# chaoting-sun/GCT-Plus

Hardware: AMD Instinct MI355X
Metric: SMILES/sec training step (vaetf, seq_len=80, d_model=512) (higher is better)
Workload: dtype f32

## Files before the change

### gct_plus_amd/csrc/gemm.hip

```cpp
#include <limits.h>
#include <stdlib.h>

#include <type_traits>

#include "common.h"

typedef float f32x16 __attribute__((ext_vector_type(16)));

namespace {

constexpr int BM = 128, BN = 128, BK = 32;
constexpr int TILE_FLOATS = BM * BK;

struct Seg3 {
  const float* p0;
  int64_t d1, d2;
};

struct GemmArgs {
  int64_t M, N, K;
  Seg3 a;
  int64_t lda;
  int64_t a_nper;
  Seg3 b;
// ... 839 lines not shown
int64_t g_x3_kernel_launches = 0;
#include "gemm_x6.inc"

__global__ __launch_bounds__(256) void gemm_f32_small_kernel(const GemmArgs g) {
  constexpr int SB = 64, STILE = SB * BK;
  __shared__ __attribute__((aligned(16))) float lds[4 * STILE];
  const int tid = threadIdx.x, lane = tid & 63, wave = tid >> 6;
  const int wm = (wave >> 1) * 32, wn = (wave & 1) * 32;
  const unsigned tiles_n = (unsigned)((g.N + SB - 1) / SB);
  const unsigned tiles_m = (unsigned)((g.M + SB - 1) / SB);
  const unsigned lid0 = gct_xcd_remap(blockIdx.x, gridDim.x);
  const unsigned z = lid0 / (tiles_m * tiles_n), lid = lid0 - z * (tiles_m * tiles_n);
  const int64_t m0 = (int64_t)(lid / tiles_n) * SB, n0 = (int64_t)(lid % tiles_n) * SB;
  const int64_t kbeg = (int64_t)z * g.ksplit;
  const int64_t kend = (kbeg + g.ksplit < g.K) ? kbeg + g.ksplit : g.K;

  uint32_t offa[2], offb[2];
#pragma unroll
  for (int i = 0; i < 2; ++i) {
    int64_t r = (tid >> 3) + 32 * i;
    int64_t ra_ = r, rb_ = r;
    if (m0 + ra_ > g.M - 1) ra_ = g.M - 1 - m0;
    if (n0 + rb_ > g.N - 1) rb_ = g.N - 1 - n0;
    offa[i] = (uint32_t)(ra_ * g.lda + (tid & 7) * 4);
    offb[i] = (uint32_t)(rb_ * g.ldb + (tid & 7) * 4);
  }
  const bool g1 = n0 >= g.b_nper, g2 = n0 >= 2 * g.b_nper;
  const float* bbase0 = g.b.p0 + (g2 ? g.b.d2 : (g1 ? g.b.d1 : 0)) +
                        (n0 - (g2 ? 2 * g.b_nper : (g1 ? g.b_nper : 0))) * g.ldb;
  const float* abase0 = g.a.p0 + m0 * g.lda;

  f32x16 acc;
#pragma unroll
  for (int r = 0; r < 16; ++r) acc[r] = 0.f;
  float4 ra[2], rb[2];
  auto gload = [&](int64_t k0) {
#pragma unroll
    for (int i = 0; i < 2; ++i) {
      ra[i] = *reinterpret_cast<const float4*>(abase0 + k0 + offa[i]);
      rb[i] = *reinterpret_cast<const float4*>(bbase0 + k0 + offb[i]);
    }
  };
  auto lstore = [&](int buf) {
    float* la = lds + buf * 2 * STILE;
    float* lb = la + STILE;
    const int c8 = tid & 7;
#pragma unroll
    for (int i = 0; i < 2; ++i) {
      const int row = (tid >> 3) + 32 * i;
      const int chunk = c8 ^ ((row >> 1) & 7);
      *reinterpret_cast<float4*>(la + row * BK + chunk * 4) = ra[i];
      *reinterpret_cast<float4*>(lb + row * BK + chunk * 4) = rb[i];
    }
  };
  const int64_t nkt = (kend - kbeg) / BK;
  gload(kbeg);
  lstore(0);
  __syncthreads();
  const int h = lane >> 5;
  for (int64_t kt = 0; kt < nkt; ++kt) {
    const int cur = (int)(kt & 1);
    if (kt + 1 < nkt) gload(kbeg + (kt + 1) * BK);
    const float* la = lds + cur * 2 * STILE;
    const float* lb = la + STILE;
    const int rowa = wm + (lane & 31), rowb = wn + (lane & 31);
    const int swa = (rowa >> 1) & 7, swb = (rowb >> 1) & 7;
#pragma unroll
    for (int c = 0; c < 4; ++c) {
      const float4 a4 = *reinterpret_cast<const float4*>(la + rowa * BK + (((h * 4 + c) ^ swa) * 4));
      const float4 b4 = *reinterpret_cast<const float4*>(lb + rowb * BK + (((h * 4 + c) ^ swb) * 4));
      acc = __builtin_amdgcn_mfma_f32_32x32x2f32(a4.x, b4.x, acc, 0, 0, 0);
      acc = __builtin_amdgcn_mfma_f32_32x32x2f32(a4.y, b4.y, acc, 0, 0, 0);
      acc = __builtin_amdgcn_mfma_f32_32x32x2f32(a4.z, b4.z, acc, 0, 0, 0);
      acc = __builtin_amdgcn_mfma_f32_32x32x2f32(a4.w, b4.w, acc, 0, 0, 0);
    }
    if (kt + 1 < nkt) lstore(cur ^ 1);
    __syncthreads();
  }
  float* stg = lds + wave * 1024;
  {
    const int c32 = lane & 31;
#pragma unroll
    for (int r = 0; r < 16; ++r) stg[((r & 3) + 8 * (r >> 2) + 4 * h) * 32 + c32] = acc[r];
  }
  __builtin_amdgcn_s_waitcnt(0xC07F);
  __builtin_amdgcn_wave_barrier();
  const FastEpi ep{g};
  const int rg = lane >> 3, c4 = lane & 7;
  const int64_t row0 = m0 + wm + rg * 4, col0 = n0 + wn + c4 * 4;
  if (row0 < g.M && col0 < g.N) {
    float4 v[4];
#pragma unroll
    for (int rr = 0; rr < 4; ++rr) v[rr] = *reinterpret_cast<const float4*>(stg + (rg * 4 + rr) * 32 + c4 * 4);
    if (g.epi == EPI_SLAB) {
      float* sl = g.c0 + (int64_t)z * g.slab_stride;
#pragma unroll
      for (int rr = 0; rr < 4; ++rr)
        if (row0 + rr < g.M) *reinterpret_cast<float4*>(sl + (row0 + rr) * g.N + col0) = v[rr];
      return;
    }
    const bool q1 = col0 >= g.c_nper, q2 = col0 >= 2 * g.c_nper;
    const int64_t cloc = col0 - (q2 ? 2 * g.c_nper : (q1 ? g.c_nper : 0));
    float* cbase = g.c0 + (q2 ? g.c_d2 : (q1 ? g.c_d1 : 0));
    float4 bias = make_float4(0.f, 0.f, 0.f, 0.f);
    if (g.bias0) bias = *reinterpret_cast<const float4*>(g.bias0 + (q2 ? g.bias_d2 : (q1 ? g.bias_d1 : 0)) + cloc);
    ep.apply(v, row0, col0, cbase, cloc, bias);
  }
}


template <int TN, bool RAGGED = false>
__global__ __launch_bounds__(256) void gemm_f32_panel_kernel(const GemmArgs g) {
  constexpr int TM = 32, KC = 256, SD = KC + 4, NBL = TN / 4;
  extern __shared__ __attribute__((aligned(16))) float plds[];
  float* As = plds;
  float* Bs = plds + TM * SD;
  const int tid = threadIdx.x, lane = tid & 63, wave = tid >> 6, g4 = lane >> 4, c16 = lane & 15;
  const unsigned tiles_m = (unsigned)((g.M + TM - 1) / TM);
  const unsigned lid = gct_xcd_remap(blockIdx.x, gridDim.x);
  const int64_t m0 = (int64_t)(lid % tiles_m) * TM, n0 = (int64_t)(lid / tiles_m) * TN;
  const bool s1 = n0 >= g.b_nper, s2 = n0 >= 2 * g.b_nper;
  const float* bbase = g.b.p0 + (s2 ? g.b.d2 : (s1 ? g.b.d1 : 0)) + (n0 - (s2 ? 2 * g.b_nper : (s1 ? g.b_nper : 0))) * g.ldb;
  const float* abase = g.a.p0;
  uint32_t offa[8], offb[NBL];
#pragma unroll
  for (int i = 0; i < 8; ++i) {
    const int idx = tid + 256 * i, row = idx >> 6, c4 = idx & 63;
    int64_t r = m0 + row;
    if (r > g.M - 1) r = g.M - 1;
    offa[i] = (uint32_t)(r * g.lda + c4 * 4);
  }
#pragma unroll
  for (int i = 0; i < NBL; ++i) {
    const int idx = tid + 256 * i, c4 = idx & 63;
    int64_t row = idx >> 6;
    if (RAGGED && n0 + row > g.N - 1) row = g.N - 1 - n0;
    offb[i] = (uint32_t)(row * g.ldb + c4 * 4);
  }
  f32x4_t ra[8], rb[NBL];
  auto gload = [&](int64_t k0) {
#pragma unroll
    for (int i = 0; i < 8; ++i) ra[i] = *reinterpret_cast<const f32x4_t*>(abase + k0 + offa[i]);
#pragma unroll
    for (int i = 0; i < NBL; ++i) rb[i] = *reinterpret_cast<const f32x4_t*>(bbase + k0 + offb[i]);
  };
  auto lstore = [&]() {
#pragma unroll
    for (int i = 0; i < 8; ++i) {
      const int idx = tid + 256 * i;
      *reinterpret_cast<f32x4_t*>(As + (idx >> 6) * SD + (idx & 63) * 4) = ra[i];
    }
#pragma unroll
    for (int i = 0; i < NBL; ++i) {
      const int idx = tid + 256 * i;
      *reinterpret_cast<f32x4_t*>(Bs + (idx >> 6) * SD + (idx & 63) * 4) = rb[i];
    }
  };
  constexpr int NS = TN / 32;
  const int wm = (wave >> 1) * 16, wn = (wave & 1) * (TN / 2);
  f32x4_t acc[NS];
#pragma unroll
  for (int j = 0; j < NS; ++j) acc[j] = (f32x4_t){0.f, 0.f, 0.f, 0.f};
  const int64_t nch = g.K / KC;
  gload(0);
  lstore();
  __syncthreads();
  for (int64_t c = 0; c < nch; ++c) {
    if (c + 1 < nch) gload((c + 1) * KC);
    const float* ap = As + (wm + c16) * SD + g4 * 64;
#pragma unroll 4
    for (int j = 0; j < 16; ++j) {
      const float4 a4 = *reinterpret_cast<const float4*>(ap + 4 * j);
#pragma unroll
      for (int u = 0; u < NS; ++u) {
        const float4 b4 = *reinterpret_cast<const float4*>(Bs + (wn + 16 * u + c16) * SD + g4 * 64 + 4 * j);
        acc[u] = __builtin_amdgcn_mfma_f32_16x16x4f32(a4.x, b4.x, acc[u], 0, 0, 0);
        acc[u] = __builtin_amdgcn_mfma_f32_16x16x4f32(a4.y, b4.y, acc[u], 0, 0, 0);
        acc[u] = __builtin_amdgcn_mfma_f32_16x16x4f32(a4.z, b4.z, acc[u], 0, 0, 0);
        acc[u] = __builtin_amdgcn_mfma_f32_16x16x4f32(a4.w, b4.w, acc[u], 0, 0, 0);
      }
    }
    __syncthreads();
    if (c + 1 < nch) {
      lstore();
      __syncthreads();
    }
  }
  float* stg = plds + wave * (16 * 20);
  const FastEpi ep{g};
#pragma unroll
  for (int u = 0; u < NS; ++u) {
#pragma unroll
    for (int i = 0; i < 4; ++i) stg[(4 * g4 + i) * 20 + c16] = acc[u][i];
    __builtin_amdgcn_s_waitcnt(0xC07F);
    __builtin_amdgcn_wave_barrier();
    if (lane < 16) {
      const int pr = lane >> 2, pc = lane & 3;
      const int64_t row0 = m0 + wm + 4 * pr, col0 = n0 + wn + 16 * u + 4 * pc;
      if (RAGGED) {
        for (int rr = 0; rr < 4; ++rr)
          for (int cc = 0; cc < 4; ++cc)
            if (row0 + rr < g.M && col0 + cc < g.N)
              g.c0[(row0 + rr) * g.ldc + col0 + cc] = stg[(4 * pr + rr) * 20 + 4 * pc + cc] + (g.bias0 ? g.bias0[col0 + cc] : 0.f);
      } else if (row0 < g.M && col0 < g.N) {
        float4 v[4];
#pragma unroll
        for (int rr = 0; rr < 4; ++rr) v[rr] = *reinterpret_cast<const float4*>(stg + (4 * pr + rr) * 20 + 4 * pc);
        const bool q1 = col0 >= g.c_nper, q2 = col0 >= 2 * g.c_nper;
        const int64_t cloc = col0 - (q2 ? 2 * g.c_nper : (q1 ? g.c_nper : 0));
        float* cbase = g.c0 + (q2 ? g.c_d2 : (q1 ? g.c_d1 : 0));
        float4 bias = make_float4(0.f, 0.f, 0.f, 0.f);
        if (g.bias0) bias = *reinterpret_cast<const float4*>(g.bias0 + (q2 ? g.bias_d2 : (q1 ? g.bias_d1 : 0)) + cloc);
        ep.apply(v, row0, col0, cbase, cloc, bias);
      }
    }
    __builtin_amdgcn_s_waitcnt(0xC07F);
    __builtin_amdgcn_wave_barrier();
  }
}

template <int TN, bool RAGGED = false>
int launch_panel(const GemmArgs& g, hipStream_t st) {
  constexpr size_t LDS = (size_t)(32 + TN) * 260 * sizeof(float);
  static bool attr_set = false;
  if (!attr_set) {
    hipError_t e = hipFuncSetAttribute((const void*)gemm_f32_panel_kernel<TN, RAGGED>, hipFuncAttributeMaxDynamicSharedMemorySize, (int)LDS);
    if (e != hipSuccess) {
      gct_set_error("gemm_f32_panel: cannot reserve %zu bytes of LDS: %s", LDS, hipGetErrorString(e));
      return GCT_ERR_HIP;
    }
    attr_set = true;
  }
  const int64_t tiles = ((g.M + 31) / 32) * (RAGGED ? 1 : g.N / TN);
  hipLaunchKernelGGL((gemm_f32_panel_kernel<TN, RAGGED>), dim3((unsigned)tiles), dim3(256), LDS, st, g);
  GCT_LAUNCH_CHECK("gemm_f32_panel");
  return GCT_OK;
}

__global__ __launch_bounds__(256) void splitk_epilogue_kernel(const GemmArgs g, const float* slabs,
                                                              int nslab, int64_t slab_stride) {
  const int64_t pc = g.N / 4, pr = (g.M + 3) / 4;
  const int64_t idx = (int64_t)blockIdx.x * blockDim.x + threadIdx.x;
  if (idx >= pc * pr) return;
  const int64_t row0 = (idx / pc) * 4, col0 = (idx % pc) * 4;
  float4 v[4];
#pragma unroll
  for (int rr = 0; rr < 4; ++rr) {
    v[rr] = make_float4(0.f, 0.f, 0.f, 0.f);
    if (row0 + rr < g.M) {
      const float* p = slabs + (row0 + rr) * g.N + col0;
      for (int s = 0; s < nslab; ++s) {
        const float4 t = *reinterpret_cast<const float4*>(p + (int64_t)s * slab_stride);
        v[rr].x += t.x; v[rr].y += t.y; v[rr].z += t.z; v[rr].w += t.w;
      }
    }
  }
  const bool q1 = col0 >= g.c_nper, q2 = col0 >= 2 * g.c_nper;
  const int64_t cloc = col0 - (q2 ? 2 * g.c_nper : (q1 ? g.c_nper : 0));
  float* cbase = g.c0 + (q2 ? g.c_d2 : (q1 ? g.c_d1 : 0));
  float4 bias = make_float4(0.f, 0.f, 0.f, 0.f);
  if (g.bias0) bias = *reinterpret_cast<const float4*>(g.bias0 + (q2 ? g.bias_d2 : (q1 ? g.bias_d1 : 0)) + cloc);
  const FastEpi ep{g};
  ep.apply(v, row0, col0, cbase, cloc, bias);
}

int g_gemm_mode = -1;
int64_t g_gemm_launches[2] = {0, 0};
inline int gemm_mode() {
  if (g_gemm_mode < 0) {
    const char* e = getenv("GCT_GEMM_MODE");
    g_gemm_mode = (e && (e[0] == 'f' || e[0] == '0')) ? GCT_GEMM_F32 : GCT_GEMM_BF16X6;
  }
  return g_gemm_mode;
}

template <bool A_KC, bool B_KC>
bool fast_ok(const GemmArgs& g, bool vec) {
  auto seg_ok = [](int64_t nper, int64_t extent, int64_t gran) { return nper >= extent || nper % gran == 0; };
  return vec && g.K % BK == 0 && g.ksplit % BK == 0 && g.M >= 4 && g.N >= 4 &&
         (A_KC ? seg_ok(g.a_nper, g.K, BK) : (seg_ok(g.a_nper, g.M, BM) && g.M % 4 == 0)) &&
         (B_KC ? seg_ok(g.b_nper, g.N, BN) : (seg_ok(g.b_nper, g.K, BK) && g.N % 4 == 0)) &&
         g.N % 4 == 0 && g.ldc % 4 == 0 && gct_aligned16(g.c0) && g.c_d1 % 4 == 0 && g.c_d2 % 4 == 0 &&
         (g.c_nper >= g.N || g.c_nper % 4 == 0) && g.slab_stride % 4 == 0 &&
         (!g.bias0 || (gct_aligned16(g.bias0) && g.bias_d1 % 4 == 0 && g.bias_d2 % 4 == 0)) &&
         (!g.resid || gct_aligned16(g.resid)) && (!g.pre || gct_aligned16(g.pre)) &&
         (!g.pre_in || gct_aligned16(g.pre_in)) && 130 * g.lda < (1ll << 31) && 130 * g.ldb < (1ll << 31);
}


inline int64_t slab_bytes(int64_t s, int64_t rows, int64_t cols) {
  return s > 1 ? s * rows * cols * (int64_t)sizeof(float) : 0;
}

inline bool skinny_m(int64_t M, int64_t N) { return ((M + BM - 1) / BM) * ((N + BN - 1) / BN) < 192; }

int skinny_splits(int64_t M, int64_t N, int64_t K) {
  const int64_t tiles = ((M + 63) / 64) * ((N + 63) / 64);
  if (tiles <= 0) return 1;
  int64_t ns = 768 / tiles;
  if (ns > K / BK / 4) ns = K / BK / 4;
  return ns < 1 ? 1 : (int)ns;
}

int x6_tail_plan(int64_t M, int64_t N, int64_t K, int64_t* m1_out) {
  constexpr int64_t CUS = 256;
  const int64_t tm = (M + XBM - 1) / XBM, tn = (N + XBN - 1) / XBN, tiles = tm * tn;
  const int64_t rem = tiles % CUS;
  if (tiles <= CUS || rem == 0 || rem % tn != 0 || K % XBK != 0) return 1;
  const int64_t nkt = K / XBK;
  int best = 1;
  double cost = 1.0;
  const double o = 3.3;
  for (int s2 = 2; s2 <= 8 && nkt / s2 >= 2; ++s2) {
    const double c = (double)((rem * s2 + CUS - 1) / CUS) * (o + (double)nkt / s2) / (o + nkt) + 0.05;
    if (c < cost - 1e-9) { cost = c; best = s2; }
  }
  if (best == 1 || cost > 0.75) return 1;
  *m1_out = (tiles - rem) / tn * XBM;
  return best;
}

int x6_splitk_all_plan(int64_t M, int64_t N, int64_t K) {
  constexpr int64_t CUS = 256;
  const int64_t tiles = ((M + XBM - 1) / XBM) * ((N + XBN - 1) / XBN), nkt = K / XBK;
  if (tiles > CUS / 2 || K % XBK != 0 || nkt < 32 || M < 1024 || (nkt < 64 && M < 2048)) return 1;
  int64_t sp = CUS / tiles;
  if (sp > nkt / 8) sp = nkt / 8;
  if (sp > 8) sp = 8;
  return sp < 2 ? 1 : (int)sp;
}


inline int64_t x6s_tiles(int64_t M, int64_t N) { return ((M + SBM - 1) / SBM) * ((N + SBN - 1) / SBN); }

inline bool x6s_shape(const GemmArgs& g) {
  const int64_t big = ((g.M + XBM - 1) / XBM) * ((g.N + XBN - 1) / XBN), small = x6s_tiles(g.M, g.N), nkt = g.K / XBK;
  return big <= 160 && small >= 96 && small <= (nkt <= 16 ? 512 : 256) && nkt <= 32;
}

constexpr int64_t X6_TAIL_SMALL_MAX = 512;

constexpr int64_t PANEL32_MAX_TILES = 4096, PANEL64_MAX_TILES = 768;


static_assert(BK == XBK, "the fp32 and bf16x6 kernels split K at the same granularity");
GemmArgs slab_args(const GemmArgs& g, int splits, float* ws) {
  const int64_t nkt = g.K / BK;
  GemmArgs p = g;
  p.ksplit = ((nkt + splits - 1) / splits) * BK;
  p.nsplit = (int)((g.K + p.ksplit - 1) / p.ksplit);
  p.epi = EPI_SLAB; p.c0 = ws; p.ldc = g.N; p.slab_stride = g.M * g.N;
  p.c_d1 = p.c_d2 = 0; p.c_nper = INT64_MAX / 4; p.bias0 = nullptr; p.resid = nullptr; p.pre = nullptr; p.pre_in = nullptr;
  return p;
}

int launch_fixup(const GemmArgs& g, const GemmArgs& slabs, hipStream_t st, const char* name) {
  const int64_t patches = ((g.M + 3) / 4) * (g.N / 4);
  hipLaunchKernelGGL(splitk_epilogue_kernel, dim3((unsigned)((patches + 255) / 256)), dim3(256), 0, st, g,
                     (const float*)slabs.c0, slabs.nsplit, slabs.slab_stride);
  GCT_LAUNCH_CHECK(name);
  return GCT_OK;
}

template <int MODE, int NP>
int launch_x6_tail_split(const GemmArgs& g, hipStream_t st, float* ws, int64_t ws_bytes) {
  if (MODE == X6_WGRAD || g.nsplit != 1 || !ws || !gct_aligned16(ws)) return launch_x6<MODE, NP>(g, st);
  int64_t m1 = 0;
  const int best = x6_tail_plan(g.M, g.N, g.K, &m1);
  const int64_t m2 = g.M - m1, nkt = g.K / XBK;
  hipStreamCaptureStatus cap = hipStreamCaptureStatusNone;
  if (best == 1 || slab_bytes(best, m2, g.N) > ws_bytes ||
      hipStreamIsCapturing(st, &cap) != hipSuccess || cap != hipStreamCaptureStatusNone)
    return launch_x6<MODE, NP>(g, st);
  GemmArgs head = g;
  head.M = m1;
  int rc = launch_x6<MODE, NP>(head, st);
  if (rc) return rc;
  GemmArgs e = g;
  e.M = m2; e.row_base = g.row_base + m1;
  e.a.p0 += m1 * g.lda;
  e.c0 += m1 * g.ldc;
  if (e.resid) e.resid += m1 * g.ldc;
  if (e.pre) e.pre += m1 * g.ldc;
  if (e.pre_in && !(g.pre_rows > 0 && g.quad_map)) e.pre_in += m1 * g.ldc;
  if (nkt <= 32 && x6s_tiles(m2, g.N) <= X6_TAIL_SMALL_MAX) {
    if (MODE == X6_FWD && x6s_ok(e, true)) return launch_x6s<X6_FWD, NP>(e, st);
    if (MODE == X6_DGRAD && x6s_dgrad_ok(e, true)) return launch_x6s<X6_DGRAD, NP>(e, st);
  }
  const GemmArgs p = slab_args(e, best, ws);
  rc = launch_x6<MODE, NP>(p, st);
  if (rc) return rc;
  return launch_fixup(e, p, st, "x6 tail fix-up");
}

struct GemmRoute {
  enum Kind {
    X6S,
    X6_SPLITK_ALL,
    PANEL_THIN,
    PANEL32,
    PANEL64,
    F32_SMALL,
    X6,
    F32_FAST,
    F32_VEC,
    F32,
  } kind;
  int splits;
};

template <bool A_KC, bool B_KC>
GemmRoute plan_gemm(const GemmArgs& g, bool vec, int mode, const float* ws, int64_t ws_bytes) {
  constexpr bool FWD = A_KC && B_KC, DGRAD = A_KC && !B_KC;
  constexpr int MODE = A_KC ? (B_KC ? X6_FWD : X6_DGRAD) : X6_WGRAD;
  const bool x6 = mode == GCT_GEMM_BF16X6 || mode == GCT_GEMM_BF16X3;
  const bool x6_fwd = x6 && FWD && g.epi < EPI_D0, x6_dgrad = x6 && DGRAD && g.epi >= EPI_D0 && g.epi < EPI_SLAB;
  const bool ws_ok = ws && gct_aligned16(ws);
  if (x6_fwd || x6_dgrad) {
    const bool x6s = x6_fwd ? x6s_ok(g, vec) : x6s_dgrad_ok(g, vec);
    if (x6s && x6s_shape(g)) return {GemmRoute::X6S, 1};
    if (x6_fwd && x6s && !x6_ok<X6_FWD>(g, vec) && x6s_tiles(g.M, g.N) >= 96) return {GemmRoute::X6S, 1};
    const int sp = x6_splitk_all_plan(g.M, g.N, g.K);
    if (x6_ok<MODE>(g, vec) && g.nsplit == 1 && ws_ok && sp > 1 && slab_bytes(sp, g.M, g.N) <= ws_bytes)
      return {GemmRoute::X6_SPLITK_ALL, sp};
  }
  if (FWD && vec && g.N <= 32 && g.K % 256 == 0 && g.epi == GCT_EPI_BIAS && g.nsplit == 1 && g.b_nper >= g.N &&
      g.c_nper >= g.N && g.M >= 1 && g.lda * 4 * 33 < (1ll << 31) && g.ldb * 4 * 33 < (1ll << 31) && g.M < (1ll << 36))
    return {GemmRoute::PANEL_THIN, 1};
  const bool fast = fast_ok<A_KC, B_KC>(g, vec);
  if (FWD && fast && g.nsplit == 1 && skinny_m(g.M, g.N) && g.epi < EPI_D0 && (g.b_nper >= g.N || g.b_nper % 64 == 0)) {
    if (g.K % 256 == 0 && g.lda * 4 * 33 < (1ll << 31) && g.ldb * 4 * 65 < (1ll << 31) &&
        (g.c_nper >= g.N || g.c_nper % 64 == 0)) {
      const int64_t tm32 = (g.M + 31) / 32;
      if (g.N % 32 == 0 && (g.b_nper >= g.N || g.b_nper % 32 == 0) && tm32 * (g.N / 32) <= PANEL32_MAX_TILES)
        return {GemmRoute::PANEL32, 1};
      if (g.N % 64 == 0 && tm32 * (g.N / 64) <= PANEL64_MAX_TILES) return {GemmRoute::PANEL64, 1};
    }
    int64_t ns = 1;
    if (ws_ok) {
      const int64_t slab = g.M * g.N * (int64_t)sizeof(float);
      ns = skinny_splits(g.M, g.N, g.K);
      if (ns * slab > ws_bytes) ns = ws_bytes / slab;
      if (ns < 1) ns = 1;
    }
    return {GemmRoute::F32_SMALL, (int)ns};
  }
  if (x6 && (A_KC || !B_KC) && x6_ok<MODE>(g, vec)) return {GemmRoute::X6, 1};
  return {fast ? GemmRoute::F32_FAST : (vec ? GemmRoute::F32_VEC : GemmRoute::F32), 1};
}

template <bool A_KC, bool B_KC>
int launch(const GemmArgs& g, bool vec, hipStream_t st, float* ws = nullptr, int64_t ws_bytes = 0) {
  constexpr int MODE = A_KC ? (B_KC ? X6_FWD : X6_DGRAD) : X6_WGRAD;
  const int64_t tiles = ((g.M + BM - 1) / BM) * ((g.N + BN - 1) / BN) * g.nsplit;
  if (tiles <= 0) return GCT_OK;
  if (tiles > INT_MAX) {
    gct_set_error("gemm: grid too large");
    return GCT_ERR_ARG;
  }
  const int mode = gemm_mode();
  const bool x3 = mode == GCT_GEMM_BF16X3;
  const GemmRoute r = plan_gemm<A_KC, B_KC>(g, vec, mode, ws, ws_bytes);
  switch (r.kind) {
    case GemmRoute::X6S:
      if (x3) return launch_x6s<B_KC ? X6_FWD : X6_DGRAD, 2>(g, st);
      ++g_gemm_launches[1];
      return launch_x6s<B_KC ? X6_FWD : X6_DGRAD, 3>(g, st);
    case GemmRoute::X6_SPLITK_ALL: {
      const GemmArgs p = slab_args(g, r.splits, ws);
      int rc = x3 ? launch_x6<MODE, 2>(p, st) : launch_x6<MODE, 3>(p, st);
      if (!rc) rc = launch_fixup(g, p, st, "x6 split-K fix-up");
      if (!rc && !x3) ++g_gemm_launches[1];
      return rc;
    }
    case GemmRoute::PANEL_THIN:
      ++g_gemm_launches[0];
      return launch_panel<32, true>(g, st);
    case GemmRoute::PANEL32:
      return launch_panel<32>(g, st);
    case GemmRoute::PANEL64:
      return launch_panel<64>(g, st);
    case GemmRoute::F32_SMALL: {
      const int64_t tiles64 = ((g.M + 63) / 64) * ((g.N + 63) / 64);
      if (r.splits == 1) {
        hipLaunchKernelGGL(gemm_f32_small_kernel, dim3((unsigned)tiles64), dim3(256), 0, st, g);
        GCT_LAUNCH_CHECK("gemm_f32_small");
        return GCT_OK;
      }
      const GemmArgs p = slab_args(g, r.splits, ws);
      hipLaunchKernelGGL(gemm_f32_small_kernel, dim3((unsigned)(tiles64 * p.nsplit)), dim3(256), 0, st, p);
      GCT_LAUNCH_CHECK("gemm_f32_small(split-K)");
      return launch_fixup(g, p, st, "splitk_epilogue");
    }
    case GemmRoute::X6:
      if (x3) return launch_x6_tail_split<MODE, 2>(g, st, ws, ws_bytes);
      ++g_gemm_launches[1];
      return launch_x6_tail_split<MODE, 3>(g, st, ws, ws_bytes);
    default:
      break;
  }
  ++g_gemm_launches[0];
  const dim3 grid((unsigned)tiles), block(256);
  if (r.kind == GemmRoute::F32_FAST)
    hipLaunchKernelGGL((gemm_f32_fast_kernel<A_KC, B_KC>), grid, block, 0, st, g);
  else if (r.kind == GemmRoute::F32_VEC)
    hipLaunchKernelGGL((gemm_f32_kernel<A_KC, B_KC, true>), grid, block, 0, st, g);
  else
    hipLaunchKernelGGL((gemm_f32_kernel<A_KC, B_KC, false>), grid, block, 0, st, g);
  GCT_LAUNCH_CHECK("gemm_f32");
  return GCT_OK;
}

inline bool al16(const void* p) { return p == nullptr || gct_aligned16(p); }

inline Seg3 mkseg(const float* p0, const float* p1, const float* p2) {
  Seg3 r;
  r.p0 = p0;
  r.d1 = p1 ? (int64_t)(p1 - p0) : 0;
  r.d2 = p2 ? (int64_t)(p2 - p0) : 0;
  return r;
}

}

int gct_reduce_slabs_seg(const float* slabs, int nslab, int64_t stride, float* d0, float* d1,
                         float* d2, int64_t nper_elems, int64_t n, hipStream_t st);
int gct_reduce_slabs_seg2(const float* sa, int nslab, int64_t stride_a, float* a0, float* a1, float* a2,
                          int64_t nper_a, int64_t na, const float* sb, int64_t stride_b, float* b0, float* b1,
                          float* b2, int64_t nper_b, int64_t nb, hipStream_t st);
int gct_colsum(const float* y0, const float* y1, const float* y2, int64_t ld, int64_t M, int nseg,
               int nper, float* d0, float* d1, float* d2, float* ws, hipStream_t st);
int64_t gct_colsum_ws_floats(int64_t M, int64_t N);

static int wgrad_splits(int64_t M, int64_t Ntot, int64_t K, bool x6 = false) {
  const int64_t tiles = x6 ? ((Ntot + XBM - 1) / XBM) * ((K + XBN - 1) / XBN)
                           : ((Ntot + BM - 1) / BM) * ((K + BN - 1) / BN);
  int64_t want = (x6 ? 256 : 512) / tiles;
  const int64_t maxs = (M + 4 * BK - 1) / (4 * BK);
  if (want > maxs) want = maxs;
  if (want < 1) want = 1;
  if (want > 64) want = 64;
  return (int)want;
}

extern "C" int64_t gct_wgrad_ws_bytes(int64_t M, int64_t Ntot, int64_t K) {
  const int s1 = wgrad_splits(M, Ntot, K), s2 = wgrad_splits(M, Ntot, K, true);
  const int s = s1 > s2 ? s1 : s2;
  const int64_t slab = (int64_t)s * Ntot * K;
  const int64_t cs = gct_colsum_ws_floats(M, Ntot);
  const int64_t need = slab + 4 + (int64_t)s * Ntot;
  return (need > cs ? need : cs) * (int64_t)sizeof(float) + 256;
}

extern "C" int gct_linear_fwd(const float* x, int64_t ldx, int64_t M, int K, const float* w0,
                              const float* w1, const float* w2, int64_t ldw, const uint16_t* wp0,
                              int64_t plane_stride, const float* b0, const float* b1,
                              const float* b2, int nseg, int nper, float* y0, float* y1, float* y2,
                              int64_t ldy, int epi, const float* resid, float* pre, float p,
                              uint64_t seed, uint32_t site, float* ws, int64_t ws_bytes,
                              const int32_t* quad_map, void* stream) {
  GCT_CHECK_ARG(x && w0 && y0 && M >= 0 && K > 0 && nseg >= 1 && nseg <= 3 && nper > 0,
                "linear_fwd: bad args");
  GCT_CHECK_ARG(!quad_map || M % 4 == 0, "linear_fwd: compacted rows come in quads");
  GCT_CHECK_ARG(ws_bytes >= 0, "linear_fwd: negative workspace size");
  GCT_CHECK_ARG(nseg < 2 || (w1 && y1), "linear_fwd: missing segment 1");
  GCT_CHECK_ARG(nseg < 3 || (w2 && y2), "linear_fwd: missing segment 2");
  GCT_CHECK_ARG(epi == GCT_EPI_BIAS || nseg == 1, "linear_fwd: fused epilogues need nseg == 1");
  GCT_CHECK_ARG(epi >= GCT_EPI_BIAS && epi <= GCT_EPI_GELU_DROP_SAVE, "linear_fwd: unknown epilogue %d", epi);
  GCT_CHECK_ARG((epi != GCT_EPI_GELU_DROP && epi != GCT_EPI_GELU_DROP_SAVE) || pre, "linear_fwd: GELU epilogue needs pre");
  GCT_CHECK_ARG(epi != GCT_EPI_DROP_RESID || resid, "linear_fwd: residual epilogue needs resid");
  GCT_CHECK_ARG(p >= 0.f && p < 1.f, "linear_fwd: dropout p out of range");
  GemmArgs g = {};
  g.M = M; g.N = (int64_t)nseg * nper; g.K = K;
  GCT_CHECK_ARG(!b0 || nseg < 2 || b1, "linear_fwd: bias of segment 1 missing");
  GCT_CHECK_ARG(!b0 || nseg < 3 || b2, "linear_fwd: bias of segment 2 missing");
  g.a = mkseg(x, nullptr, nullptr); g.lda = ldx; g.a_nper = INT64_MAX / 4;
  g.b = mkseg(w0, w1, w2); g.ldb = ldw; g.b_nper = nper;
  g.c0 = y0; g.c_d1 = y1 ? y1 - y0 : 0; g.c_d2 = y2 ? y2 - y0 : 0; g.ldc = ldy; g.c_nper = nper;
  g.ksplit = K; g.nsplit = 1; g.epi = epi;
  g.bias0 = b0; g.bias_d1 = (b0 && b1) ? b1 - b0 : 0; g.bias_d2 = (b0 && b2) ? b2 - b0 : 0;
  g.resid = resid; g.pre = pre;
  g.thr = gct_drop_threshold(p); g.keep_scale = 1.0f / (1.0f - p); g.rng = gct_rng_make(seed, site);
  g.bp0 = wp0; g.bp_stride = plane_stride;
  g.quad_map = quad_map;
  const bool vec = al16(x) && al16(w0) && al16(w1) && al16(w2) && (ldx % 4 == 0) &&
                   (ldw % 4 == 0) && (K % 4 == 0);
  return launch<true, true>(g, vec, (hipStream_t)stream, ws, ws ? ws_bytes : 0);
}

extern "C" int gct_gemm_set_mode(int mode) {
  GCT_CHECK_ARG(mode == GCT_GEMM_F32 || mode == GCT_GEMM_BF16X6 || mode == GCT_GEMM_BF16X3,
                "gemm_set_mode: unknown mode %d", mode);
  g_gemm_mode = mode;
  return GCT_OK;
}
extern "C" int gct_gemm_get_mode(void) { return gemm_mode(); }
extern "C" int64_t gct_gemm_x6_kernel_launches(void) { return g_x6_kernel_launches; }
extern "C" int64_t gct_gemm_x3_launches(void) { return g_x3_kernel_launches; }
extern "C" int gct_gemm_launch_counts(int64_t* out2) {
  GCT_CHECK_ARG(out2, "gemm_launch_counts: null");
  out2[0] = g_gemm_launches[0]; out2[1] = g_gemm_launches[1];
  return GCT_OK;
}

extern "C" int gct_split_planes(const float* src, int64_t numel, uint16_t* planes, int64_t plane_stride,
                                void* stream) {
  GCT_CHECK_ARG(src && planes && numel >= 0 && numel % 4 == 0 && plane_stride >= numel && plane_stride % 4 == 0 &&
                    gct_aligned16(src) && ((((uintptr_t)planes) & 7u) == 0),
                "split_planes: bad args (numel and plane_stride must be multiples of 4, src 16-B aligned)");
  if (numel == 0) return GCT_OK;
  const int64_t n4 = numel / 4;
  hipLaunchKernelGGL(split_planes_kernel, dim3((unsigned)((n4 + 255) / 256)), dim3(256), 0, (hipStream_t)stream,
                     src, planes, n4, plane_stride);
  GCT_LAUNCH_CHECK("split_planes");
  return GCT_OK;
}

extern "C" int64_t gct_linear_fwd_ws_bytes(int64_t M, int K, int Ntot) {
  int64_t need = 0, m1 = 0;
  if (skinny_m(M, Ntot)) {
    need = slab_bytes(skinny_splits(M, Ntot, K), M, Ntot);
  } else {
    const int s = x6_tail_plan(M, Ntot, K, &m1);
    need = slab_bytes(s, M - m1, Ntot);
  }
  const int64_t all = slab_bytes(x6_splitk_all_plan(M, Ntot, K), M, Ntot);
  return (need > all ? need : all) + 256;
}

extern "C" int64_t gct_linear_dgrad_ws_bytes(int64_t M, int Ntot, int K) {
  int64_t m1 = 0;
  const int s = x6_tail_plan(M, K, Ntot, &m1);
  const int64_t tail = slab_bytes(s, M - m1, K);
  const int64_t all = slab_bytes(x6_splitk_all_plan(M, K, Ntot), M, K);
  return (tail > all ? tail : all) + 256;
}

extern "C" int gct_linear_dgrad(const float* dy0, const float* dy1, const float* dy2, int64_t lddy,
                                int64_t M, int nseg, int nper, const float* w0, const float* w1,
                                const float* w2, int64_t ldw, const uint16_t* wp0,
                                int64_t plane_stride, int K, float* dx, int64_t lddx, int depi,
                                const float* pre, float p, uint64_t seed, uint32_t site,
                                float* ws, int64_t ws_bytes, const int32_t* quad_map, int64_t pre_rows,
                                void* stream) {
  GCT_CHECK_ARG(ws_bytes >= 0, "linear_dgrad: negative workspace size");
  GCT_CHECK_ARG(dy0 && w0 && dx && M >= 0 && K > 0 && nseg >= 1 && nseg <= 3 && nper > 0,
                "linear_dgrad: bad args");
  GCT_CHECK_ARG(!quad_map || M % 4 == 0, "linear_dgrad: compacted rows come in quads");
  GCT_CHECK_ARG(nseg < 2 || (w1 && dy1), "linear_dgrad: missing segment 1");
  GCT_CHECK_ARG(nseg < 3 || (w2 && dy2), "linear_dgrad: missing segment 2");
  GCT_CHECK_ARG(depi >= GCT_DEPI_STORE && depi <= GCT_DEPI_MUL_SAVED, "linear_dgrad: unknown epilogue %d", depi);
  GCT_CHECK_ARG(depi != GCT_DEPI_GELU_BWD || pre, "linear_dgrad: GELU bwd needs pre");
  GCT_CHECK_ARG(depi != GCT_DEPI_MUL_SAVED || pre, "linear_dgrad: saved-factor epilogue needs pre");
  GCT_CHECK_ARG(p >= 0.f && p < 1.f, "linear_dgrad: dropout p out of range");
  GemmArgs g = {};
  g.M = M; g.N = K; g.K = (int64_t)nseg * nper;
  g.a = mkseg(dy0, dy1, dy2); g.lda = lddy; g.a_nper = nper;
  g.b = mkseg(w0, w1, w2); g.ldb = ldw; g.b_nper = nper;
  g.c0 = dx; g.ldc = lddx; g.c_nper = INT64_MAX / 4;
  g.ksplit = g.K; g.nsplit = 1; g.epi = EPI_D0 + depi;
  g.pre_in = pre;
  g.thr = gct_drop_threshold(p); g.keep_scale = 1.0f / (1.0f - p); g.rng = gct_rng_make(seed, site);
  g.bp0 = wp0; g.bp_stride = plane_stride;
  g.quad_map = quad_map;
  g.pre_rows = quad_map ? pre_rows : 0;
  const bool vec = al16(dy0) && al16(dy1) && al16(dy2) && al16(w0) && al16(w1) && al16(w2) &&
                   (lddy % 4 == 0) && (ldw % 4 == 0) && (nper % 4 == 0) && (K % 4 == 0);
  return launch<true, false>(g, vec, (hipStream_t)stream, ws, ws ? ws_bytes : 0);
}

extern "C" int gct_linear_wgrad(const float* dy0, const float* dy1, const float* dy2, int64_t lddy,
                                int64_t M, int nseg, int nper, const float* x, int64_t ldx, int K,
                                float* dw0, float* dw1, float* dw2, int64_t lddw, float* db0,
                                float* db1, float* db2, float* ws, const int32_t* tile_list,
                                const int32_t* tile_count, void* stream) {
  GCT_CHECK_ARG(dy0 && x && dw0 && ws && M >= 0 && K > 0 && nseg >= 1 && nseg <= 3 && nper > 0,
                "linear_wgrad: bad args");
  GCT_CHECK_ARG(nseg < 2 || (dy1 && dw1), "linear_wgrad: missing segment 1");
  GCT_CHECK_ARG(nseg < 3 || (dy2 && dw2), "linear_wgrad: missing segment 2");
  GCT_CHECK_ARG(lddw == K, "linear_wgrad: dW must be dense [nper][K]");
  hipStream_t st = (hipStream_t)stream;
  const int64_t Ntot = (int64_t)nseg * nper;
  const bool vec = al16(dy0) && al16(dy1) && al16(dy2) && al16(x) && (lddy % 4 == 0) &&
                   (ldx % 4 == 0) && (nper % 4 == 0) && (K % 4 == 0);
  GemmArgs g = {};
  g.M = Ntot; g.N = K; g.K = M;
  g.a = mkseg(dy0, dy1, dy2); g.lda = lddy; g.a_nper = nper;
  g.b = mkseg(x, nullptr, nullptr); g.ldb = ldx; g.b_nper = INT64_MAX / 4;
  g.c0 = ws; g.ldc = K; g.c_nper = INT64_MAX / 4;
  g.slab_stride = Ntot * K;
  g.ksplit = BK; g.nsplit = 1; g.epi = EPI_SLAB;
  const bool use_x6 = gemm_mode() != GCT_GEMM_F32 && x6_ok<X6_WGRAD>(g, vec);
  if (use_x6 && tile_list && tile_count) { g.kt_list = tile_list; g.kt_count = tile_count; }
  const int splits = wgrad_splits(M, Ntot, K, use_x6);
  int64_t ks = (M + splits - 1) / splits;
  ks = (ks + BK - 1) / BK * BK;
  g.ksplit = ks > 0 ? ks : BK;
  g.nsplit = (int)((M + g.ksplit - 1) / g.ksplit);
  if (g.nsplit < 1) g.nsplit = 1;
  g.epi = EPI_SLAB;
  float* bslab = nullptr;
  if (db0) {
    if (use_x6 || fast_ok<false, false>(g, vec)) {
      int64_t off = (int64_t)g.nsplit * g.slab_stride;
      off = (off + 3) / 4 * 4;
      bslab = ws + off;
      g.bias_slab = bslab;
    } else {
      int rc = gct_colsum(dy0, dy1, dy2, lddy, M, nseg, nper, db0, db1, db2, ws, st);
      if (rc) return rc;
    }
  }
  int rc = launch<false, false>(g, vec, st);
  if (rc) return rc;
  if (bslab)
    return gct_reduce_slabs_seg2(ws, g.nsplit, g.slab_stride, dw0, dw1, dw2, (int64_t)nper * K, Ntot * K, bslab, Ntot,
                                 db0, db1, db2, nper, Ntot, st);
  return gct_reduce_slabs_seg(ws, g.nsplit, g.slab_stride, dw0, dw1, dw2, (int64_t)nper * K, Ntot * K, st);
}
```

### gct_plus_amd/csrc/gemm_x6.inc

```

typedef __bf16 x6_bf16x8 __attribute__((ext_vector_type(8)));
typedef __bf16 x6_bf16x2 __attribute__((ext_vector_type(2)));
typedef float x6_f32x2 __attribute__((ext_vector_type(2)));
typedef unsigned x6_u32x4 __attribute__((ext_vector_type(4)));
typedef unsigned x6_u32x2 __attribute__((ext_vector_type(2)));
typedef short x6_s16x4 __attribute__((ext_vector_type(4)));
typedef short x6_s16x8 __attribute__((ext_vector_type(8)));

enum { X6_FWD = 0, X6_DGRAD = 1, X6_WGRAD = 2 };
constexpr int XBM = 128, XBN = 256, XBK = 32;
constexpr int X_APL = 8192, X_BPL = 16384, X_STAGE = 3 * X_APL + 3 * X_BPL;
constexpr int X_KLIST_MAX = 1024;
constexpr int X_LDS_BYTES = 2 * X_STAGE + X_KLIST_MAX * 4;

__device__ __forceinline__ unsigned x6_pk(float a, float b) {
  x6_f32x2 v = {a, b};
  return __builtin_bit_cast(unsigned, __builtin_convertvector(v, x6_bf16x2));
}
__device__ __forceinline__ float x6_sub(float a, float b) {
  float r;
  asm("v_sub_f32 %0, %1, %2" : "=v"(r) : "v"(a), "v"(b));
  return r;
}
__device__ __forceinline__ void x6_split2(float a, float b, unsigned& h, unsigned& m, unsigned& l) {
  h = x6_pk(a, b);
  const float ra = x6_sub(a, __uint_as_float(h << 16)), rb = x6_sub(b, __uint_as_float(h & 0xffff0000u));
  m = x6_pk(ra, rb);
  const float sa = x6_sub(ra, __uint_as_float(m << 16)), sb = x6_sub(rb, __uint_as_float(m & 0xffff0000u));
  l = x6_pk(sa, sb);
}
__device__ __forceinline__ void x6_split4(const float4 v, x6_u32x2& h, x6_u32x2& m, x6_u32x2& l) {
  unsigned h0, m0, l0, h1, m1, l1;
  x6_split2(v.x, v.y, h0, m0, l0);
  x6_split2(v.z, v.w, h1, m1, l1);
  h = x6_u32x2{h0, h1}; m = x6_u32x2{m0, m1}; l = x6_u32x2{l0, l1};
}
template <int NP>
__device__ __forceinline__ void x6_split4n(const float4 v, x6_u32x2 (&pc)[NP]) {
  if constexpr (NP == 3) {
    x6_split4(v, pc[0], pc[1], pc[2]);
  } else {
    static_assert(NP == 2, "bf16x6 (3 pieces) or bf16x3 (2 pieces)");
    unsigned h0, h1;
    h0 = x6_pk(v.x, v.y);
    h1 = x6_pk(v.z, v.w);
    const float r0 = x6_sub(v.x, __uint_as_float(h0 << 16)), r1 = x6_sub(v.y, __uint_as_float(h0 & 0xffff0000u));
    const float r2 = x6_sub(v.z, __uint_as_float(h1 << 16)), r3 = x6_sub(v.w, __uint_as_float(h1 & 0xffff0000u));
    pc[0] = x6_u32x2{h0, h1};
    pc[1] = x6_u32x2{x6_pk(r0, r1), x6_pk(r2, r3)};
  }
}

__device__ __forceinline__ int x6_row_off(int r, int c) {
  const int g = (0x78 >> (2 * ((r >> 2) & 3))) & 3;
  return r * 64 + ((c ^ g) << 4);
}
__device__ __forceinline__ int x6_tr_off(int k, int cb, int stride) {
  return k * stride + (cb ^ (((k & 3) << 6) | (((k >> 3) & 1) << 5)));
}

__device__ __forceinline__ x6_bf16x8 x6_tr_frag(const unsigned char* p, int stride) {
  typedef __attribute__((address_space(3))) x6_s16x4 lds_s16x4;
  const x6_s16x4 lo = __builtin_amdgcn_ds_read_tr16_b64_v4i16((lds_s16x4*)(p));
  const x6_s16x4 hi = __builtin_amdgcn_ds_read_tr16_b64_v4i16((lds_s16x4*)(p + 4 * stride));
  const x6_s16x8 v = __builtin_shufflevector(lo, hi, 0, 1, 2, 3, 4, 5, 6, 7);
  return __builtin_bit_cast(x6_bf16x8, v);
}

typedef float x6_f32x4 __attribute__((ext_vector_type(4)));
#define X6_MFMA(a_, b_, c_) c_ = __builtin_amdgcn_mfma_f32_16x16x32_bf16(a_, b_, c_, 0, 0, 0)

template <int MODE, int NP = 3>
__global__ __launch_bounds__(512) __attribute__((amdgpu_waves_per_eu(2, 2))) void
gemm_x6_kernel(const GemmArgs g) {
  static_assert(NP == 2 || NP == 3, "bf16x3 or bf16x6");
  extern __shared__ __attribute__((aligned(16))) unsigned char xlds[];
  constexpr bool A_TR = MODE == X6_WGRAD, B_TR = MODE != X6_FWD, B_PL = MODE != X6_WGRAD;
  constexpr int NB = B_PL ? 2 : 4;
  const int tid = threadIdx.x, lane = tid & 63, wave = tid >> 6;
  const int wm = (wave >> 2) * 64, wn = (wave & 3) * 64;

  const unsigned tiles_n = (unsigned)((g.N + XBN - 1) / XBN);
  const unsigned tiles_m = (unsigned)((g.M + XBM - 1) / XBM);
  const unsigned per_split = tiles_m * tiles_n;
  const unsigned lid = gct_xcd_remap(blockIdx.x, gridDim.x);
  const unsigned z = lid / per_split, rest = lid - z * per_split;
  const int64_t m0 = (int64_t)(rest / tiles_n) * XBM, n0 = (int64_t)(rest % tiles_n) * XBN;
  const int64_t kbeg = (int64_t)z * g.ksplit;
  const int64_t kend = (kbeg + g.ksplit < g.K) ? kbeg + g.ksplit : g.K;

  uint32_t offa[2], offb[NB];
  int sta[2], stb[NB];
#pragma unroll
  for (int j = 0; j < 2; ++j) {
    if (!A_TR) {
      int64_t r = (tid >> 3) + 64 * j;
      sta[j] = x6_row_off((int)r, (tid & 7) >> 1) + (tid & 1) * 8;
      if (m0 + r > g.M - 1) r = g.M - 1 - m0;
      offa[j] = (uint32_t)(r * g.lda + (tid & 7) * 4);
    } else {
      const int kr = (tid >> 5) + 16 * j;
      int64_t c = (tid & 31) * 4;
      sta[j] = x6_tr_off(kr, (tid & 31) * 8, 256);
      if (m0 + c > g.M - 4) c = g.M - 4 - m0;
      offa[j] = (uint32_t)(kr * g.lda + c);
    }
  }
#pragma unroll
  for (int j = 0; j < NB; ++j) {
    if (MODE == X6_FWD) {
      int64_t r = (tid >> 2) + 128 * j;
      stb[j] = x6_row_off((int)r, tid & 3);
      if (n0 + r > g.N - 1) r = g.N - 1 - n0;
      offb[j] = (uint32_t)(r * g.ldb + (tid & 3) * 8);
    } else if (MODE == X6_DGRAD) {
      const int kr = (tid >> 5) + 16 * j;
      int64_t c = (tid & 31) * 8;
      stb[j] = x6_tr_off(kr, (tid & 31) * 16, 512);
      if (n0 + c > g.N - 8) c = g.N - 8 - n0;
      offb[j] = (uint32_t)(kr * g.ldb + c);
    } else {
      const int kr = (tid >> 6) + 8 * j;
      int64_t c = (tid & 63) * 4;
      stb[j] = x6_tr_off(kr, (tid & 63) * 8, 512);
      if (n0 + c > g.N - 4) c = g.N - 4 - n0;
      offb[j] = (uint32_t)(kr * g.ldb + c);
    }
  }
  auto seg_off = [](const Seg3& s, int64_t idx, int64_t nper, int64_t& local) -> int64_t {
    const bool g1 = idx >= nper, g2 = idx >= 2 * nper;
    local = idx - (g2 ? 2 * nper : (g1 ? nper : 0));
    return g2 ? s.d2 : (g1 ? s.d1 : 0);
  };
  int64_t a_fix = 0, b_fix = 0;
  {
    int64_t loc;
    if (A_TR) { a_fix = seg_off(g.a, m0, g.a_nper, loc); a_fix += loc; }
    else a_fix = m0 * g.lda;
    if (MODE == X6_FWD) { b_fix = seg_off(g.b, n0, g.b_nper, loc); b_fix += loc * g.ldb; }
    else b_fix = n0;
  }
  auto abase = [&](int64_t k0) -> const float* {
    if (A_TR) return g.a.p0 + a_fix + k0 * g.lda;
    int64_t loc;
    const int64_t so = seg_off(g.a, k0, g.a_nper, loc);
    return g.a.p0 + so + a_fix + loc;
  };
  auto boff = [&](int64_t k0) -> int64_t {
    if (MODE == X6_FWD) return b_fix + k0;
    int64_t loc;
    const int64_t so = seg_off(g.b, k0, g.b_nper, loc);
    return so + loc * g.ldb + b_fix;
  };

  x6_f32x4 acc[4][4];
#pragma unroll
  for (int i = 0; i < 4; ++i)
#pragma unroll
    for (int j = 0; j < 4; ++j) acc[i][j] = x6_f32x4{0.f, 0.f, 0.f, 0.f};

  float4 pa[2];
  x6_u32x4 pbp[NP][2];
  float4 pbf[4];
#define X6_GLOAD(k0_)                                                                          \
  do {                                                                                         \
    const float* ab__ = abase(k0_);                                                            \
    const int64_t bo__ = boff(k0_);                                                            \
    _Pragma("unroll") for (int j = 0; j < 2; ++j)                                              \
        pa[j] = *reinterpret_cast<const float4*>(ab__ + offa[j]);                              \
    if (B_PL) {                                                                                \
      _Pragma("unroll") for (int p = 0; p < NP; ++p)                                           \
      _Pragma("unroll") for (int j = 0; j < 2; ++j)                                            \
          pbp[p][j] = *reinterpret_cast<const x6_u32x4*>(g.bp0 + p * g.bp_stride + bo__ + offb[j]); \
    } else {                                                                                   \
      _Pragma("unroll") for (int j = 0; j < 4; ++j)                                            \
          pbf[j] = *reinterpret_cast<const float4*>(g.b.p0 + bo__ + offb[j]);                  \
    }                                                                                          \
  } while (0)
#define X6_LSTORE(st_)                                                                         \
  do {                                                                                         \
    unsigned char* s__ = (st_);                                                                \
    _Pragma("unroll") for (int j = 0; j < 2; ++j) {                                            \
      x6_u32x2 pc__[NP];                                                                       \
      x6_split4n<NP>(pa[j], pc__);                                                             \
      _Pragma("unroll") for (int p = 0; p < NP; ++p)                                           \
          *reinterpret_cast<x6_u32x2*>(s__ + p * X_APL + sta[j]) = pc__[p];                    \
    }                                                                                          \
    if (B_PL) {                                                                                \
      _Pragma("unroll") for (int p = 0; p < NP; ++p)                                           \
      _Pragma("unroll") for (int j = 0; j < 2; ++j)                                            \
          *reinterpret_cast<x6_u32x4*>(s__ + 3 * X_APL + p * X_BPL + stb[j]) = pbp[p][j];      \
    } else {                                                                                   \
      _Pragma("unroll") for (int j = 0; j < 4; ++j) {                                          \
        x6_u32x2 pc__[NP];                                                                     \
        x6_split4n<NP>(pbf[j], pc__);                                                          \
        _Pragma("unroll") for (int p = 0; p < NP; ++p)                                         \
            *reinterpret_cast<x6_u32x2*>(s__ + 3 * X_APL + p * X_BPL + stb[j]) = pc__[p];      \
      }                                                                                        \
    }                                                                                          \
  } while (0)

  constexpr bool BAL = B_PL;
  x6_u32x2 pk[2][NP];
#define X6_GLOAD_A(k0_)                                                                        \
  do {                                                                                         \
    const float* ab__ = abase(k0_);                                                            \
    _Pragma("unroll") for (int j = 0; j < 2; ++j)                                              \
        pa[j] = *reinterpret_cast<const float4*>(ab__ + offa[j]);                              \
  } while (0)
#define X6_GLOAD_B(k0_)                                                                        \
  do {                                                                                         \
    const int64_t bo__ = boff(k0_);                                                            \
    _Pragma("unroll") for (int p = 0; p < NP; ++p)                                             \
    _Pragma("unroll") for (int j = 0; j < 2; ++j)                                              \
        pbp[p][j] = *reinterpret_cast<const x6_u32x4*>(g.bp0 + p * g.bp_stride + bo__ + offb[j]); \
  } while (0)
#define X6_SPLIT_A()                                                                           \
  _Pragma("unroll") for (int j = 0; j < 2; ++j) x6_split4n<NP>(pa[j], pk[j]);
#define X6_LSTORE_PK(st_)                                                                      \
  do {                                                                                         \
    unsigned char* s__ = (st_);                                                                \
    _Pragma("unroll") for (int j = 0; j < 2; ++j)                                              \
    _Pragma("unroll") for (int p = 0; p < NP; ++p)                                             \
        *reinterpret_cast<x6_u32x2*>(s__ + p * X_APL + sta[j]) = pk[j][p];                     \
    _Pragma("unroll") for (int p = 0; p < NP; ++p)                                             \
    _Pragma("unroll") for (int j = 0; j < 2; ++j)                                              \
        *reinterpret_cast<x6_u32x4*>(s__ + 3 * X_APL + p * X_BPL + stb[j]) = pbp[p][j];        \
  } while (0)

  const int fr = lane & 15, fc = lane >> 4;
  const int tq = (lane & 15) >> 2, tp = lane & 3;
  int fao[4], fbo[4];
#pragma unroll
  for (int i = 0; i < 4; ++i) {
    fao[i] = A_TR ? x6_tr_off(8 * fc + tq, (wm + 16 * i + 4 * tp) * 2, 256) : x6_row_off(wm + 16 * i + fr, fc);
    fbo[i] = 3 * X_APL + (B_TR ? x6_tr_off(8 * fc + tq, (wn + 16 * i + 4 * tp) * 2, 512)
                               : x6_row_off(wn + 16 * i + fr, fc));
  }
  x6_bf16x8 fA01[2][NP], fA23[2][NP], fB01[2][NP], fB23[2][NP];
#define X6_LD_A(dst_, st_, i0_)                                                                \
  _Pragma("unroll") for (int ii = 0; ii < 2; ++ii)                                             \
  _Pragma("unroll") for (int p = 0; p < NP; ++p) {                                             \
    if (A_TR) dst_[ii][p] = x6_tr_frag((st_) + p * X_APL + fao[(i0_) + ii], 256);              \
    else dst_[ii][p] = *reinterpret_cast<const x6_bf16x8*>((st_) + p * X_APL + fao[0] + ((i0_) + ii) * 1024); \
  }
#define X6_LD_B(dst_, st_, j0_)                                                                \
  _Pragma("unroll") for (int jj = 0; jj < 2; ++jj)                                             \
  _Pragma("unroll") for (int p = 0; p < NP; ++p) {                                             \
    if (B_TR) dst_[jj][p] = x6_tr_frag((st_) + p * X_BPL + fbo[(j0_) + jj], 512);              \
    else dst_[jj][p] = *reinterpret_cast<const x6_bf16x8*>((st_) + p * X_BPL + fbo[0] + ((j0_) + jj) * 1024); \
  }
#define X6_MM(a_, b_, i0_, j0_)                                                                \
  _Pragma("unroll") for (int ii = 0; ii < 2; ++ii)                                             \
  _Pragma("unroll") for (int jj = 0; jj < 2; ++jj) {                                           \
    if constexpr (NP == 3) {                                                                   \
      X6_MFMA(a_[ii][NP - 1], b_[jj][0], acc[(i0_) + ii][(j0_) + jj]);                         \
      X6_MFMA(a_[ii][0], b_[jj][NP - 1], acc[(i0_) + ii][(j0_) + jj]);                         \
      X6_MFMA(a_[ii][1], b_[jj][1], acc[(i0_) + ii][(j0_) + jj]);                              \
    }                                                                                          \
    X6_MFMA(a_[ii][1], b_[jj][0], acc[(i0_) + ii][(j0_) + jj]);                                \
    X6_MFMA(a_[ii][0], b_[jj][1], acc[(i0_) + ii][(j0_) + jj]);                                \
    X6_MFMA(a_[ii][0], b_[jj][0], acc[(i0_) + ii][(j0_) + jj]);                                \
  }

  float4 bsum = make_float4(0.f, 0.f, 0.f, 0.f);
  const float bw0 = (MODE == X6_WGRAD && g.bias_slab && n0 == 0) ? 1.f : 0.f;
#define X6_BSUM(w_)                                                                            \
  _Pragma("unroll") for (int j = 0; j < 2; ++j) {                                              \
    bsum.x = fmaf(w_, pa[j].x, bsum.x); bsum.y = fmaf(w_, pa[j].y, bsum.y);                    \
    bsum.z = fmaf(w_, pa[j].z, bsum.z); bsum.w = fmaf(w_, pa[j].w, bsum.w);                    \
  }

#ifdef GCT_STAMPS
  unsigned long long seg[8] = {0, 0, 0, 0, 0, 0, 0, 0}, tprev;
  asm volatile("s_memtime %0\n\ts_waitcnt lgkmcnt(0)" : "=s"(tprev)::"memory");
#endif
  int64_t nkt = (kend - kbeg) / XBK;
  int64_t lt0 = 0;
  const int32_t* klist = (MODE == X6_WGRAD) ? g.kt_list : nullptr;
  if (klist) {
    const int64_t cnt = *g.kt_count;
    const int64_t per = (cnt + g.nsplit - 1) / g.nsplit;
    lt0 = (int64_t)z * per;
    nkt = cnt - lt0 < per ? cnt - lt0 : per;
    if (nkt < 0) nkt = 0;
  }
  int32_t* kl_s = reinterpret_cast<int32_t*>(xlds + 2 * X_STAGE);
  const bool kl_cached = klist && nkt <= X_KLIST_MAX;
  if (kl_cached) {
    for (int i = tid; i < nkt; i += 512) kl_s[i] = klist[lt0 + i];
    __syncthreads();
  }
  auto ktile = [&](int64_t t) -> int64_t {
    const int64_t tc = t < nkt ? t : nkt - 1;
    if (kl_cached) return (int64_t)__builtin_amdgcn_readfirstlane(kl_s[tc]) * XBK;
    return klist ? (int64_t)klist[lt0 + tc] * XBK : kbeg + tc * XBK;
  };
  if (nkt > 0) {
    if (BAL) {
      X6_GLOAD_A(ktile(0));
      X6_GLOAD_B(ktile(0));
      X6_SPLIT_A()
      X6_LSTORE_PK(xlds);
      X6_GLOAD_A(ktile(1));
      X6_GLOAD_B(ktile(1));
      X6_SPLIT_A()
      X6_GLOAD_A(ktile(2));
    } else {
      X6_GLOAD(ktile(0));
      if (MODE == X6_WGRAD) { X6_BSUM(bw0) }
      X6_LSTORE(xlds);
      X6_GLOAD(ktile(1));
    }
  }
  __syncthreads();
  if (nkt > 0) {
    X6_LD_A(fA01, xlds, 0)
    X6_LD_B(fB01, xlds, 0)
  }
  STAMP(0);
  constexpr int RA = 2 * NP * (A_TR ? 2 : 1), RB = 2 * NP * (B_TR ? 2 : 1);
  constexpr int NWR = B_PL ? 4 * NP : 6 * NP;
  constexpr int NG = 2 * NP;
  constexpr int MPW = NP == 3 ? 2 : 1;
  auto ktile_in = [&](int64_t t) -> int64_t { return kbeg + t * XBK; };
  int64_t k2n = nkt > 0 ? ktile(2) : 0;
  const int64_t mw = m0 + wm, nw = n0 + wn;
  constexpr int SIDE = MODE == X6_FWD ? 1 : (MODE == X6_DGRAD ? 2 : 3);
  EpiLane el;
  EpiAhead ah;
  float4 ex[4][4];
  int qv[4];
  if (BAL) epi_ahead_quads<SIDE>(g, lane, mw, nw, qv);
  auto ktile_iter = [&](auto tail_c, const int64_t kt) __attribute__((always_inline)) {
    constexpr int TAIL = decltype(tail_c)::value;
    constexpr bool NEXT1 = TAIL != 1 && TAIL != 4, NEXT2 = TAIL == 0 || TAIL == 3, NEXT3 = TAIL == 0, AHEAD = TAIL == 4;
    unsigned char* st = xlds + (kt & 1) * X_STAGE;
    unsigned char* stn = xlds + ((kt + 1) & 1) * X_STAGE;
    const int64_t k2 = k2n;
    if (TAIL == 0) k2n = BAL ? ktile_in(kt + 3) : ktile(kt + 3);
    __builtin_amdgcn_sched_barrier(0);
    X6_LD_A(fA23, st, 2)
    X6_LD_B(fB23, st, 2)
    if (MODE == X6_WGRAD) {
      const float bw = (kt + 1 < nkt) ? bw0 : 0.f;
      X6_BSUM(bw)
    }
    if (BAL) {
      if (NEXT1) { X6_LSTORE_PK(stn); }
      if (NEXT2) { X6_GLOAD_B(k2); }
      if (AHEAD) epi_ahead_issue<0, 1>(g, ah, ex);
    } else {
      X6_LSTORE(stn);
    }
    X6_MM(fA01, fB01, 0, 0)
    X6_MM(fA23, fB01, 2, 0)
#pragma unroll
    for (int q = 0; q < NG; ++q) {
      __builtin_amdgcn_sched_group_barrier(0x008, 1, 0);
      __builtin_amdgcn_sched_group_barrier(0x100, (RA + RB) / NG, 0);
    }
    if (BAL) {
#pragma unroll
      for (int q = 0; q < (NEXT1 ? NWR : 0); ++q) {
        __builtin_amdgcn_sched_group_barrier(0x008, MPW, 0);
        __builtin_amdgcn_sched_group_barrier(0x200, 1, 0);
      }
#pragma unroll
      for (int q = 0; q < (NEXT2 ? 2 * NP : (AHEAD ? 4 : 0)); ++q) {
        __builtin_amdgcn_sched_group_barrier(0x008, 2, 0);
        __builtin_amdgcn_sched_group_barrier(0x020, 1, 0);
      }
    } else {
#pragma unroll
      for (int q = 0; q < (NP == 3 ? 21 : 8); ++q) {
        __builtin_amdgcn_sched_group_barrier(0x008, 1, 0);
        __builtin_amdgcn_sched_group_barrier(0x002, NP == 3 ? 6 : 9, 0);
      }
#pragma unroll
      for (int q = 0; q < NWR; ++q) {
        __builtin_amdgcn_sched_group_barrier(0x008, 1, 0);
        __builtin_amdgcn_sched_group_barrier(0x200, 1, 0);
      }
    }
    __builtin_amdgcn_sched_barrier(0);
    STAMP(1);
    __syncthreads();
    STAMP(2);
    if (NEXT1) { X6_LD_B(fB01, stn, 0) }
    if (BAL) {
      if (NEXT2) { X6_SPLIT_A() }
      if (NEXT3) { X6_GLOAD_A(k2n); }
      if (AHEAD) epi_ahead_issue<1, 2>(g, ah, ex);
    } else {
      X6_GLOAD(k2);
    }
    X6_MM(fA01, fB23, 0, 2)
#pragma unroll
    for (int q = 0; q < (NEXT1 ? NG : 0); ++q) {
      __builtin_amdgcn_sched_group_barrier(0x008, 1, 0);
      __builtin_amdgcn_sched_group_barrier(0x100, RB / NG, 0);
    }
    if (BAL) {
#pragma unroll
      for (int q = 0; q < (NEXT2 ? (NP == 3 ? 14 : 6) : 0); ++q) {
        __builtin_amdgcn_sched_group_barrier(0x008, 1, 0);
        __builtin_amdgcn_sched_group_barrier(0x002, NP == 3 ? 3 : 4, 0);
      }
      if (NEXT3) {
        __builtin_amdgcn_sched_group_barrier(0x008, 2, 0);
        __builtin_amdgcn_sched_group_barrier(0x020, 2, 0);
      }
#pragma unroll
      for (int q = 0; q < (AHEAD ? 4 : 0); ++q) {
        __builtin_amdgcn_sched_group_barrier(0x008, 2, 0);
        __builtin_amdgcn_sched_group_barrier(0x020, 1, 0);
      }
    } else {
#pragma unroll
      for (int q = 0; q < (NP == 3 ? 8 : 4); ++q) {
        __builtin_amdgcn_sched_group_barrier(0x008, 2, 0);
        __builtin_amdgcn_sched_group_barrier(0x020, 1, 0);
      }
    }
    __builtin_amdgcn_sched_barrier(0);
    if (NEXT1) { X6_LD_A(fA01, stn, 0) }
    if (AHEAD) epi_ahead_issue<2, 4>(g, ah, ex);
    X6_MM(fA23, fB23, 2, 2)
#pragma unroll
    for (int q = 0; q < (AHEAD ? 8 : 0); ++q) {
      __builtin_amdgcn_sched_group_barrier(0x008, 2, 0);
      __builtin_amdgcn_sched_group_barrier(0x020, 1, 0);
    }
#pragma unroll
    for (int q = 0; q < (NEXT1 ? NG : 0); ++q) {
      __builtin_amdgcn_sched_group_barrier(0x008, 1, 0);
      __builtin_amdgcn_sched_group_barrier(0x100, RA / NG, 0);
    }
    __builtin_amdgcn_sched_barrier(0);
    STAMP(3);
    };
  if (BAL) {
    int64_t kt = 0;
    for (; kt < nkt - 3; ++kt) ktile_iter(std::integral_constant<int, 0>{}, kt);
    el = epi_lane(g, lane, nw, z);
    const bool ahead = nkt > 0 && epi_ahead_ok<SIDE>(g);
    ah.have = 0;
    if (ahead) ah = epi_ahead_plan<SIDE>(g, el, lane, mw, qv);
    if (nkt >= 3) ktile_iter(std::integral_constant<int, 3>{}, nkt - 3);
    if (nkt >= 2) ktile_iter(std::integral_constant<int, 2>{}, nkt - 2);
    if (ahead) ktile_iter(std::integral_constant<int, 4>{}, nkt - 1);
    else if (nkt >= 1) ktile_iter(std::integral_constant<int, 1>{}, nkt - 1);
  } else {
    for (int64_t kt = 0; kt < nkt; ++kt) ktile_iter(std::integral_constant<int, 0>{}, kt);
    __syncthreads();
  }
#undef X6_GLOAD
#undef X6_GLOAD_A
#undef X6_GLOAD_B
#undef X6_SPLIT_A
#undef X6_LSTORE_PK
#undef X6_LSTORE
#undef X6_LD_A
#undef X6_LD_B
#undef X6_MM
#undef X6_BSUM
  if (MODE == X6_WGRAD) {
    if (g.bias_slab && n0 == 0) {
      float4* red = reinterpret_cast<float4*>(xlds);
      red[tid] = bsum;
      __syncthreads();
      if (tid < 32) {
        float4 t4 = red[tid];
        for (int r = 1; r < 16; ++r) {
          const float4 u = red[r * 32 + tid];
          t4.x += u.x; t4.y += u.y; t4.z += u.z; t4.w += u.w;
        }
        const int64_t col = m0 + tid * 4;
        if (col + 3 < g.M) *reinterpret_cast<float4*>(g.bias_slab + (int64_t)z * g.M + col) = t4;
      }
      __syncthreads();
    }
  }
  STAMP(4);
  {
    float* stg = reinterpret_cast<float*>(xlds) + wave * 4096;
#pragma unroll
    for (int i = 0; i < 4; ++i)
#pragma unroll
      for (int j = 0; j < 4; ++j)
#pragma unroll
        for (int r = 0; r < 4; ++r) stg[(16 * i + 4 * fc + r) * 64 + 16 * j + fr] = acc[i][j][r];
#ifdef GCT_LAB_NO_EPI
    if (acc[0][0][0] == 123456.789f)
#endif
    {
      if (BAL) wave_epilogue_finish<SIDE>(g, stg, lane, mw, el, ex, ah.have);
      else wave_epilogue_tail<SIDE>(g, stg, lane, mw, nw, z);
    }
  }
#ifdef GCT_STAMPS
  __builtin_amdgcn_s_waitcnt(0x0070);
  STAMP(5);
  if (g.stamps && (threadIdx.x & 63) == 0 && blockIdx.x < 64) {
    for (int i = 0; i < 8; ++i) g.stamps[((size_t)blockIdx.x * 8 + (threadIdx.x >> 6)) * 8 + i] = seg[i];
  }
#endif
}

template <int MODE>
bool x6_ok(const GemmArgs& g, bool vec, int fwd_bn = XBN) {
  auto seg_ok = [](int64_t nper, int64_t extent, int64_t gran) { return nper >= extent || nper % gran == 0; };
  const bool common = vec && g.K % XBK == 0 && g.ksplit % XBK == 0 && g.K >= XBK && g.M >= 8 && g.N >= 8 &&
      g.N % 4 == 0 && g.ldc % 4 == 0 && gct_aligned16(g.c0) && g.c_d1 % 4 == 0 && g.c_d2 % 4 == 0 &&
      (g.c_nper >= g.N || g.c_nper % 4 == 0) && g.slab_stride % 4 == 0 &&
      (!g.bias0 || (gct_aligned16(g.bias0) && g.bias_d1 % 4 == 0 && g.bias_d2 % 4 == 0)) &&
      (!g.resid || gct_aligned16(g.resid)) && (!g.pre || gct_aligned16(g.pre)) &&
      (!g.pre_in || gct_aligned16(g.pre_in)) && 130 * g.lda < (1ll << 31) && 260 * g.ldb < (1ll << 31);
  if (!common) return false;
  if (MODE == X6_FWD)
    return g.bp0 && seg_ok(g.a_nper, g.K, XBK) && seg_ok(g.b_nper, g.N, fwd_bn) && g.ldb % 8 == 0 &&
           g.b.d1 % 8 == 0 && g.b.d2 % 8 == 0 && g.bp_stride % 8 == 0 && (((uintptr_t)g.bp0) & 15u) == 0;
  if (MODE == X6_DGRAD)
    return g.bp0 && seg_ok(g.a_nper, g.K, XBK) && seg_ok(g.b_nper, g.K, XBK) && g.N % 8 == 0 && g.ldb % 8 == 0 &&
           g.b.d1 % 8 == 0 && g.b.d2 % 8 == 0 && g.bp_stride % 8 == 0 && (((uintptr_t)g.bp0) & 15u) == 0;
  return seg_ok(g.a_nper, g.M, XBM) && g.M % 4 == 0;
}

template <int MODE, int NP>
int launch_x6(const GemmArgs& g, hipStream_t st) {
  const int64_t tiles = ((g.M + XBM - 1) / XBM) * ((g.N + XBN - 1) / XBN) * g.nsplit;
  if (tiles <= 0) return GCT_OK;
  if (tiles > INT_MAX) {
    gct_set_error("gemm_x6: grid too large");
    return GCT_ERR_ARG;
  }
  static bool attr_set = false;
  if (!attr_set) {
    hipError_t e = hipFuncSetAttribute((const void*)gemm_x6_kernel<MODE, NP>,
                                       hipFuncAttributeMaxDynamicSharedMemorySize, X_LDS_BYTES);
    if (e != hipSuccess) {
      gct_set_error("gemm_x6: cannot reserve %d bytes of LDS: %s", X_LDS_BYTES, hipGetErrorString(e));
      return GCT_ERR_HIP;
    }
    attr_set = true;
  }
  hipLaunchKernelGGL((gemm_x6_kernel<MODE, NP>), dim3((unsigned)tiles), dim3(512), X_LDS_BYTES, st, g);
  ++(NP == 3 ? g_x6_kernel_launches : g_x3_kernel_launches);
  GCT_LAUNCH_CHECK("gemm_x6");
  return GCT_OK;
}

constexpr int SBM = 64, SBN = 128;
constexpr int XS_APL = SBM * 64, XS_BPL = SBN * 64, XS_STAGE = 3 * XS_APL + 3 * XS_BPL;
constexpr int XS_LDS_BYTES = 2 * XS_STAGE;

template <int MODE, int NP = 3>
__global__ __launch_bounds__(512) void gemm_x6s_kernel(const GemmArgs g) {
  static_assert(NP == 2 || NP == 3, "bf16x3 or bf16x6");
  extern __shared__ __attribute__((aligned(16))) unsigned char xlds[];
  constexpr bool B_TR = MODE == X6_DGRAD;
  const int tid = threadIdx.x, lane = tid & 63, wave = tid >> 6;
  const int wm = (wave >> 2) * 32, wn = (wave & 3) * 32;
  const unsigned tiles_n = (unsigned)((g.N + SBN - 1) / SBN);
  const unsigned lid = gct_xcd_remap(blockIdx.x, gridDim.x);
  const int64_t m0 = (int64_t)(lid / tiles_n) * SBM, n0 = (int64_t)(lid % tiles_n) * SBN;
  int64_t ra = tid >> 3, rb = tid >> 2;
  const int sta = x6_row_off((int)ra, (tid & 7) >> 1) + (tid & 1) * 8;
  const int stb = B_TR ? x6_tr_off(tid >> 4, (tid & 15) * 16, 256) : x6_row_off((int)rb, tid & 3);
  if (m0 + ra > g.M - 1) ra = g.M - 1 - m0;
  if (n0 + rb > g.N - 1) rb = g.N - 1 - n0;
  const float* ap = g.a.p0 + (m0 + ra) * g.lda + (tid & 7) * 4;
  int64_t bo;
  if (B_TR) {
    int64_t c = (tid & 15) * 8;
    if (n0 + c > g.N - 8) c = g.N - 8 - n0;
    bo = (int64_t)(tid >> 4) * g.ldb + n0 + c;
  } else {
    const bool s1 = n0 >= g.b_nper, s2 = n0 >= 2 * g.b_nper;
    bo = (s2 ? g.b.d2 : (s1 ? g.b.d1 : 0)) + (n0 - (s2 ? 2 * g.b_nper : (s1 ? g.b_nper : 0)) + rb) * g.ldb + (tid & 3) * 8;
  }
  const uint16_t* bp = g.bp0 + bo;
  auto koff = [&](int64_t k0, int64_t& ao, int64_t& bko) {
    if (!B_TR) { ao = k0; bko = k0; return; }
    const bool a1 = k0 >= g.a_nper, a2 = k0 >= 2 * g.a_nper;
    ao = (a2 ? g.a.d2 : (a1 ? g.a.d1 : 0)) + (k0 - (a2 ? 2 * g.a_nper : (a1 ? g.a_nper : 0)));
    const bool b1 = k0 >= g.b_nper, b2 = k0 >= 2 * g.b_nper;
    bko = (b2 ? g.b.d2 : (b1 ? g.b.d1 : 0)) + (k0 - (b2 ? 2 * g.b_nper : (b1 ? g.b_nper : 0))) * g.ldb;
  };

  x6_f32x4 acc[2][2];
#pragma unroll
  for (int i = 0; i < 2; ++i)
#pragma unroll
    for (int j = 0; j < 2; ++j) acc[i][j] = x6_f32x4{0.f, 0.f, 0.f, 0.f};
  float4 pa;
  x6_u32x4 pb[NP];
  auto gload = [&](int64_t k0) {
    int64_t ao, bko;
    koff(k0, ao, bko);
    pa = *reinterpret_cast<const float4*>(ap + ao);
#pragma unroll
    for (int p = 0; p < NP; ++p) pb[p] = *reinterpret_cast<const x6_u32x4*>(bp + p * g.bp_stride + bko);
  };
  auto lstore = [&](unsigned char* st) {
    x6_u32x2 pc[NP];
    x6_split4n<NP>(pa, pc);
#pragma unroll
    for (int p = 0; p < NP; ++p) *reinterpret_cast<x6_u32x2*>(st + p * XS_APL + sta) = pc[p];
#pragma unroll
    for (int p = 0; p < NP; ++p) *reinterpret_cast<x6_u32x4*>(st + 3 * XS_APL + p * XS_BPL + stb) = pb[p];
  };
  const int fr = lane & 15, fc = lane >> 4;
  const int tq = (lane & 15) >> 2, tp = lane & 3;
  const int fao = x6_row_off(wm + fr, fc);
  int fbo[2];
#pragma unroll
  for (int j = 0; j < 2; ++j)
    fbo[j] = 3 * XS_APL + (B_TR ? x6_tr_off(8 * fc + tq, (wn + 16 * j + 4 * tp) * 2, 256)
                                : x6_row_off(wn + fr, fc) + j * 1024);
  const int64_t nkt = g.K / XBK;
  gload(0);
  lstore(xlds);
  if (nkt > 1) gload(XBK);
  __syncthreads();
  for (int64_t kt = 0; kt < nkt; ++kt) {
    const unsigned char* st = xlds + (kt & 1) * XS_STAGE;
    x6_bf16x8 fa[2][NP], fb[2][NP];
#pragma unroll
    for (int i = 0; i < 2; ++i)
#pragma unroll
      for (int p = 0; p < NP; ++p) {
        fa[i][p] = *reinterpret_cast<const x6_bf16x8*>(st + p * XS_APL + fao + i * 1024);
        if (B_TR) fb[i][p] = x6_tr_frag(st + p * XS_BPL + fbo[i], 256);
        else fb[i][p] = *reinterpret_cast<const x6_bf16x8*>(st + p * XS_BPL + fbo[i]);
      }
    if (kt + 1 < nkt) lstore(xlds + ((kt + 1) & 1) * XS_STAGE);
    if (kt + 2 < nkt) gload((kt + 2) * XBK);
#pragma unroll
    for (int i = 0; i < 2; ++i)
#pragma unroll
      for (int j = 0; j < 2; ++j) {
        if constexpr (NP == 3) {
          X6_MFMA(fa[i][NP - 1], fb[j][0], acc[i][j]);
          X6_MFMA(fa[i][0], fb[j][NP - 1], acc[i][j]);
          X6_MFMA(fa[i][1], fb[j][1], acc[i][j]);
        }
        X6_MFMA(fa[i][1], fb[j][0], acc[i][j]);
        X6_MFMA(fa[i][0], fb[j][1], acc[i][j]);
        X6_MFMA(fa[i][0], fb[j][0], acc[i][j]);
      }
#ifndef GCT_X6S_PLAIN
    __builtin_amdgcn_sched_group_barrier(0x100, NP == 3 ? (B_TR ? 15 : 9) : (B_TR ? 10 : 6), 0);
#pragma unroll
    for (int q = 0; q < (NP == 3 ? 3 : 2); ++q) {
      __builtin_amdgcn_sched_group_barrier(0x008, NP == 3 ? 2 : 1, 0);
      __builtin_amdgcn_sched_group_barrier(0x100, 1, 0);
    }
#pragma unroll
    for (int q = 0; q < (NP == 3 ? 6 : 3); ++q) {
      __builtin_amdgcn_sched_group_barrier(0x008, 1, 0);
      __builtin_amdgcn_sched_group_barrier(0x002, NP == 3 ? 5 : 4, 0);
    }
#pragma unroll
    for (int q = 0; q < 2 * NP; ++q) {
      __builtin_amdgcn_sched_group_barrier(0x008, 1, 0);
      __builtin_amdgcn_sched_group_barrier(0x200, 1, 0);
    }
#pragma unroll
    for (int q = 0; q < NP + 1; ++q) {
      __builtin_amdgcn_sched_group_barrier(0x008, 1, 0);
      __builtin_amdgcn_sched_group_barrier(0x020, 1, 0);
    }
    if constexpr (NP == 3) __builtin_amdgcn_sched_group_barrier(0x008, 2, 0);
#endif
    __syncthreads();
  }
  float* stg = reinterpret_cast<float*>(xlds) + wave * 1024;
#pragma unroll
  for (int i = 0; i < 2; ++i)
#pragma unroll
    for (int j = 0; j < 2; ++j)
#pragma unroll
      for (int r = 0; r < 4; ++r) stg[(16 * i + 4 * fc + r) * 32 + 16 * j + fr] = acc[i][j][r];
  __builtin_amdgcn_s_waitcnt(0xC07F);
  __builtin_amdgcn_wave_barrier();
  const FastEpiT<MODE == X6_FWD ? 1 : 2> ep{g};
  const int rg = lane >> 3, c4 = lane & 7;
  const int64_t row0 = m0 + wm + rg * 4, col0 = n0 + wn + c4 * 4;
  if (row0 < g.M && col0 < g.N) {
    float4 v[4];
#pragma unroll
    for (int rr = 0; rr < 4; ++rr) v[rr] = *reinterpret_cast<const float4*>(stg + (rg * 4 + rr) * 32 + c4 * 4);
    const bool q1 = col0 >= g.c_nper, q2 = col0 >= 2 * g.c_nper;
    const int64_t cloc = col0 - (q2 ? 2 * g.c_nper : (q1 ? g.c_nper : 0));
    float* cbase = g.c0 + (q2 ? g.c_d2 : (q1 ? g.c_d1 : 0));
    float4 bias = make_float4(0.f, 0.f, 0.f, 0.f);
    if (g.epi < EPI_D0 && g.bias0)
      bias = *reinterpret_cast<const float4*>(g.bias0 + (q2 ? g.bias_d2 : (q1 ? g.bias_d1 : 0)) + cloc);
    ep.apply(v, row0, col0, cbase, cloc, bias);
  }
}

inline bool x6s_ok(const GemmArgs& g, bool vec) {
  return x6_ok<X6_FWD>(g, vec, SBN) && g.nsplit == 1 && g.a_nper >= g.K && (g.b_nper >= g.N || g.b_nper % SBN == 0) &&
         (g.c_nper >= g.N || g.c_nper % 4 == 0) && g.epi < EPI_D0 && 70 * g.lda < (1ll << 31);
}
inline bool x6s_dgrad_ok(const GemmArgs& g, bool vec) {
  return x6_ok<X6_DGRAD>(g, vec) && g.nsplit == 1 && g.c_nper >= g.N && g.epi >= EPI_D0 && g.epi < EPI_SLAB &&
         70 * g.lda < (1ll << 31) && 40 * g.ldb < (1ll << 31);
}

template <int MODE, int NP>
inline int launch_x6s(const GemmArgs& g, hipStream_t st) {
  const int64_t tiles = ((g.M + SBM - 1) / SBM) * ((g.N + SBN - 1) / SBN);
  if (tiles <= 0) return GCT_OK;
  static bool attr_set = false;
  if (!attr_set) {
    hipError_t e = hipFuncSetAttribute((const void*)gemm_x6s_kernel<MODE, NP>, hipFuncAttributeMaxDynamicSharedMemorySize, XS_LDS_BYTES);
    if (e != hipSuccess) {
      gct_set_error("gemm_x6s: cannot reserve %d bytes of LDS: %s", XS_LDS_BYTES, hipGetErrorString(e));
      return GCT_ERR_HIP;
    }
    attr_set = true;
  }
  hipLaunchKernelGGL((gemm_x6s_kernel<MODE, NP>), dim3((unsigned)tiles), dim3(512), XS_LDS_BYTES, st, g);
  ++(NP == 3 ? g_x6_kernel_launches : g_x3_kernel_launches);
  GCT_LAUNCH_CHECK("gemm_x6s");
  return GCT_OK;
}

__global__ __launch_bounds__(256) void split_planes_kernel(const float* __restrict__ src, uint16_t* __restrict__ planes,
                                                           int64_t n4, int64_t pstride) {
  const int64_t i = (int64_t)blockIdx.x * 256 + threadIdx.x;
  if (i >= n4) return;
  const float4 v = reinterpret_cast<const float4*>(src)[i];
  x6_u32x2 h, m, l;
  x6_split4(v, h, m, l);
  *reinterpret_cast<x6_u32x2*>(planes + 4 * i) = h;
  *reinterpret_cast<x6_u32x2*>(planes + pstride + 4 * i) = m;
  *reinterpret_cast<x6_u32x2*>(planes + 2 * pstride + 4 * i) = l;
}
```

### gct_plus_amd/engine.py

```python
from __future__ import annotations

import math
import os
from typing import List, NamedTuple, Optional

import torch

from . import ops
from .flat import HANDED_SLOTS

_SEED = {"base": None, "ctr": 0}

COMPACT_BWD = os.environ.get("GCT_COMPACT_BWD", "1") != "0"
COMPACT_MAX_FRACTION = 0.85
COMPACT_KV = os.environ.get("GCT_COMPACT_KV", "1") != "0"
COMPACT_FWD = os.environ.get("GCT_COMPACT_FWD", "1") != "0"
COMPACT_ENC_KV = os.environ.get("GCT_COMPACT_ENC_KV", "1") != "0"


GRAD_NOTIFY = None


def _grads_done(module, G: "GradSink"):
    if GRAD_NOTIFY is not None:
        if ops.SIDE_ENABLED:
            ops.join_side()
        ps = list(module.parameters())
        GRAD_NOTIFY(ps, [G.out.get(p) for p in ps])


MODEL = "model"
DECODER = "decoder"
PREFILL = "prefill"
ENCODER = "encoder"


class RowMaps(NamedTuple):
    enc_keys: bool = False
    dec_keys: bool = False
    live: bool = False
    nc_lat: int = 0
    enc_rows: int = 0
    dec_rows: int = 0
    live_rows: int = 0


def plan_rows(caller, B=0, T=0, Le=0, mask_shape=None, *, loss_rows=False, trg_mask=False, get_attn=False,
              cond2dec=False, cond2lat=False, nconds=0, n_enc=0, n_dec=0, capturing=False, compact_fwd=False,
              compact_kv=False, compact_enc_kv=False) -> RowMaps:
    c2d = cond2dec and nconds > 0
    nc_lat = nconds if (not c2d and cond2lat and nconds > 0) else 0
    Td, Lk = T + (nconds if c2d else 0), Le + nc_lat
    none = RowMaps(nc_lat=nc_lat, enc_rows=B * Le, dec_rows=B * Lk, live_rows=B * Td)
    if caller == ENCODER or capturing:
        return none
    if caller == MODEL:
        if get_attn or mask_shape is None or tuple(mask_shape) != (B, 1, Le):
            return none
        mask_ok = True
    elif caller in (DECODER, PREFILL):
        mask_ok = mask_shape is not None and math.prod(mask_shape) == B * Le
    else:
        raise ValueError(f"plan_rows: unknown caller {caller!r}")
    return none._replace(
        enc_keys=bool(caller == MODEL and compact_enc_kv and n_enc > 0),
        dec_keys=bool(mask_ok and compact_kv and n_dec > 0),
        live=bool(compact_fwd and loss_rows and trg_mask and not get_attn and not c2d and n_dec > 0
                  and Td <= ops.ATTN_DIRECT_MAX_KEYS and Lk <= ops.ATTN_DIRECT_MAX_KEYS))


class RowPlan:

    def __init__(self, ek=None, dk=None, lr=None, rows=(0, 0, 0)):
        self._maps, self._rows = (ek, dk, lr), rows
        self._pending = ops.PendingReadBack(ek, dk, lr)
        self._usable = None
        self.enc_keys = self.dec_keys = self.live = None

    @staticmethod
    def usable_keys(h, rows):
        return h["nonprefix"] == 0 and h["empty"] == 0 and 0 < h["padded"] <= COMPACT_MAX_FRACTION * rows

    @staticmethod
    def usable_live(h, rows):
        return h["violations"] == 0 and h["nonprefix"] == 0 and 0 < h["padded"] <= COMPACT_MAX_FRACTION * rows

    @classmethod
    def launch(cls, caller, dec=None, src_mask=None, trg_mask=None, loss_rows=None, B=0, T=0, Le=0, n_enc=0):
        shape = None if (src_mask is None or not src_mask.is_cuda) else tuple(src_mask.shape)
        want = plan_rows(caller, B, T, Le, shape, loss_rows=loss_rows is not None, trg_mask=trg_mask is not None,
                         get_attn=getattr(dec, "get_attn", False), cond2dec=getattr(dec, "use_cond2dec", False),
                         cond2lat=getattr(dec, "use_cond2lat", False), nconds=getattr(dec, "nconds", 0), n_enc=n_enc,
                         n_dec=0 if dec is None else len(dec.layers), capturing=torch.cuda.is_current_stream_capturing(),
                         compact_fwd=COMPACT_FWD, compact_kv=COMPACT_KV, compact_enc_kv=COMPACT_ENC_KV)
        if not (want.enc_keys or want.dec_keys or want.live):
            return cls()
        ek = dk = lr = None
        if want.enc_keys or want.dec_keys:
            sm = ops.to_mask_u8(src_mask).view(B, Le)
            if want.enc_keys:
                ek = ops.KeyRows(sm, B, Le)
            if want.dec_keys and want.nc_lat > 0:
                ones = torch.ones(B, want.nc_lat, dtype=torch.uint8, device=sm.device)
                dk = ops.KeyRows(torch.cat([ones, sm], dim=1).contiguous(), B, Le + want.nc_lat)
            elif want.dec_keys:
                dk = ek if ek is not None else ops.KeyRows(sm, B, Le)
        if want.live:
            lr = ops.LiveRows.from_rows(loss_rows.to(torch.uint8).contiguous().reshape(B, T), B, T,
                                        ops.to_mask_u8(trg_mask))
        return cls(ek, dk, lr, (want.enc_rows, want.dec_rows, want.live_rows))

    def finish(self) -> "RowPlan":
        if self._usable is None:
            self._pending.finish()
            (ek, dk, lr), (re, rd, rt) = self._maps, self._rows
            self._usable = (ek if ek is not None and self.usable_keys(ek.host(), re) else None,
                            dk if dk is not None and self.usable_keys(dk.host(), rd) else None,
                            lr if lr is not None and self.usable_live(lr.host(), rt) else None)
            if self._usable[2] is not None:
                self._usable[2].fwd = True
        self.enc_keys, self.dec_keys, self.live = self._usable
        if self.live is not None and torch.cuda.is_current_stream_capturing():
            self.live = None
        return self


def next_seed() -> int:
    if _SEED["base"] != torch.initial_seed():
        _SEED["base"] = torch.initial_seed()
        _SEED["ctr"] = 0
    _SEED["ctr"] += 1
    return (_SEED["base"] * 0x9E3779B97F4A7C15 + _SEED["ctr"] * 0xD1B54A32D192ED03) & ((1 << 64) - 1)


class Run:

    def __init__(self, p: float, training: bool):
        self.p = float(p) if training else 0.0
        self.seed = next_seed() if self.p > 0 else 0
        self._site = 0
        self.kt = None

    def site(self) -> int:
        self._site += 1
        return self._site


class GradSink:

    def __init__(self):
        self.out = {}

    def __call__(self, p: torch.nn.Parameter) -> torch.Tensor:
        t = self.out.get(p)
        if t is None:
            v = getattr(p, "_gct_gview", None)
            if v is not None and id(p) not in HANDED_SLOTS and \
                    (p.grad is None or p.grad.data_ptr() != v.data_ptr()):
                t = v.view(v.shape)
                HANDED_SLOTS.add(id(p))
            else:
                t = torch.empty_like(p)
            self.out[p] = t
        return t

    def collect(self, params):
        ops.join_side()
        return tuple(self.out.get(p) for p in params)


def _empty(rows, cols, like):
    return torch.empty(rows, cols, dtype=torch.float32, device=like.device)


class MhaSaved(NamedTuple):
    xq: torch.Tensor
    xkv: torch.Tensor
    qb: torch.Tensor
    kvb: Optional[torch.Tensor]
    o: torch.Tensor
    lse: torch.Tensor
    mask_u8: object
    B: int
    Lq: int
    Lk: int
    site_p: int
    site_o: int
    fused: bool
    keys: object
    self_split: bool

    @property
    def qkv(self) -> torch.Tensor:
        assert self.kvb is None, "no fused q | k | v buffer: K | V were projected on their own"
        return self.qb


class FfnSaved(NamedTuple):
    x: torch.Tensor
    gelu_d: torch.Tensor
    hdn: torch.Tensor
    site_h: int
    site_o: int
    fused: bool


class EncLayerSaved(NamedTuple):
    x_in: torch.Tensor
    m1: torch.Tensor
    r1: torch.Tensor
    attn: MhaSaved
    a: torch.Tensor
    m2: torch.Tensor
    r2: torch.Tensor
    ffn: FfnSaved


class DecLayerSaved(NamedTuple):
    x: torch.Tensor
    m1: torch.Tensor
    r1: torch.Tensor
    attn_1: MhaSaved
    xa: torch.Tensor
    m2: torch.Tensor
    r2: torch.Tensor
    attn_2: MhaSaved
    xb: torch.Tensor
    m3: torch.Tensor
    r3: torch.Tensor
    ffn: FfnSaved


class EncoderSaved(NamedTuple):
    src: torch.Tensor
    econds: Optional[torch.Tensor]
    site_pe: int
    layers: List[EncLayerSaved]
    x_last: torch.Tensor
    mean: torch.Tensor
    rstd: torch.Tensor
    B: int
    L: int


class DecoderSaved(NamedTuple):
    trg: torch.Tensor
    z2: torch.Tensor
    dconds: Optional[torch.Tensor]
    site_pe: int
    layers: List[DecLayerSaved]
    x_last: torch.Tensor
    mean: torch.Tensor
    rstd: torch.Tensor
    B: int
    T: int
    Le: int
    Lk: int
    c2d: bool
    c2l: bool
    trg_mask_u8: Optional[torch.Tensor]
    keys: object
    live: object


def mha_fwd(run: Run, m, xq, xkv, B, Lq, Lk, mask_u8, resid, want_probs=False, keys=None, live=None):
    d, H = m.d_model, m.h
    dk = d // H
    self_attn = xkv is xq
    Mq = xq.shape[0]
    self_split = self_attn and keys is not None and live is None and not want_probs
    if self_split:
        xkv = keys.gather(xq)
    if self_attn and not self_split:
        qkv = _empty(Mq, 3 * d, xq)
        ops.linear_fwd(xq, [m.q_linear.weight, m.k_linear.weight, m.v_linear.weight],
                       [m.q_linear.bias, m.k_linear.bias, m.v_linear.bias],
                       [qkv, qkv[:, d:], qkv[:, 2 * d:]], 3 * d)
        q, k, v, ldq, ldkv = qkv, qkv[:, d:], qkv[:, 2 * d:], 3 * d, 3 * d
        qb, kvb = qkv, None
        if live is not None:
            keys = live
    else:
        qb = _empty(Mq, d, xq)
        ops.linear_fwd(xq, [m.q_linear.weight], [m.q_linear.bias], [qb], d)
        kvb = _empty(B * Lk, 2 * d, xkv) if keys is None else keys.empty(2 * d)
        ops.linear_fwd(xkv, [m.k_linear.weight, m.v_linear.weight],
                       [m.k_linear.bias, m.v_linear.bias], [kvb, kvb[:, d:]], 2 * d)
        q, k, v, ldq, ldkv = qb, kvb, kvb[:, d:], d, 2 * d
    site_p = run.site()
    o, lse, probs = ops.attn_fwd(q, k, v, ldq, ldkv, ldkv, mask_u8, B, H, Lq, Lk, dk, run.p,
                                 run.seed, site_p, want_probs=want_probs, keys=keys, live=live)
    y = _empty(Mq, d, xq)
    site_o = run.site()
    if resid is not None:
        ops.linear_fwd(o, [m.out.weight], [m.out.bias], [y], d, epi=ops.EPI_DROP_RESID,
                       resid=resid, p=run.p, seed=run.seed, site=site_o, live=live)
    else:
        ops.linear_fwd(o, [m.out.weight], [m.out.bias], [y], d)
    saved = MhaSaved(xq, xkv, qb, kvb, o, lse, mask_u8, B, Lq, Lk, site_p, site_o, resid is not None,
                     None if (self_attn and live is not None) else keys, self_split)
    return y, saved, probs


def mha_bwd(run: Run, m, sv: MhaSaved, dy, G: GradSink, dxq_out, depi_q, dxkv_out=None,
            depi_kv=ops.DEPI_STORE, live=None, gdrop=None):
    B, Lq, Lk, keys = sv.B, sv.Lq, sv.Lk, sv.keys
    d, H = m.d_model, m.h
    dk = d // H
    Mq, Mk = B * Lq, sv.xkv.shape[0]
    kt = run.kt
    new = lambda cols: _empty(Mq, cols, dy)
    if live is not None:
        Mq, kt = live.Mc, None
        new = live.empty_zero_gaps
        o_in, xq_in = (sv.o, sv.xq) if live.fwd else (live.gather(sv.o), live.gather(sv.xq))
    else:
        o_in, xq_in = sv.o, sv.xq
    if gdrop is not None:
        g = gdrop
    else:
        g = ops.dropout_bwd(dy, run.p, run.seed, sv.site_o, live=live) if (sv.fused and run.p > 0) else dy
    ops.linear_wgrad([g], d, o_in, [G(m.out.weight)], [G(m.out.bias)], kt=kt)
    do = _empty(Mq, d, dy) if live is None else live.empty(d)
    ops.linear_dgrad([g], d, Mq, [m.out.weight], do)
    if sv.kvb is None:
        dqkv = new(3 * d)
        fwdc = live is not None and live.fwd
        ops.attn_bwd(sv.qb, sv.qb[:, d:], sv.qb[:, 2 * d:], 3 * d, 3 * d, 3 * d, sv.mask_u8, sv.o, do, sv.lse, dqkv,
                     dqkv[:, d:], dqkv[:, 2 * d:], 3 * d, 3 * d, 3 * d, B, H, Lq, Lk, dk, run.p,
                     run.seed, sv.site_p, live=live, kv_compact=live is not None and not fwdc,
                     keys=live if fwdc else None)
        segs = [dqkv, dqkv[:, d:], dqkv[:, 2 * d:]]
        ops.linear_wgrad(segs, 3 * d, xq_in,
                         [G(m.q_linear.weight), G(m.k_linear.weight), G(m.v_linear.weight)],
                         [G(m.q_linear.bias), G(m.k_linear.bias), G(m.v_linear.bias)], kt=kt)
        ops.linear_dgrad(segs, 3 * d, Mq,
                         [m.q_linear.weight, m.k_linear.weight, m.v_linear.weight], dxq_out,
                         depi=depi_q)
    else:
        dq = new(d)
        if keys is None:
            dkv = _empty(Mk, 2 * d, dy)
        else:
            dkv = keys.empty_zero_gaps(2 * d)
        ops.attn_bwd(sv.qb, sv.kvb, sv.kvb[:, d:], d, 2 * d, 2 * d, sv.mask_u8, sv.o, do, sv.lse, dq, dkv, dkv[:, d:],
                     d, 2 * d, 2 * d, B, H, Lq, Lk, dk, run.p, run.seed, sv.site_p, live=live, keys=keys)
        ops.linear_wgrad([dq], d, xq_in, [G(m.q_linear.weight)], [G(m.q_linear.bias)], kt=kt)
        ops.linear_wgrad([dkv, dkv[:, d:]], 2 * d, sv.xkv,
                         [G(m.k_linear.weight), G(m.v_linear.weight)],
                         [G(m.k_linear.bias), G(m.v_linear.bias)])
        ops.linear_dgrad([dq], d, Mq, [m.q_linear.weight], dxq_out, depi=depi_q)
        if sv.self_split:
            dxk = keys.empty(d)
            ops.linear_dgrad([dkv, dkv[:, d:]], 2 * d, Mk, [m.k_linear.weight, m.v_linear.weight], dxk)
            keys.scatter_add(dxk, dxq_out)
        elif dxkv_out is not None:
            ops.linear_dgrad([dkv, dkv[:, d:]], 2 * d, Mk, [m.k_linear.weight, m.v_linear.weight],
                             dxkv_out, depi=depi_kv)


def ffn_fwd(run: Run, ff, x, resid, live=None):
    M, d = x.shape
    dff = ff.linear_1.weight.shape[0]
    gelu_d = _empty(M, dff, x)
    hdn = _empty(M, dff, x)
    site_h = run.site()
    ops.linear_fwd(x, [ff.linear_1.weight], [ff.linear_1.bias], [hdn], dff, epi=ops.EPI_GELU_DROP_SAVE,
                   pre=gelu_d, p=run.p, seed=run.seed, site=site_h, live=live)
    y = _empty(M, d, x)
    site_o = run.site()
    if resid is not None:
        ops.linear_fwd(hdn, [ff.linear_2.weight], [ff.linear_2.bias], [y], d,
                       epi=ops.EPI_DROP_RESID, resid=resid, p=run.p, seed=run.seed, site=site_o, live=live)
    else:
        ops.linear_fwd(hdn, [ff.linear_2.weight], [ff.linear_2.bias], [y], d)
    return y, FfnSaved(x, gelu_d, hdn, site_h, site_o, resid is not None)


def ffn_bwd(run: Run, ff, sv: FfnSaved, dy, G: GradSink, dx_out, depi, live=None, gdrop=None):
    x, gelu_d, hdn = sv.x, sv.gelu_d, sv.hdn
    M, d = x.shape
    dff = gelu_d.shape[1]
    kt = run.kt
    if live is not None:
        M, kt = live.Mc, None
        if not live.fwd:
            x, hdn = live.gather(x), live.gather(hdn)
    if gdrop is not None:
        g = gdrop
    else:
        g = ops.dropout_bwd(dy, run.p, run.seed, sv.site_o, live=live) if (sv.fused and run.p > 0) else dy
    ops.linear_wgrad([g], d, hdn, [G(ff.linear_2.weight)], [G(ff.linear_2.bias)], kt=kt)
    dpre = _empty(M, dff, dy) if live is None else live.empty(dff)
    ops.linear_dgrad([g], d, M, [ff.linear_2.weight], dpre, depi=ops.DEPI_MUL_SAVED, pre=gelu_d,
                     p=run.p, seed=run.seed, site=sv.site_h, live=live, pre_full=live is not None and not live.fwd)
    ops.linear_wgrad([dpre], dff, x, [G(ff.linear_1.weight)], [G(ff.linear_1.bias)], kt=kt)
    ops.linear_dgrad([dpre], dff, M, [ff.linear_1.weight], dx_out, depi=depi)


def enc_layer_fwd(run: Run, layer, x_in, B, L, mask_u8, want_probs=False, keys=None):
    n1, m1, r1 = ops.norm_fwd(x_in, layer.norm_1.alpha, layer.norm_1.bias, layer.norm_1.eps)
    a, sv_a, probs = mha_fwd(run, layer.attn, n1, n1, B, L, L, mask_u8, n1, want_probs, keys=keys)
    n2, m2, r2 = ops.norm_fwd(a, layer.norm_2.alpha, layer.norm_2.bias, layer.norm_2.eps)
    out, sv_f = ffn_fwd(run, layer.ff, n2, n2)
    return out, EncLayerSaved(x_in, m1, r1, sv_a, a, m2, r2, sv_f), probs


def _mha_drop(run: Run, sv: MhaSaved, buf):
    return (buf, run.p, run.seed, sv.site_o) if (buf is not None and sv.fused and run.p > 0) else None


def _ffn_drop(run: Run, sv: Optional[FfnSaved], buf):
    return (buf, run.p, run.seed, sv.site_o) if (buf is not None and sv is not None and sv.fused and run.p > 0) else None


def enc_layer_bwd(run: Run, layer, sv: EncLayerSaved, g, G: GradSink, gd=None, gdbuf=None, below=None):
    with ops.deferred_reductions():
        ffn_bwd(run, layer.ff, sv.ffn, g, G, g, ops.DEPI_ACCUM, gdrop=gd)
        dr = _mha_drop(run, sv.attn, gdbuf)
        ops.norm_bwd(g, sv.a, layer.norm_2.alpha, sv.m2, sv.r2, G(layer.norm_2.alpha), G(layer.norm_2.bias),
                     out=g, eps=layer.norm_2.eps, drop=dr)
        mha_bwd(run, layer.attn, sv.attn, g, G, g, ops.DEPI_ACCUM, gdrop=None if dr is None else gdbuf)
        dr = _ffn_drop(run, below, gdbuf)
        ops.norm_bwd(g, sv.x_in, layer.norm_1.alpha, sv.m1, sv.r1, G(layer.norm_1.alpha), G(layer.norm_1.bias),
                     out=g, eps=layer.norm_1.eps, drop=dr)
    _grads_done(layer, G)
    return g, (None if dr is None else gdbuf)


def dec_layer_fwd(run: Run, layer, x, e, B, T, Lk, src_mask_u8, trg_mask_u8, want_probs=False, keys=None, live=None):
    x2, m1, r1 = ops.norm_fwd(x, layer.norm_1.alpha, layer.norm_1.bias, layer.norm_1.eps)
    xa, sa1, p1 = mha_fwd(run, layer.attn_1, x2, x2, B, T, T, trg_mask_u8, x, want_probs, live=live)
    x2, m2, r2 = ops.norm_fwd(xa, layer.norm_2.alpha, layer.norm_2.bias, layer.norm_2.eps)
    xb, sa2, p2 = mha_fwd(run, layer.attn_2, x2, e, B, T, Lk, src_mask_u8, xa, want_probs, keys=keys, live=live)
    x2, m3, r3 = ops.norm_fwd(xb, layer.norm_3.alpha, layer.norm_3.bias, layer.norm_3.eps)
    xc, sf = ffn_fwd(run, layer.ff, x2, xb, live=live)
    return xc, DecLayerSaved(x, m1, r1, sa1, xa, m2, r2, sa2, xb, m3, r3, sf), p1, p2


def dec_layer_bwd(run: Run, layer, sv: DecLayerSaved, g, de, first_de, G: GradSink, live=None, gd=None, gdbuf=None,
                  below=None):
    t = torch.empty_like(g) if live is None else live.empty(g.shape[1])
    with ops.deferred_reductions():
        ffn_bwd(run, layer.ff, sv.ffn, g, G, t, ops.DEPI_STORE, live=live, gdrop=gd)
        dr = _mha_drop(run, sv.attn_2, gdbuf)
        ops.norm_bwd(t, sv.xb, layer.norm_3.alpha, sv.m3, sv.r3, G(layer.norm_3.alpha), G(layer.norm_3.bias),
                     dres=g, out=g, eps=layer.norm_3.eps, live=live, drop=dr)
        mha_bwd(run, layer.attn_2, sv.attn_2, g, G, t, ops.DEPI_STORE, de,
                ops.DEPI_STORE if first_de else ops.DEPI_ACCUM, live=live, gdrop=None if dr is None else gdbuf)
        dr = _mha_drop(run, sv.attn_1, gdbuf)
        ops.norm_bwd(t, sv.xa, layer.norm_2.alpha, sv.m2, sv.r2, G(layer.norm_2.alpha), G(layer.norm_2.bias),
                     dres=g, out=g, eps=layer.norm_2.eps, live=live, drop=dr)
        mha_bwd(run, layer.attn_1, sv.attn_1, g, G, t, ops.DEPI_STORE, live=live, gdrop=None if dr is None else gdbuf)
        dr = _ffn_drop(run, below, gdbuf)
        ops.norm_bwd(t, sv.x, layer.norm_1.alpha, sv.m1, sv.r1, G(layer.norm_1.alpha), G(layer.norm_1.bias),
                     dres=g, out=g, eps=layer.norm_1.eps, live=live, drop=dr)
    _grads_done(layer, G)
    return g, (None if dr is None else gdbuf)


def _pe2d(pe_mod, L):
    pe = pe_mod.pe
    if L > pe.shape[1]:
        raise ValueError(f"sequence length {L} exceeds the positional table ({pe.shape[1]})")
    return pe[0]


def encoder_trunk_fwd(enc, run: Run, src, mask_u8, econds, want_probs, plan: RowPlan):
    keys = plan.enc_keys
    B, S = src.shape
    d, nc = enc.d_model, enc.nconds
    cond = None
    if nc > 0:
        if econds is None:
            raise ValueError("econds required when nconds > 0")
        cond = ops.small_linear_fwd(econds.contiguous(), enc.embed_cond2enc.weight,
                                    enc.embed_cond2enc.bias)
    L = S + nc
    mask_u8 = ops.pack_mask(mask_u8, B, L, L)
    site_pe = run.site()
    x = ops.embed_pe_fwd(src, enc.embed_sentence.embed.weight, cond, _pe2d(enc.pe, L), nc,
                         math.sqrt(d), run.p, run.seed, site_pe)
    layers, probs = [], []
    for layer in enc.layers:
        x, sv, pr = enc_layer_fwd(run, layer, x, B, L, mask_u8, want_probs, keys=keys)
        layers.append(sv)
        probs.append(pr)
    y, mean, rstd = ops.norm_fwd(x, enc.norm.alpha, enc.norm.bias, enc.norm.eps)
    return y.view(B, L, d), EncoderSaved(src, econds, site_pe, layers, x, mean, rstd, B, L), probs


def encoder_trunk_bwd(enc, run: Run, sv: EncoderSaved, dy, G: GradSink):
    layers, B, L = sv.layers, sv.B, sv.L
    d, nc = enc.d_model, enc.nconds
    g = dy.reshape(B * L, d).clone()
    gdbuf = torch.empty_like(g) if (run.p > 0 and len(layers) > 0) else None
    dr = _ffn_drop(run, layers[-1].ffn if layers else None, gdbuf)
    ops.norm_bwd(g, sv.x_last, enc.norm.alpha, sv.mean, sv.rstd, G(enc.norm.alpha), G(enc.norm.bias), out=g,
                 eps=enc.norm.eps, drop=dr)
    gd = None if dr is None else gdbuf
    for i in range(len(layers) - 1, -1, -1):
        g, gd = enc_layer_bwd(run, enc.layers[i], layers[i], g, G, gd=gd, gdbuf=gdbuf,
                              below=layers[i - 1].ffn if i > 0 else None)
    dcond = torch.empty(B, nc * d, dtype=torch.float32, device=g.device) if nc > 0 else None
    ops.embed_pe_bwd(g, sv.src, G(enc.embed_sentence.embed.weight), dcond, nc, math.sqrt(d), run.p,
                     run.seed, sv.site_pe)
    if nc > 0:
        ops.small_linear_bwd(dcond, sv.econds.contiguous(), G(enc.embed_cond2enc.weight),
                             G(enc.embed_cond2enc.bias))


def decoder_trunk_fwd(dec, run: Run, trg, z, src_mask_u8, trg_mask_u8, dconds, want_probs, plan: RowPlan):
    B, T0 = trg.shape
    d, nc = dec.d_model, dec.nconds
    Le, lat = z.shape[1], z.shape[2]
    z2 = z.reshape(B * Le, lat)
    c2d = dec.use_cond2dec and nc > 0
    c2l = (not c2d) and dec.use_cond2lat and nc > 0
    cond_x = None
    if c2d:
        cond_x = ops.small_linear_fwd(dconds.contiguous(), dec.embed_cond2dec.weight,
                                      dec.embed_cond2dec.bias)
    T = T0 + (nc if c2d else 0)
    site_pe = run.site()
    x = ops.embed_pe_fwd(trg, dec.embed.embed.weight, cond_x, _pe2d(dec.pe, T), nc if c2d else 0,
                         math.sqrt(d), run.p, run.seed, site_pe)
    ez = _empty(B * Le, d, z2)
    ops.linear_fwd(z2, [dec.fc_z.weight], [dec.fc_z.bias], [ez], d)
    Lk = Le
    e = ez
    if c2l:
        Lk = Le + nc
        cl = ops.small_linear_fwd(dconds.contiguous(), dec.embed_cond2lat.weight,
                                  dec.embed_cond2lat.bias)
        e = _empty(B * Lk, d, z2)
        ops.copy_rows(cl, nc, 0, e, Lk, 0, B * nc, nc, d)
        ops.copy_rows(ez, Le, 0, e, Lk, nc, B * Le, Le, d)
        if src_mask_u8 is not None:
            ones = torch.ones(B, nc, dtype=torch.uint8, device=src_mask_u8.device)
            src_mask_u8 = torch.cat([ones, src_mask_u8.view(B, Le)], dim=1).contiguous()
    layers, p1s, p2s = [], [], []
    live, keys = plan.live, plan.dec_keys
    if live is not None:
        x = live.gather(x)
    if keys is not None:
        e = keys.gather(e)
    src_m = ops.pack_mask(src_mask_u8, B, T, Lk)
    trg_m = ops.pack_mask(trg_mask_u8, B, T, T)
    for layer in dec.layers:
        x, sv, p1, p2 = dec_layer_fwd(run, layer, x, e, B, T, Lk, src_m, trg_m, want_probs, keys=keys, live=live)
        layers.append(sv)
        p1s.append(p1)
        p2s.append(p2)
    y, mean, rstd = ops.norm_fwd(x, dec.norm.alpha, dec.norm.bias, dec.norm.eps)
    saved = DecoderSaved(trg, z2, dconds, site_pe, layers, x, mean, rstd, B, T, Le, Lk, c2d, c2l,
                         trg_mask_u8.u8 if isinstance(trg_mask_u8, ops.MaskBits) else trg_mask_u8, keys, live)
    if live is not None:
        return y, saved, p1s, p2s
    return y.view(B, T, d), saved, p1s, p2s


def decoder_trunk_bwd(dec, run: Run, sv: DecoderSaved, dy, G: GradSink, need_dz=True):
    layers, keys, live_fwd = sv.layers, sv.keys, sv.live
    B, T, Le, Lk = sv.B, sv.T, sv.Le, sv.Lk
    new_de = (lambda: _empty(B * Lk, d, dy)) if keys is None else (lambda: keys.empty(d))
    d, nc = dec.d_model, dec.nconds
    live, lr = live_fwd, None
    if live_fwd is None:
        lr = ops.LiveRows(dy.reshape(B * T, d), B, T, sv.trg_mask_u8) if (COMPACT_BWD or (B * T) % 32 == 0) else None
        if COMPACT_BWD and len(dec.layers) > 0 and not torch.cuda.is_current_stream_capturing():
            live = lr if RowPlan.usable_live(lr.host(), B * T) else None
    if live_fwd is not None:
        g = dy.reshape(live.Mc, d).clone()
    elif live is not None:
        g = live.gather(dy.reshape(B * T, d))
    else:
        g = dy.reshape(B * T, d).clone()
        run.kt = lr.kt if (lr is not None and (B * T) % 32 == 0) else None
    gdbuf = None
    if run.p > 0 and len(layers) > 0:
        gdbuf = torch.empty_like(g) if live is None else live.empty(d)
    dr = _ffn_drop(run, layers[-1].ffn if layers else None, gdbuf)
    ops.norm_bwd(g, sv.x_last, dec.norm.alpha, sv.mean, sv.rstd, G(dec.norm.alpha), G(dec.norm.bias), out=g,
                 eps=dec.norm.eps, live=live, drop=dr)
    gd = None if dr is None else gdbuf
    de = new_de()
    for i in range(len(layers) - 1, -1, -1):
        g, gd = dec_layer_bwd(run, dec.layers[i], layers[i], g, de, i == len(layers) - 1, G, live=live, gd=gd,
                              gdbuf=gdbuf, below=layers[i - 1].ffn if i > 0 else None)
    run.kt = None
    if live is not None:
        g = live.scatter(g)
    if len(dec.layers) == 0:
        de.zero_()
    if keys is not None:
        de = keys.scatter(de)
    dcx = torch.empty(B, nc * d, dtype=torch.float32, device=g.device) if sv.c2d else None
    ops.embed_pe_bwd(g, sv.trg, G(dec.embed.embed.weight), dcx, nc if sv.c2d else 0, math.sqrt(d), run.p,
                     run.seed, sv.site_pe)
    if sv.c2d:
        ops.small_linear_bwd(dcx, sv.dconds.contiguous(), G(dec.embed_cond2dec.weight),
                             G(dec.embed_cond2dec.bias))
    dez = de
    if sv.c2l:
        dcl = torch.empty(B, nc * d, dtype=torch.float32, device=g.device)
        ops.copy_rows(de, Lk, 0, dcl, nc, 0, B * nc, nc, d)
        ops.small_linear_bwd(dcl, sv.dconds.contiguous(), G(dec.embed_cond2lat.weight),
                             G(dec.embed_cond2lat.bias))
        dez = _empty(B * Le, d, g)
        ops.copy_rows(de, Lk, nc, dez, Le, 0, B * Le, Le, d)
    ops.linear_wgrad([dez], d, sv.z2, [G(dec.fc_z.weight)], [G(dec.fc_z.bias)])
    dz = None
    if need_dz:
        dz = _empty(B * Le, sv.z2.shape[1], g)
        ops.linear_dgrad([dez], d, B * Le, [dec.fc_z.weight], dz)
        dz = dz.view(B, Le, -1)
    return dz


def _f32c(t):
    return t if (t.dtype == torch.float32 and t.is_contiguous()) else t.float().contiguous()


class EncoderFn(torch.autograd.Function):
    @staticmethod
    def forward(ctx, enc, run, src, mask_u8, econds, want_probs, plan, *params):
        y, saved, probs = encoder_trunk_fwd(enc, run, src, mask_u8, econds, want_probs, plan)
        ctx.enc, ctx.run, ctx.saved, ctx.params = enc, run, saved, params
        if want_probs:
            for p in probs:
                ctx.mark_non_differentiable(p)
            return (y, *probs)
        return y

    @staticmethod
    def backward(ctx, dy, *unused):
        G = GradSink()
        encoder_trunk_bwd(ctx.enc, ctx.run, ctx.saved, _f32c(dy), G)
        ctx.saved = None
        return (None,) * 7 + G.collect(ctx.params)


class DecoderFn(torch.autograd.Function):
    @staticmethod
    def forward(ctx, dec, run, trg, z, src_mask_u8, trg_mask_u8, dconds, want_probs, plan, *params):
        y, saved, p1, p2 = decoder_trunk_fwd(dec, run, trg, _f32c(z), src_mask_u8, trg_mask_u8, dconds, want_probs,
                                             plan)
        ctx.dec, ctx.run, ctx.saved, ctx.params = dec, run, saved, params
        ctx.need_dz = z.requires_grad
        if want_probs:
            for p in p1 + p2:
                ctx.mark_non_differentiable(p)
            return (y, *p1, *p2)
        return y

    @staticmethod
    def backward(ctx, dy, *unused):
        G = GradSink()
        dz = decoder_trunk_bwd(ctx.dec, ctx.run, ctx.saved, _f32c(dy), G, ctx.need_dz)
        ctx.saved = None
        return (None, None, None, dz, None, None, None, None, None) + G.collect(ctx.params)
# ... 295 lines not shown
```

### gct_plus_amd/ops.py

```python
from __future__ import annotations

import contextlib
import math
import os
import threading
import weakref
from typing import List, Optional, Sequence

import torch

from . import _lib
from ._lib import check

EPI_BIAS, EPI_GELU_DROP, EPI_DROP_RESID, EPI_GELU_DROP_SAVE = 0, 1, 2, 3
DEPI_STORE, DEPI_ACCUM, DEPI_GELU_BWD, DEPI_MUL_SAVED = 0, 1, 2, 3


def _L():
    return _lib.load()


_raw_stream, _cur_dev = torch._C._cuda_getCurrentRawStream, torch._C._cuda_getDevice


def _st():
    return _raw_stream(_cur_dev())


def _p(t: Optional[torch.Tensor]):
    return None if t is None else t.data_ptr()


def _chk(t: torch.Tensor, name: str, dtype=torch.float32):
    if not t.is_cuda:
        raise _lib.GctError(f"{name}: expected a CUDA (ROCm) tensor; gct_plus_amd has no CPU path")
    if t.dtype != dtype:
        raise _lib.GctError(f"{name}: expected {dtype}, got {t.dtype}")
    return t


SIDE_ENABLED = os.environ.get("GCT_SIDE_STREAM", "0") != "0"
_SIDE = {}
_PENDING = {}


def _side_stream(device):
    idx = device.index if device.index is not None else torch.cuda.current_device()
    st = _SIDE.get(idx)
    if st is None:
        st = torch.cuda.Stream(device=idx)
        _SIDE[idx] = st
    return st


def _wait_pending(t):
    if _PENDING and t is not None:
        ev = _PENDING.pop(t.untyped_storage().data_ptr(), None)
        if ev is not None:
            torch.cuda.current_stream().wait_event(ev)


def join_side(device=None):
    if _SIDE:
        cur = torch.cuda.current_stream()
        for st in _SIDE.values():
            cur.wait_stream(st)
        _PENDING.clear()


_WS = {}


def workspace(nbytes: int, device) -> torch.Tensor:
    key = (device.index if device.index is not None else torch.cuda.current_device(), _st())
    buf = _WS.get(key)
    if buf is None or buf.numel() * 4 < nbytes:
        n = max(int(nbytes * 1.25) // 4 + 64, 1 << 20)
        buf = torch.empty(n, dtype=torch.float32, device=device)
        _WS[key] = buf
    return buf


DEFER_REDUCTIONS = os.environ.get("GCT_DEFER_REDUCTIONS", "1") != "0"
class _DeferState(threading.local):
    def __init__(self):
        self.d = {"on": False, "off": 0, "demand": 0, "want": 0}


_DEFER_TL = _DeferState()
_ARENA = {}


def kept_workspace(nbytes: int, device) -> torch.Tensor:
    if not _DEFER_TL.d["on"]:
        return workspace(nbytes, device)
    key = (device.index if device.index is not None else torch.cuda.current_device(), _st())
    n = (int(nbytes) + 255) // 256 * 64
    _DEFER_TL.d["demand"] += n
    buf = _ARENA.get(key)
    if buf is None or _DEFER_TL.d["off"] + n > buf.numel():
        check(_L().gct_reduce_defer_flush(_st()), "gct_reduce_defer_flush")
        _DEFER_TL.d["off"] = 0
        if buf is None or n > buf.numel():
            buf = _ARENA[key] = torch.empty(max(n, _DEFER_TL.d["want"], 1 << 22), dtype=torch.float32, device=device)
    out = buf[_DEFER_TL.d["off"]:_DEFER_TL.d["off"] + n]
    _DEFER_TL.d["off"] += n
    return out


class deferred_reductions:

    def __enter__(self):
        self.mine = (DEFER_REDUCTIONS and not _DEFER_TL.d["on"] and not SIDE_ENABLED
                     and not torch.cuda.is_current_stream_capturing())
        if self.mine:
            key = (torch.cuda.current_device(), _st())
            buf = _ARENA.get(key)
            if buf is not None and buf.numel() < _DEFER_TL.d["want"]:
                del _ARENA[key]
            _DEFER_TL.d.update(on=True, off=0, demand=0)
            check(_L().gct_reduce_defer_begin(), "gct_reduce_defer_begin")
        return self

    def __exit__(self, et, ev, tb):
        if self.mine:
            _DEFER_TL.d["on"] = False
            _DEFER_TL.d["want"] = max(_DEFER_TL.d["want"], _DEFER_TL.d["demand"])
            rc = _L().gct_reduce_defer_end(_st())
            if et is None:
                check(rc, "gct_reduce_defer_end")
        return False


_WS_NEED = {}


def _ws_need(fn: str, a: int, b: int, c: int) -> int:
    key = (fn, a, b, c)
    v = _WS_NEED.get(key)
    if v is None:
        v = _WS_NEED[key] = int(getattr(_L(), fn)(a, b, c))
    return v


def norm_fwd(x2d, alpha, bias, eps=1e-6, out=None):
    _chk(x2d, "norm_fwd.x")
    rows, d = x2d.shape
    y = torch.empty_like(x2d) if out is None else out
    mean = torch.empty(rows, dtype=torch.float32, device=x2d.device)
    rstd = torch.empty(rows, dtype=torch.float32, device=x2d.device)
    check(_L().gct_norm_fwd(_p(x2d), _p(alpha), _p(bias), _p(y), _p(mean), _p(rstd), rows, d, eps,
                            _st()), "gct_norm_fwd")
    return y, mean, rstd


def norm_bwd(dy, x2d, alpha, mean, rstd, dalpha, dbias, dres=None, out=None, eps=1e-6, live=None, drop=None):
    src_rows, d = x2d.shape
    rows = src_rows if live is None else live.Mc
    if live is not None and live.fwd:
        src_rows = 0
    dx = (torch.empty_like(x2d) if live is None else live.empty(d)) if out is None else out
    _wait_pending(out)
    if drop is not None:
        _wait_pending(drop[0])
    ws = kept_workspace(_L().gct_rowred_ws_bytes(rows, 2 * d), x2d.device)
    check(_L().gct_norm_bwd(_p(dy), _p(x2d), _p(alpha), _p(mean), _p(rstd), _p(dres), _p(dx),
                            _p(dalpha), _p(dbias), _p(ws), rows, d, eps,
                            None if live is None else _p(live.quad_list), src_rows,
                            None if drop is None else _p(drop[0]), 0.0 if drop is None else drop[1],
                            0 if drop is None else drop[2], 0 if drop is None else drop[3], _st()), "gct_norm_bwd")
    return dx


def embed_pe_fwd(tok, table, cond, pe2d, n_c, scale, p, seed, site, d=None):
    _chk(tok, "embed.tok", torch.int64)
    B, S = tok.shape
    if table is not None:
        vocab, d = table.shape
    else:
        vocab = 1
    out = torch.empty(B * (S + n_c), d, dtype=torch.float32, device=pe2d.device)
    check(_L().gct_embed_pe_fwd(_p(tok), _p(table), _p(cond), _p(pe2d), _p(out), B, S, n_c, d, vocab,
                                scale, p, seed, site, _st()), "gct_embed_pe_fwd")
    return out


def embed_pe_bwd(dout, tok, dtable, dcond, n_c, scale, p, seed, site, d=None):
    B, S = tok.shape
    if dtable is not None:
        vocab, d = dtable.shape
    else:
        vocab = 1
    ws = kept_workspace(_L().gct_embed_ws_bytes(B, S, d, vocab), dout.device)
    check(_L().gct_embed_pe_bwd(_p(dout), _p(tok), _p(dtable), _p(dcond), _p(ws), B, S, n_c, d, vocab,
                                scale, p, seed, site, _st()), "gct_embed_pe_bwd")


PROFILE = None
PROFILE_KINDS = None


class _Timed:
    def __init__(self, kind, flops, nbytes=0):
        self.kind, self.flops, self.nbytes = kind, flops, nbytes

    def __enter__(self):
        self.on = PROFILE is not None and (PROFILE_KINDS is None or self.kind in PROFILE_KINDS)
        if self.on:
            self.c0 = gemm_launch_counts()[1]
            self.k0 = _L().gct_gemm_x6_kernel_launches()
            self.e0 = torch.cuda.Event(enable_timing=True)
            self.e1 = torch.cuda.Event(enable_timing=True)
            self.e0.record()
        return self

    def __exit__(self, *a):
        if self.on:
            self.e1.record()
            kind = self.kind + "[x6]" if gemm_launch_counts()[1] > self.c0 else self.kind
            PROFILE.setdefault(kind, []).append((self.flops, self.e0, self.e1))
            PROFILE["_x6_kernel_launches:" + kind] = PROFILE.get("_x6_kernel_launches:" + kind, 0) + \
                (_L().gct_gemm_x6_kernel_launches() - self.k0)
            PROFILE["_bytes:" + kind] = PROFILE.get("_bytes:" + kind, 0) + self.nbytes


def _seg3(ts: Sequence[Optional[torch.Tensor]]):
    ts = list(ts) + [None] * (3 - len(ts))
    return [_p(t) for t in ts]


GEMM_F32, GEMM_BF16X6 = 0, 1
GEMM_BF16X3 = 2
_PLANES = []


def gemm_set_mode(mode: int):
    check(_L().gct_gemm_set_mode(int(mode)), "gct_gemm_set_mode")


def gemm_get_mode() -> int:
    return _L().gct_gemm_get_mode()


def gemm_x3_launches() -> int:
    return int(_L().gct_gemm_x3_launches())


def gemm_launch_counts():
    import ctypes
    out = (ctypes.c_int64 * 2)()
    check(_L().gct_gemm_launch_counts(ctypes.cast(out, ctypes.c_void_p)), "gct_gemm_launch_counts")
    return int(out[0]), int(out[1])


def split_planes(flat: torch.Tensor, planes: Optional[torch.Tensor] = None) -> torch.Tensor:
    _chk(flat, "flat")
    n = flat.numel()
    if planes is None:
        planes = torch.empty(3, n, dtype=torch.int16, device=flat.device)
    check(_L().gct_split_planes(_p(flat), n, _p(planes), planes.stride(0), _st()), "gct_split_planes")
    return planes


def _drop_planes(base: int, end: int):
    _PLANES[:] = [e for e in _PLANES if e[1] <= base or e[0] >= end]


def register_planes(flat: torch.Tensor, planes: torch.Tensor):
    base, end = flat.data_ptr(), flat.data_ptr() + flat.numel() * 4
    known = any(e[0] == base and e[1] == end and e[4]() is flat for e in _PLANES)
    _drop_planes(base, end)
    _PLANES.append((base, end, planes, flat.numel(), weakref.ref(flat)))
    if not known:
        weakref.finalize(flat, _drop_planes, base, end)


def unregister_planes(flat: torch.Tensor):
    _drop_planes(flat.data_ptr(), flat.data_ptr() + flat.numel() * 4)


def _plane_ptr(ws_):
    if not _PLANES:
        return None, 0
    a = ws_[0].data_ptr()
    for base, end, planes, numel, ref in _PLANES:
        if base <= a < end:
            if ref() is None:
                return None, 0
            if all(base <= w.data_ptr() < end for w in ws_[1:]):
                return planes.data_ptr() + (a - base) // 2, planes.stride(0)
            return None, 0
    return None, 0


def linear_fwd(x2d, ws_: Sequence[torch.Tensor], bs: Sequence[Optional[torch.Tensor]],
               outs: Sequence[torch.Tensor], ldy: int, epi=EPI_BIAS, resid=None, pre=None,
               p=0.0, seed=0, site=0, splitk_ws: Optional[torch.Tensor] = None, ws: Optional[torch.Tensor] = None,
               live=None):
    M, K = x2d.shape
    nper = ws_[0].shape[0]
    w = _seg3(ws_)
    b = _seg3(bs)
    y = _seg3(outs)
    need = _ws_need("gct_linear_fwd_ws_bytes", M, K, nper * len(ws_))
    for t in (splitk_ws, ws):
        if t is not None and t.numel() * 4 < need:
            raise _lib.GctError(f"linear_fwd: workspace of {t.numel() * 4} B < {need} B "
                                f"(gct_linear_fwd_ws_bytes({M}, {K}, {nper * len(ws_)}))")
    if splitk_ws is not None:
        wp, pstride, wsb, quad_map, timed = None, 0, splitk_ws, None, contextlib.nullcontext()
    else:
        wp, pstride = _plane_ptr(ws_)
        wsb = ws if ws is not None else (workspace(need, x2d.device) if need > 256 else None)
        quad_map = None if live is None else _p(live.quad_list)
        N = nper * len(ws_)
        nbytes = 4 * M * K + (6 if wp else 4) * N * K + 4 * N + 4 * M * N * (2 if epi in (EPI_GELU_DROP, EPI_DROP_RESID, EPI_GELU_DROP_SAVE) else 1)
        timed = _Timed("gemm_fwd", 2.0 * M * K * N, nbytes)
    with timed:
        check(_L().gct_linear_fwd(_p(x2d), x2d.stride(0), M, K, w[0], w[1], w[2], ws_[0].stride(0),
                                  wp, pstride, b[0], b[1], b[2], len(ws_), nper, y[0], y[1], y[2],
                                  ldy, epi, _p(resid), _p(pre), p, seed, site, _p(wsb),
                                  0 if wsb is None else wsb.numel() * 4, quad_map, _st()),
              "gct_linear_fwd")


def linear_dgrad(dys: Sequence[torch.Tensor], lddy: int, M: int, ws_: Sequence[torch.Tensor], dx,
                 depi=DEPI_STORE, pre=None, p=0.0, seed=0, site=0, live=None, pre_full=False):
    nper, K = ws_[0].shape
    d = _seg3(dys)
    w = _seg3(ws_)
    _wait_pending(dx)
    with _Timed("gemm_dgrad", 2.0 * M * K * nper * len(ws_)):
        wp, pstride = _plane_ptr(ws_)
        need = _ws_need("gct_linear_dgrad_ws_bytes", M, nper * len(ws_), K)
        wsb = workspace(need, dx.device) if need > 256 else None
        check(_L().gct_linear_dgrad(d[0], d[1], d[2], lddy, M, len(ws_), nper, w[0], w[1], w[2],
                                    ws_[0].stride(0), wp, pstride, K, _p(dx), dx.stride(0), depi,
                                    _p(pre), p, seed, site, _p(wsb), 0 if wsb is None else wsb.numel() * 4,
                                    None if live is None else _p(live.quad_list),
                                    pre.shape[0] if (live is not None and pre is not None and pre_full) else 0,
                                    _st()), "gct_linear_dgrad")


def nonzero_row_tiles(x2d: torch.Tensor):
    _chk(x2d, "x2d")
    rows, cols = x2d.shape
    nt = (rows + 31) // 32
    lst = torch.empty(max(nt, 1), dtype=torch.int32, device=x2d.device)
    cnt = torch.empty(1, dtype=torch.int32, device=x2d.device)
    flags = torch.empty(max(nt, 1), dtype=torch.uint8, device=x2d.device)
    check(_L().gct_nonzero_row_tiles(_p(x2d), x2d.stride(0), rows, cols, _p(lst), _p(cnt), _p(flags), _st()),
          "gct_nonzero_row_tiles")
    return lst, cnt


_SKIPPED = {}
_SKIPPED_MSG = ("{} decoder rows that an earlier forward skipped (loss_rows: rows that do not reach the loss) received a "
                "non-zero gradient in its backward pass: that gradient was ignored, and the optimizer steps launched since "
                "then were skipped on the device (FusedAdam's guard), so no wrong update has been applied; this error is "
                "raised at the first host read-back after the fact.  Call the model without loss_rows "
                "(forward_propagation(..., skip_ignored=False)) for losses other than the reference's ignore_index "
                "cross-entropy.")


def assert_no_skipped_row_gradients():
    n = int(skipped_row_gradients().item())
    if n:
        skipped_row_gradients().zero_()
        raise _lib.GctError(_SKIPPED_MSG.format(n))


def skipped_row_gradients():
    dev = torch.cuda.current_device()
    t = _SKIPPED.get(dev)
    if t is None:
        t = _SKIPPED[dev] = torch.zeros(1, dtype=torch.int32, device=torch.device("cuda", dev))
    return t


class LiveRows:
    SLACK = 256
    fwd = False

    def __init__(self, g2d, B, T, mask_u8, lists=True):
        _chk(g2d, "g2d")
        dev = g2d.device
        M = B * T
        assert g2d.shape[0] == M
        nt, nq = (M + 31) // 32, (M + 3) // 4
        i32 = lambda n: torch.empty(max(n, 1), dtype=torch.int32, device=dev)
        self.B, self.T, self.M, self.dev = B, T, M, dev
        self.live = torch.empty(max(M, 1), dtype=torch.uint8, device=dev)
        self.n_b, self.info = i32(B), i32(8)
        self.cstart = i32(B) if lists else None
        self.quad_list = i32(nq + 32) if lists else None
        qrank = i32(nq) if lists else None
        self.tile_list, self.tile_count = i32(nt), i32(1)
        flags = torch.empty(max(nt, 1), dtype=torch.uint8, device=dev)
        if mask_u8 is None:
            sb = sq = 0
        else:
            _chk(mask_u8, "live_rows.mask", torch.uint8)
            sb, sq = _mask_strides(mask_u8, B, T, T)
        check(_L().gct_live_rows(_p(g2d), g2d.stride(0), B, T, g2d.shape[1], _p(mask_u8), sb, sq, _p(self.live),
                                 _p(self.n_b), _p(self.info), _p(self.cstart), _p(self.quad_list), _p(qrank),
                                 _p(self.tile_list), _p(self.tile_count), _p(flags), _st()), "gct_live_rows")
        self.kt = (self.tile_list, self.tile_count)
        self._host = None
        self.Mc = None

    @classmethod
    def from_rows(cls, rows_u8, B, T, mask_u8):
        _chk(rows_u8, "live_rows.rows", torch.uint8)
        return cls(rows_u8.reshape(B * T, 1).to(torch.float32), B, T, mask_u8)

    def _fill_host(self, v):
        self._host = dict(n_live=v[0], violations=v[1], nonprefix=v[2], tiles=v[3], padded=v[4], quads=v[5], empty=v[6])
        self.Mc = v[4]

    def host(self):
        if self._host is None:
            PendingReadBack(self).finish()
        return self._host

    def scatter_add(self, src2d, dst2d):
        cols = src2d.shape[1]
        check(_L().gct_scatter_add_quads(_p(src2d), src2d.stride(0), _p(self.quad_list), self.Mc, cols, _p(dst2d),
                                         dst2d.stride(0), self.M, _st()), "gct_scatter_add_quads")
        return dst2d

    def check_grad(self, g2d):
        check(_L().gct_dead_rows_nonzero(_p(g2d), g2d.stride(0), self.M, g2d.shape[1], _p(self.live),
                                         _p(skipped_row_gradients()), _st()), "gct_dead_rows_nonzero")

    def empty(self, cols):
        return torch.empty(self.Mc + self.SLACK, cols, dtype=torch.float32, device=self.dev)[:self.Mc]

    def empty_zero_gaps(self, cols):
        t = self.empty(cols)
        check(_L().gct_zero_gap_rows(_p(t), t.stride(0), cols, _p(self.cstart), _p(self.n_b), self.B, self.Mc, _st()),
              "gct_zero_gap_rows")
        return t

    def gather(self, src2d, out=None):
        cols = src2d.shape[1]
        dst = self.empty(cols) if out is None else out
        check(_L().gct_gather_quads(_p(src2d), src2d.stride(0), src2d.shape[0], _p(self.quad_list), self.Mc, cols,
                                    _p(dst), dst.stride(0), _st()), "gct_gather_quads")
        return dst

    def scatter(self, src2d, out=None):
        cols = src2d.shape[1]
        dst = torch.zeros(self.M, cols, dtype=torch.float32, device=self.dev) if out is None else out
        check(_L().gct_scatter_quads(_p(src2d), src2d.stride(0), _p(self.quad_list), self.Mc, cols, _p(dst),
                                     dst.stride(0), self.M, _st()), "gct_scatter_quads")
        return dst


HOST_BLOCKED_S = [0.0]


class PendingReadBack:

    def __init__(self, *objs):
        seen, self.objs = set(), []
        for o in objs:
            if o is not None and o._host is None and id(o) not in seen:
                seen.add(id(o))
                self.objs.append(o)
        self.host = self.ev = None
        if self.objs:
            dev = torch.cat([o.info for o in self.objs] + [skipped_row_gradients()])
            self.host = torch.empty(dev.numel(), dtype=dev.dtype, pin_memory=True)
            self.host.copy_(dev, non_blocking=True)
            self.ev = torch.cuda.Event()
            self.ev.record()

    def finish(self):
        if self.host is None:
            return
        import time
        t0 = time.perf_counter()
        self.ev.synchronize()
        HOST_BLOCKED_S[0] += time.perf_counter() - t0
        v = self.host.tolist()
        self.host = None
        for i, o in enumerate(self.objs):
            if o._host is None:
                o._fill_host(v[8 * i:8 * i + 8])
        if v[-1] != 0:
            skipped_row_gradients().zero_()
            raise _lib.GctError(_SKIPPED_MSG.format(v[-1]))


class KeyRows(LiveRows):

    def __init__(self, mask_u8, B, Lk):
        _chk(mask_u8, "key_rows.mask", torch.uint8)
        dev = mask_u8.device
        M = B * Lk
        nq = (M + 3) // 4
        i32 = lambda n: torch.empty(max(n, 1), dtype=torch.int32, device=dev)
        self.B, self.T, self.M, self.dev = B, Lk, M, dev
        self.live = torch.empty(max(M, 1), dtype=torch.uint8, device=dev)
        self.n_b, self.info = i32(B), i32(8)
        self.cstart, self.quad_list = i32(B), i32(nq + 32)
        qrank = i32(nq)
        check(_L().gct_key_rows(_p(mask_u8), Lk, B, Lk, _p(self.live), _p(self.n_b), _p(self.info), _p(self.cstart),
                                _p(self.quad_list), _p(qrank), _st()), "gct_key_rows")
        self._host = None
        self.Mc = None



def linear_wgrad(dys: Sequence[torch.Tensor], lddy: int, x2d, dws: Sequence[torch.Tensor],
                 dbs: Sequence[Optional[torch.Tensor]], kt=None):
    M, K = x2d.shape
    nper = dws[0].shape[0]
    nseg = len(dws)
    d = _seg3(dys)
    dw = _seg3(dws)
    db = _seg3(dbs)

    def launch():
        ws = kept_workspace(_ws_need("gct_wgrad_ws_bytes", M, nseg * nper, K), x2d.device)
        with _Timed("gemm_wgrad+bias+reduce", 2.0 * M * K * nper * nseg):
            check(_L().gct_linear_wgrad(d[0], d[1], d[2], lddy, M, nseg, nper, _p(x2d), x2d.stride(0),
                                        K, dw[0], dw[1], dw[2], K, db[0], db[1], db[2], _p(ws),
                                        _p(kt[0]) if kt else None, _p(kt[1]) if kt else None, _st()),
                  "gct_linear_wgrad")

    if not SIDE_ENABLED or torch.cuda.is_current_stream_capturing():
        launch()
        return
    main = torch.cuda.current_stream()
    side = _side_stream(x2d.device)
    ready = torch.cuda.Event()
    ready.record(main)
    side.wait_event(ready)
    with torch.cuda.stream(side):
        launch()
        done = torch.cuda.Event()
        done.record(side)
    for t in list(dys) + [x2d]:
        t.record_stream(side)
        _PENDING[t.untyped_storage().data_ptr()] = done


def dropout_bwd(dout2d, p, seed, site, out=None, live=None):
    rows, cols = dout2d.shape
    if live is not None:
        rows = live.Mc
    dy = torch.empty_like(dout2d) if out is None else out
    _wait_pending(out)
    check(_L().gct_dropout_bwd(_p(dout2d), _p(dy), rows, cols, p, seed, site,
                               None if live is None else _p(live.quad_list), _st()), "gct_dropout_bwd")
    return dy


ATTN_DIRECT_MAX_KEYS = 96


class MaskBits:

    def __init__(self, mask_u8, B, Lq, Lk):
        _chk(mask_u8, "attn.mask", torch.uint8)
        if Lk > 256 or Lq > 256:
            raise _lib.GctError(f"attention: sequence length {max(Lq, Lk)} > 256 unsupported")
        sb, sq = _mask_strides(mask_u8, B, Lq, Lk)
        rows = 1 if sq == 0 else Lq
        self.u8, self.B, self.Lq, self.Lk = mask_u8, B, Lq, Lk
        self.bits = torch.empty(B, rows, 8, dtype=torch.int32, device=mask_u8.device)
        self.sb, self.sq = rows * 8, (0 if sq == 0 else 8)
        ntr = 1 if sq == 0 else (Lq + 15) // 16
        self.tiles = torch.empty(B, ntr, dtype=torch.int32, device=mask_u8.device)
        self.t_sb, self.t_su = ntr, (0 if sq == 0 else 1)
        check(_L().gct_attn_mask_pack(_p(mask_u8), sb, sq, B, Lq, Lk, _p(self.bits), _p(self.tiles), _st()),
              "gct_attn_mask_pack")


def pack_mask(mask, B, Lq, Lk) -> Optional["MaskBits"]:
    if mask is None or isinstance(mask, MaskBits):
        if isinstance(mask, MaskBits) and (mask.B, mask.Lk) != (B, Lk):
            raise _lib.GctError(f"packed mask was built for B={mask.B}, Lk={mask.Lk}, not B={B}, Lk={Lk}")
        return mask
    return MaskBits(to_mask_u8(mask), B, Lq, Lk)


def _mb(mask, B, Lq, Lk):
    mb = pack_mask(mask, B, Lq, Lk)
    if mb is None:
        return None, 0, 0, None
    if mb.t_su and mb.Lq != Lq:
        raise _lib.GctError(f"packed mask was built for Lq={mb.Lq}, not Lq={Lq}")
    return mb.bits.data_ptr(), mb.sb, mb.sq, mb


def _tb(mb):
    return (None, 0, 0) if mb is None else (mb.tiles.data_ptr(), mb.t_sb, mb.t_su)


def attn_fwd(q, k, v, ld_q, ld_k, ld_v, mask, B, H, Lq, Lk, dk, p, seed, site, out=None,
             want_probs=False, keys=None, live=None):
    dev = q.device
    if out is not None:
        o = out
    elif live is not None:
        o = live.empty_zero_gaps(H * dk)
    else:
        o = torch.empty(B * Lq, H * dk, dtype=torch.float32, device=dev)
    lse = torch.empty(B * H * Lq, dtype=torch.float32, device=dev)
    probs = torch.empty(B, H, Lq, Lk, dtype=torch.float32, device=dev) if want_probs else None
    mp, sb, sq, mask_owner = _mb(mask, B, Lq, Lk)
    check(_L().gct_attn_fwd(_p(q), ld_q, _p(k), ld_k, _p(v), ld_v, mp, sb, sq, _p(o),
                            o.stride(0), _p(lse), _p(probs), B, H, Lq, Lk, dk,
                            1.0 / math.sqrt(dk), p, seed, site, None if keys is None else _p(keys.cstart),
                            None if keys is None else _p(keys.n_b), *_tb(mask_owner),
                            None if live is None else _p(live.cstart), None if live is None else _p(live.n_b),
                            _st()), "gct_attn_fwd")
    del mask_owner
    return o, lse, probs


_ATTN_BWD_WS = {}


def _attn_bwd_ws(dev, nbytes):
    if nbytes <= 0:
        return None
    key = (dev, _st())
    ws = _ATTN_BWD_WS.get(key)
    if ws is None or ws.numel() < nbytes:
        ws = torch.empty(nbytes, dtype=torch.uint8, device=dev)
        _ATTN_BWD_WS[key] = ws
    return ws


def attn_bwd(q, k, v, ld_q, ld_k, ld_v, mask, o, dout, lse, dq, dk_, dv, ld_dq, ld_dk, ld_dv,
             B, H, Lq, Lk, dk, p, seed, site, live=None, kv_compact=False, keys=None):
    ws = _attn_bwd_ws(q.device, int(_L().gct_attn_bwd_ws_bytes(B, H, Lq, Lk)))
    mp, sb, sq, mask_owner = _mb(mask, B, Lq, Lk)
    check(_L().gct_attn_bwd(_p(q), ld_q, _p(k), ld_k, _p(v), ld_v, mp, sb, sq, _p(o),
                            _p(dout), o.stride(0), _p(lse), _p(dq), ld_dq, _p(dk_), ld_dk,
                            _p(dv), ld_dv, B, H, Lq, Lk, dk, 1.0 / math.sqrt(dk), p, seed, site,
                            None if live is None else _p(live.cstart), None if live is None else _p(live.n_b),
                            int(bool(kv_compact)) | (2 if (live is not None and live.fwd) else 0),
# ... 319 lines not shown
```

### include/gctplus_hip.h

```cpp
#ifndef GCTPLUS_HIP_H
#define GCTPLUS_HIP_H

#include <stdint.h>

#ifdef __cplusplus
extern "C" {
#endif

#define GCT_OK 0
#define GCT_ERR_ARG (-1)
#define GCT_ERR_HIP (-2)

#define GCT_ABI_VERSION 22

int gct_version(void);
const char* gct_last_error(void);

int64_t gct_wgrad_ws_bytes(int64_t M, int64_t Ntot, int64_t K);
int64_t gct_rowred_ws_bytes(int64_t rows, int64_t cols);

int gct_norm_fwd(const float* x, const float* alpha, const float* bias, float* y,
                 float* mean, float* rstd, int64_t rows, int d, float eps, void* stream);
int gct_norm_bwd(const float* dy, const float* x, const float* alpha, const float* mean,
                 const float* rstd, const float* dres, float* dx, float* dalpha, float* dbias,
                 float* ws, int64_t rows, int d, float eps, const int32_t* quad_map, int64_t src_rows,
                 float* drop_out, float p, uint64_t seed, uint32_t site, void* stream);

int gct_embed_pe_fwd(const int64_t* tok, const float* table, const float* cond, const float* pe,
                     float* out, int B, int S, int n_c, int d, int vocab, float scale, float p,
                     uint64_t seed, uint32_t site, void* stream);
int64_t gct_embed_ws_bytes(int B, int S, int d, int vocab);
int gct_embed_pe_bwd(const float* dout, const int64_t* tok, float* dtable, float* dcond,
                     float* ws, int B, int S, int n_c, int d, int vocab, float scale, float p,
                     uint64_t seed, uint32_t site, void* stream);

#define GCT_EPI_BIAS 0
#define GCT_EPI_GELU_DROP 1
#define GCT_EPI_DROP_RESID 2
#define GCT_EPI_GELU_DROP_SAVE 3
int gct_linear_fwd(const float* x, int64_t ldx, int64_t M, int K,
                   const float* w0, const float* w1, const float* w2, int64_t ldw,
                   const uint16_t* wp0, int64_t plane_stride,
                   const float* b0, const float* b1, const float* b2,
                   int nseg, int nper, float* y0, float* y1, float* y2, int64_t ldy,
                   int epi, const float* resid, float* pre, float p, uint64_t seed, uint32_t site,
                   float* ws, int64_t ws_bytes, const int32_t* quad_map, void* stream);
int64_t gct_linear_fwd_ws_bytes(int64_t M, int K, int Ntot);

#define GCT_DEPI_STORE 0
#define GCT_DEPI_ACCUM 1
#define GCT_DEPI_GELU_BWD 2
#define GCT_DEPI_MUL_SAVED 3
int gct_linear_dgrad(const float* dy0, const float* dy1, const float* dy2, int64_t lddy,
                     int64_t M, int nseg, int nper,
                     const float* w0, const float* w1, const float* w2, int64_t ldw,
                     const uint16_t* wp0, int64_t plane_stride, int K,
                     float* dx, int64_t lddx, int depi, const float* pre, float p, uint64_t seed,
                     uint32_t site, float* ws, int64_t ws_bytes, const int32_t* quad_map, int64_t pre_rows,
                     void* stream);
int64_t gct_linear_dgrad_ws_bytes(int64_t M, int Ntot, int K);

int gct_linear_wgrad(const float* dy0, const float* dy1, const float* dy2, int64_t lddy,
                     int64_t M, int nseg, int nper, const float* x, int64_t ldx, int K,
                     float* dw0, float* dw1, float* dw2, int64_t lddw,
                     float* db0, float* db1, float* db2, float* ws,
                     const int32_t* tile_list, const int32_t* tile_count, void* stream);

#define GCT_GEMM_F32 0
#define GCT_GEMM_BF16X6 1
#define GCT_GEMM_BF16X3 2
int gct_gemm_set_mode(int mode);
int gct_gemm_get_mode(void);
int gct_gemm_launch_counts(int64_t* out2);
int64_t gct_gemm_x6_kernel_launches(void);
int64_t gct_gemm_x3_launches(void);

int gct_split_planes(const float* src, int64_t numel, uint16_t* planes, int64_t plane_stride,
                     void* stream);

int gct_dead_rows_nonzero(const float* g, int64_t ld, int64_t rows, int cols, const uint8_t* live,
                          int32_t* counter, void* stream);
int gct_nonzero_row_tiles(const float* x, int64_t ld, int64_t rows, int cols, int32_t* list,
                          int32_t* count, uint8_t* flags_ws, void* stream);
int gct_live_rows(const float* g, int64_t ld, int B, int T, int cols, const uint8_t* mask, int64_t mask_sb,
                  int64_t mask_sq, uint8_t* live, int32_t* n_b, int32_t* info, int32_t* cstart,
                  int32_t* quad_list, int32_t* qrank_ws, int32_t* tile_list, int32_t* tile_count,
                  uint8_t* tile_flags_ws, void* stream);
int gct_key_rows(const uint8_t* mask, int64_t mask_sb, int B, int Lk, uint8_t* live, int32_t* n_b, int32_t* info,
                 int32_t* cstart, int32_t* quad_list, int32_t* qrank_ws, void* stream);
int gct_gather_quads(const float* src, int64_t ld, int64_t M, const int32_t* quad_list, int64_t nrows, int cols,
                     float* dst, int64_t ldd, void* stream);
int gct_scatter_quads(const float* src, int64_t ld, const int32_t* quad_list, int64_t nrows, int cols, float* dst,
                      int64_t ldd, int64_t M, void* stream);
int gct_zero_gap_rows(float* buf, int64_t ld, int cols, const int32_t* cstart, const int32_t* n_b, int B, int64_t nrows,
                      void* stream);
int gct_scatter_add_quads(const float* src, int64_t ld, const int32_t* quad_list, int64_t nrows, int cols, float* dst,
                          int64_t ldd, int64_t M, void* stream);

int gct_dropout_bwd(const float* dout, float* dy, int64_t rows, int cols, float p, uint64_t seed,
                    uint32_t site, const int32_t* quad_map, void* stream);

#define GCT_ATTN_DIRECT_MAX_KEYS 96
int gct_attn_mask_pack(const uint8_t* mask, int64_t mask_sb, int64_t mask_sq, int B, int Lq, int Lk,
                       uint32_t* bits, uint32_t* tiles, void* stream);
int gct_trg_mask_tokens(const int64_t* tokens, int64_t ld_tok, int64_t pad, int B, int T, uint8_t* out, void* stream);
int gct_attn_fwd(const float* q, int64_t ldq, const float* k, int64_t ldk, const float* v,
                 int64_t ldv, const uint32_t* mbits, int64_t mb_sb, int64_t mb_sq,
                 float* o, int64_t ldo, float* lse, float* probs, int B, int H, int Lq, int Lk,
                 int dk, float scale, float p, uint64_t seed, uint32_t site, const int32_t* kstart,
                 const int32_t* klen, const uint32_t* tbits, int64_t tb_sb, int64_t tb_su,
                 const int32_t* qstart, const int32_t* qlen, void* stream);
int gct_attn_bwd(const float* q, int64_t ldq, const float* k, int64_t ldk, const float* v,
                 int64_t ldv, const uint32_t* mbits, int64_t mb_sb, int64_t mb_sq,
                 const float* o, const float* dout, int64_t ldo, const float* lse,
                 float* dq, int64_t lddq, float* dk_, int64_t lddk, float* dv, int64_t lddv,
                 int B, int H, int Lq, int Lk, int dk, float scale, float p, uint64_t seed,
                 uint32_t site, const int32_t* cstart, const int32_t* nlive, int kv_compact,
                 const int32_t* kstart, const int32_t* klen, const uint32_t* tbits, int64_t tb_sb, int64_t tb_su,
                 void* ws, int64_t ws_bytes, void* stream);
int64_t gct_attn_bwd_ws_bytes(int B, int H, int Lq, int Lk);

int gct_reparam_fwd(const float* mu, const float* log_var, const float* eps_in, float* eps_out,
                    float* z, int64_t n, uint64_t seed, uint32_t site, void* stream);
int gct_reparam_bwd(const float* dz, const float* log_var, const float* eps, const float* dmu_ext,
                    const float* dlv_ext, float* dmu, float* dlv, int64_t n, void* stream);
int gct_kld_fwd(const float* mu, const float* log_var, float* out, float* ws, int64_t n,
                void* stream);
int gct_kld_bwd(const float* mu, const float* log_var, const float* gout, float* dmu, float* dlv,
                int64_t n, void* stream);

int gct_ce_fwd(const float* logits, const int64_t* target, float* out, float* ws, int64_t rows,
               int V, int64_t pad_id, void* stream);
int gct_ce_bwd(const float* logits, const int64_t* target, const float* gout, float* dlogits,
               int64_t rows, int V, int64_t pad_id, void* stream);
int gct_seq_logp(const float* logits, int64_t ld, int V, int64_t rows_per_seq, int row_shift, const int64_t* ys,
                 int64_t ld_ys, const int32_t* prefix_lens, int64_t pad_id, int n, int W, float* token_logp,
                 int64_t ld_out, float* logp, int32_t* tokens, int32_t* hits, void* stream);
int gct_chosen_logp(const float* logits, int V, const int64_t* ys, int64_t ld_ys, const int32_t* pos,
                    const int32_t* row_off, const int32_t* item, const int32_t* prefix_len, int64_t pad_id, float* out,
                    int64_t ld_out, int out_rows, int n, void* stream);

int gct_adam_step(float* p, const float* g, float* m, float* v, int64_t n, float lr, float b1,
                  float b2, float eps, int64_t step, float gscale, const int32_t* skip_if_nonzero,
                  void* stream);

int gct_attn_decode(const float* q, int64_t ldq, float* k, float* v, int64_t kv_row,
                    int64_t kv_batch, const uint8_t* valid, int64_t valid_sb, float* o, int64_t ldo,
                    int n, int H, int Lc, int dk, float scale, const int32_t* pos, int cache_off,
                    const float* knew, const float* vnew, int64_t ldn, const int32_t* klen,
                    const int32_t* row_off, void* stream);
int gct_attn_decode_z(const float* q, int64_t ldq, int qoff, const float* z, int64_t z_batch, int lat, int Le,
                      const float* ckv, int64_t ckv_batch, int64_t ld_ckv, int nc, const uint8_t* valid,
                      int64_t valid_sb, const int32_t* klen, float* out, int64_t ldo, int ooff, int n, int H, int dk,
                      float scale, void* stream);
int gct_decode_embed(const int64_t* ys, int64_t ld_ys, const int32_t* pos, int pe_off, const float* table,
                     int vocab, const float* pe, float* out, int n, int d, float scale, const int32_t* row_off,
                     void* stream);
int gct_decode_advance(int32_t* pos, void* stream);
typedef struct GctSampleFilter {
  int32_t k;
  float top_p;
  float inv_temp;
  int32_t reserved;
} GctSampleFilter;
#define GCT_SAMPLE_FILTER_MAX_VOCAB 1024
int gct_select_token(const float* logits, int V, int64_t* ys, int64_t ld_ys, int pos, uint8_t* valid,
                     int64_t valid_sb, uint8_t* done, float* probs_out, int n, int mode,
                     int64_t pad_id, int64_t eos_id, uint64_t seed, const int32_t* pos_dev, int valid_off,
                     const uint64_t* seed_dev, const int32_t* row_off, const GctSampleFilter* filt,
                     const int32_t* item, const int32_t* prefix_len, int item_base, void* stream);

#define GCT_GRAMMAR_ATOM 0
#define GCT_GRAMMAR_BOND 1
#define GCT_GRAMMAR_OPEN 2
#define GCT_GRAMMAR_CLOSE 3
#define GCT_GRAMMAR_RING 4
#define GCT_GRAMMAR_DOT 5
#define GCT_GRAMMAR_EOS 6
#define GCT_GRAMMAR_PAD 7
#define GCT_GRAMMAR_BANNED 8
#define GCT_GRAMMAR_MAX_RINGS 64
int gct_grammar_mask(const float* logits, float* masked, int V, const int32_t* table, const int64_t* ys, int64_t ld_ys,
                     int T, int n, const int32_t* pos, const int32_t* row_off, const int32_t* gram, const int32_t* item,
                     const int32_t* prefix_len, const int32_t* limit, void* stream);

#define GCT_STREAM_MAX_ROWS 8192
#define GCT_STREAM_MAX_LAYERS 16
typedef struct GctStreamState {
  int64_t* ys;
  uint8_t* valid;
  uint8_t* done;
  int32_t* row_off;
  const int32_t* pos;
  float* z3;
  uint8_t* src_valid;
  int32_t* src_klen;
  float* ckv[GCT_STREAM_MAX_LAYERS];
  int32_t* item;
  int32_t* harvest;
  uint8_t* fresh;
  const float* z_pool;
  const uint8_t* valid_pool;
  const int32_t* klen_pool;
  const float* ckv_pool[GCT_STREAM_MAX_LAYERS];
  const int64_t* prefix_pool;
  const int32_t* prefix_len;
  const int32_t* limit;
  int64_t* out_ys;
  int32_t* out_len;
  int32_t* row_of;
  int32_t* start_step;
  int32_t* next_item;
  int32_t* n_harvested;
  const int32_t* enable;
  int64_t rows, items, ld_ys, valid_sb, valid_off, T, width, t0_max, z_row, Lk, ckv_row, layers, pad_id;
} GctStreamState;
int gct_stream_refill(const GctStreamState* state, void* stream);

#define GCT_BEAM_MAX_K 16
#define GCT_BEAM_MAX_VOCAB 65536
int gct_attn_decode_beam(const float* q, int64_t ldq, float* k, float* v, int64_t kv_row, int64_t kv_batch,
                         const uint8_t* valid, int64_t valid_sb, float* o, int64_t ldo, int n, int H, int T, int dk,
                         float scale, const int32_t* pos, int cache_off, const float* knew, const float* vnew,
                         int64_t ldn, const int32_t* kv_src, int64_t ld_src, void* stream);
int gct_beam_select(const float* logits, int V, int n, int k, float* scores, uint8_t* finished, int32_t* lengths,
                    int32_t* parent, int64_t* ys, int64_t ld_ys, uint8_t* valid, int64_t valid_sb, int valid_off,
                    int32_t* kv_src, int64_t ld_src, int T, uint8_t* done, const int32_t* pos_dev, int64_t pad_id,
                    int64_t eos_id, void* stream);

int gct_smiles_tokenize(const char* smi, int with_sep, int32_t* tok_start, int32_t* tok_len,
                        int max_tokens);
int gct_smiles_encode_batch(const char* const* smiles, int n, int with_sep, const char* const* vocab,
                            int vocab_size, int64_t unk_id, int64_t pad_id, int64_t sos_id,
                            int64_t eos_id, int64_t* out, int64_t width, int32_t* lengths);

int gct_copy_rows(const float* src, int64_t src_rpb, int64_t src_off, float* dst, int64_t dst_rpb,
                  int64_t dst_off, int64_t rows, int64_t rpb, int cols, int accumulate,
                  void* stream);
int gct_small_linear_fwd(const float* x, const float* w, const float* b, float* y, int rows,
                         int K, int N, void* stream);
int gct_small_linear_bwd(const float* dy, const float* x, float* dw, float* db, int rows, int K,
                         int N, void* stream);
int gct_reduce_slabs(const float* slabs, int nslab, int64_t stride, float* dst, int64_t n,
                     int accumulate, void* stream);
int gct_reduce_defer_begin(void);
int gct_reduce_defer_flush(void* stream);
int gct_reduce_defer_end(void* stream);
int gct_reduce_defer_pending(void);
int gct_add(const float* a, const float* b, float* y, int64_t n, void* stream);

#ifdef __cplusplus
}
#endif
#endif
```

Measured before the change: 11330.

## Launch independent Q and KV projection GEMMs as one grouped x6 kernel

Adds paired linear forward and dgrad entry points that run two independent GEMMs, such as the Q and KV projections in attention, as a single grouped x6 launch. The combined tile count is planned together, and the tail of the second GEMM is optionally cut out and run split-K so the last wave fills the CUs. The goal is to remove separate partially filled waves and an extra kernel launch. In exchange it needs a new pair kernel, more routing logic, and a fallback to two launches when shapes or stream capture rule the grouped path out.

```diff
diff --git a/gct_plus_amd/csrc/gemm.hip b/gct_plus_amd/csrc/gemm.hip
--- a/gct_plus_amd/csrc/gemm.hip
+++ b/gct_plus_amd/csrc/gemm.hip
@@ -1165,12 +1165,8 @@
   return ns < 1 ? 1 : (int)ns;
 }
 
-int x6_tail_plan(int64_t M, int64_t N, int64_t K, int64_t* m1_out) {
+int x6_tail_rule(int64_t rem, int64_t nkt) {
   constexpr int64_t CUS = 256;
-  const int64_t tm = (M + XBM - 1) / XBM, tn = (N + XBN - 1) / XBN, tiles = tm * tn;
-  const int64_t rem = tiles % CUS;
-  if (tiles <= CUS || rem == 0 || rem % tn != 0 || K % XBK != 0) return 1;
-  const int64_t nkt = K / XBK;
   int best = 1;
   double cost = 1.0;
   const double o = 3.3;
@@ -1178,9 +1174,44 @@
     const double c = (double)((rem * s2 + CUS - 1) / CUS) * (o + (double)nkt / s2) / (o + nkt) + 0.05;
     if (c < cost - 1e-9) { cost = c; best = s2; }
   }
-  if (best == 1 || cost > 0.75) return 1;
+  return (best == 1 || cost > 0.75) ? 1 : best;
+}
+
+int x6_tail_plan(int64_t M, int64_t N, int64_t K, int64_t* m1_out) {
+  constexpr int64_t CUS = 256;
+  const int64_t tm = (M + XBM - 1) / XBM, tn = (N + XBN - 1) / XBN, tiles = tm * tn;
+  const int64_t rem = tiles % CUS;
+  if (tiles <= CUS || rem == 0 || rem % tn != 0 || K % XBK != 0) return 1;
+  const int best = x6_tail_rule(rem, K / XBK);
+  if (best == 1) return 1;
   *m1_out = (tiles - rem) / tn * XBM;
   return best;
+}
+
+struct X6PairPlan {
+  enum Kind { NONE, GROUPED, GROUPED_CUT } kind;
+  bool swap;
+  int64_t m1;
+  int splits;
+};
+X6PairPlan x6_pair_plan(int64_t Ma, int64_t Na, int64_t Ka, int64_t Mb, int64_t Nb, int64_t Kb) {
+  constexpr int64_t CUS = 256;
+  X6PairPlan r = {X6PairPlan::NONE, Kb > Ka, 0, 1};
+  if (Ma <= 0 || Mb <= 0 || Ka % XBK != 0 || Kb % XBK != 0) return r;
+  const int64_t M0 = r.swap ? Mb : Ma, N0 = r.swap ? Nb : Na;
+  const int64_t M1 = r.swap ? Ma : Mb, N1 = r.swap ? Na : Nb, K1 = r.swap ? Ka : Kb;
+  const int64_t t0 = ((M0 + XBM - 1) / XBM) * ((N0 + XBN - 1) / XBN);
+  const int64_t tm1 = (M1 + XBM - 1) / XBM, tn1 = (N1 + XBN - 1) / XBN, T = t0 + tm1 * tn1, rem = T % CUS;
+  if (T > INT_MAX) return r;
+  r.kind = X6PairPlan::GROUPED;
+  if (T <= CUS || rem == 0) return r;
+  const int64_t rows = (rem + tn1 - 1) / tn1;
+  if (rows >= tm1) { r.kind = X6PairPlan::NONE; return r; }
+  r.splits = x6_tail_rule(rows * tn1, K1 / XBK);
+  if (r.splits == 1) return r;
+  r.kind = X6PairPlan::GROUPED_CUT;
+  r.m1 = (tm1 - rows) * XBM;
+  return r;
 }
 
 int x6_splitk_all_plan(int64_t M, int64_t N, int64_t K) {
@@ -1225,35 +1256,46 @@
   return GCT_OK;
 }
 
+GemmArgs x6_tail_rows(const GemmArgs& g, int64_t m1) {
+  GemmArgs e = g;
+  e.M = g.M - m1; e.row_base = g.row_base + m1;
+  e.a.p0 += m1 * g.lda;
+  e.c0 += m1 * g.ldc;
+  if (e.resid) e.resid += m1 * g.ldc;
+  if (e.pre) e.pre += m1 * g.ldc;
+  if (e.pre_in && !(g.pre_rows > 0 && g.quad_map)) e.pre_in += m1 * g.ldc;
+  return e;
+}
+
+template <int MODE, int NP>
+int launch_x6_tail(const GemmArgs& e, int best, hipStream_t st, float* ws) {
+  if (e.K / XBK <= 32 && x6s_tiles(e.M, e.N) <= X6_TAIL_SMALL_MAX) {
+    if (MODE == X6_FWD && x6s_ok(e, true)) return launch_x6s<X6_FWD, NP>(e, st);
+    if (MODE == X6_DGRAD && x6s_dgrad_ok(e, true)) return launch_x6s<X6_DGRAD, NP>(e, st);
+  }
+  const GemmArgs p = slab_args(e, best, ws);
+  const int rc = launch_x6<MODE, NP>(p, st);
+  if (rc) return rc;
+  return launch_fixup(e, p, st, "x6 tail fix-up");
+}
+
+inline bool stream_capturing(hipStream_t st) {
+  hipStreamCaptureStatus cap = hipStreamCaptureStatusNone;
+  return hipStreamIsCapturing(st, &cap) != hipSuccess || cap != hipStreamCaptureStatusNone;
+}
+
 template <int MODE, int NP>
 int launch_x6_tail_split(const GemmArgs& g, hipStream_t st, float* ws, int64_t ws_bytes) {
   if (MODE == X6_WGRAD || g.nsplit != 1 || !ws || !gct_aligned16(ws)) return launch_x6<MODE, NP>(g, st);
   int64_t m1 = 0;
   const int best = x6_tail_plan(g.M, g.N, g.K, &m1);
-  const int64_t m2 = g.M - m1, nkt = g.K / XBK;
-  hipStreamCaptureStatus cap = hipStreamCaptureStatusNone;
-  if (best == 1 || slab_bytes(best, m2, g.N) > ws_bytes ||
-      hipStreamIsCapturing(st, &cap) != hipSuccess || cap != hipStreamCaptureStatusNone)
+  if (best == 1 || slab_bytes(best, g.M - m1, g.N) > ws_bytes || stream_capturing(st))
     return launch_x6<MODE, NP>(g, st);
   GemmArgs head = g;
   head.M = m1;
-  int rc = launch_x6<MODE, NP>(head, st);
+  const int rc = launch_x6<MODE, NP>(head, st);
   if (rc) return rc;
-  GemmArgs e = g;
-  e.M = m2; e.row_base = g.row_base + m1;
-  e.a.p0 += m1 * g.lda;
-  e.c0 += m1 * g.ldc;
-  if (e.resid) e.resid += m1 * g.ldc;
-  if (e.pre) e.pre += m1 * g.ldc;
-  if (e.pre_in && !(g.pre_rows > 0 && g.quad_map)) e.pre_in += m1 * g.ldc;
-  if (nkt <= 32 && x6s_tiles(m2, g.N) <= X6_TAIL_SMALL_MAX) {
-    if (MODE == X6_FWD && x6s_ok(e, true)) return launch_x6s<X6_FWD, NP>(e, st);
-    if (MODE == X6_DGRAD && x6s_dgrad_ok(e, true)) return launch_x6s<X6_DGRAD, NP>(e, st);
-  }
-  const GemmArgs p = slab_args(e, best, ws);
-  rc = launch_x6<MODE, NP>(p, st);
-  if (rc) return rc;
-  return launch_fixup(e, p, st, "x6 tail fix-up");
+  return launch_x6_tail<MODE, NP>(x6_tail_rows(g, m1), best, st, ws);
 }
 
 struct GemmRoute {
@@ -1374,6 +1416,39 @@
   return GCT_OK;
 }
 
+template <bool B_KC>
+int launch_pair(const GemmArgs& ga, bool veca, const GemmArgs& gb, bool vecb, hipStream_t st, float* ws,
+                int64_t ws_bytes) {
+  constexpr int MODE = B_KC ? X6_FWD : X6_DGRAD;
+  const int mode = gemm_mode();
+  const bool x3 = mode == GCT_GEMM_BF16X3;
+  auto plain = [&](const GemmArgs& g, bool vec) {
+    return g.M > 0 && g.N > 0 && g.nsplit == 1 &&
+           plan_gemm<true, B_KC>(g, vec, mode, ws, ws_bytes).kind == GemmRoute::X6;
+  };
+  if (plain(ga, veca) && plain(gb, vecb) && !stream_capturing(st)) {
+    const X6PairPlan pl = x6_pair_plan(ga.M, ga.N, ga.K, gb.M, gb.N, gb.K);
+    if (pl.kind != X6PairPlan::NONE) {
+      const GemmArgs& g0 = pl.swap ? gb : ga;
+      const GemmArgs& g1 = pl.swap ? ga : gb;
+      const bool cut = pl.kind == X6PairPlan::GROUPED_CUT && ws && gct_aligned16(ws) &&
+                       slab_bytes(pl.splits, g1.M - pl.m1, g1.N) <= ws_bytes;
+      GemmArgs head = g1;
+      if (cut) head.M = pl.m1;
+      int rc = x3 ? launch_x6_pair<MODE, 2>(g0, head, st) : launch_x6_pair<MODE, 3>(g0, head, st);
+      if (!rc && cut) {
+        const GemmArgs e = x6_tail_rows(g1, pl.m1);
+        rc = x3 ? launch_x6_tail<MODE, 2>(e, pl.splits, st, ws) : launch_x6_tail<MODE, 3>(e, pl.splits, st, ws);
+      }
+      if (!rc && !x3) g_gemm_launches[1] += 2;
+      return rc;
+    }
+  }
+  const int rc = launch<true, B_KC>(ga, veca, st, ws, ws_bytes);
+  if (rc) return rc;
+  return launch<true, B_KC>(gb, vecb, st, ws, ws_bytes);
+}
+
 inline bool al16(const void* p) { return p == nullptr || gct_aligned16(p); }
 
 inline Seg3 mkseg(const float* p0, const float* p1, const float* p2) {
@@ -1415,13 +1490,11 @@
   return (need > cs ? need : cs) * (int64_t)sizeof(float) + 256;
 }
 
-extern "C" int gct_linear_fwd(const float* x, int64_t ldx, int64_t M, int K, const float* w0,
-                              const float* w1, const float* w2, int64_t ldw, const uint16_t* wp0,
-                              int64_t plane_stride, const float* b0, const float* b1,
-                              const float* b2, int nseg, int nper, float* y0, float* y1, float* y2,
-                              int64_t ldy, int epi, const float* resid, float* pre, float p,
-                              uint64_t seed, uint32_t site, float* ws, int64_t ws_bytes,
-                              const int32_t* quad_map, void* stream) {
+static int linear_fwd_args(GemmArgs& g, bool& vec, const float* x, int64_t ldx, int64_t M, int K, const float* w0, const float* w1, const float* w2,
+                    int64_t ldw, const uint16_t* wp0, int64_t plane_stride, const float* b0, const float* b1,
+                    const float* b2, int nseg, int nper, float* y0, float* y1, float* y2, int64_t ldy, int epi,
+                    const float* resid, float* pre, float p, uint64_t seed, uint32_t site, int64_t ws_bytes,
+                    const int32_t* quad_map) {
   GCT_CHECK_ARG(x && w0 && y0 && M >= 0 && K > 0 && nseg >= 1 && nseg <= 3 && nper > 0,
                 "linear_fwd: bad args");
   GCT_CHECK_ARG(!quad_map || M % 4 == 0, "linear_fwd: compacted rows come in quads");
@@ -1433,7 +1506,7 @@
   GCT_CHECK_ARG((epi != GCT_EPI_GELU_DROP && epi != GCT_EPI_GELU_DROP_SAVE) || pre, "linear_fwd: GELU epilogue needs pre");
   GCT_CHECK_ARG(epi != GCT_EPI_DROP_RESID || resid, "linear_fwd: residual epilogue needs resid");
   GCT_CHECK_ARG(p >= 0.f && p < 1.f, "linear_fwd: dropout p out of range");
-  GemmArgs g = {};
+  g = GemmArgs{};
   g.M = M; g.N = (int64_t)nseg * nper; g.K = K;
   GCT_CHECK_ARG(!b0 || nseg < 2 || b1, "linear_fwd: bias of segment 1 missing");
   GCT_CHECK_ARG(!b0 || nseg < 3 || b2, "linear_fwd: bias of segment 2 missing");
@@ -1446,9 +1519,50 @@
   g.thr = gct_drop_threshold(p); g.keep_scale = 1.0f / (1.0f - p); g.rng = gct_rng_make(seed, site);
   g.bp0 = wp0; g.bp_stride = plane_stride;
   g.quad_map = quad_map;
-  const bool vec = al16(x) && al16(w0) && al16(w1) && al16(w2) && (ldx % 4 == 0) &&
+  vec = al16(x) && al16(w0) && al16(w1) && al16(w2) && (ldx % 4 == 0) &&
                    (ldw % 4 == 0) && (K % 4 == 0);
+  return GCT_OK;
+}
+
+extern "C" int gct_linear_fwd(const float* x, int64_t ldx, int64_t M, int K, const float* w0,
+                              const float* w1, const float* w2, int64_t ldw, const uint16_t* wp0,
+                              int64_t plane_stride, const float* b0, const float* b1,
+                              const float* b2, int nseg, int nper, float* y0, float* y1, float* y2,
+                              int64_t ldy, int epi, const float* resid, float* pre, float p,
+                              uint64_t seed, uint32_t site, float* ws, int64_t ws_bytes,
+                              const int32_t* quad_map, void* stream) {
+  GemmArgs g;
+  bool vec;
+  const int rc = linear_fwd_args(g, vec, x, ldx, M, K, w0, w1, w2, ldw, wp0, plane_stride, b0, b1, b2, nseg, nper, y0, y1,
+                                 y2, ldy, epi, resid, pre, p, seed, site, ws_bytes, quad_map);
+  if (rc) return rc;
   return launch<true, true>(g, vec, (hipStream_t)stream, ws, ws ? ws_bytes : 0);
+}
+
+extern "C" int gct_linear_fwd_pair(
+    const float* xa, int64_t ldxa, int64_t Ma, int Ka, const float* wa0, const float* wa1, const float* wa2, int64_t ldwa,
+    const uint16_t* wpa0, int64_t plane_stride_a, const float* ba0, const float* ba1, const float* ba2, int nsega,
+    int npera, float* ya0, float* ya1, float* ya2, int64_t ldya, int epia, const float* resida, float* prea, float pa,
+    uint64_t seeda, uint32_t sitea, const int32_t* quad_map_a,
+    const float* xb, int64_t ldxb, int64_t Mb, int Kb, const float* wb0, const float* wb1, const float* wb2, int64_t ldwb,
+    const uint16_t* wpb0, int64_t plane_stride_b, const float* bb0, const float* bb1, const float* bb2, int nsegb,
+    int nperb, float* yb0, float* yb1, float* yb2, int64_t ldyb, int epib, const float* residb, float* preb, float pb,
+    uint64_t seedb, uint32_t siteb, const int32_t* quad_map_b, float* ws, int64_t ws_bytes, void* stream) {
+  GemmArgs ga, gb;
+  bool veca, vecb;
+  int rc = linear_fwd_args(ga, veca, xa, ldxa, Ma, Ka, wa0, wa1, wa2, ldwa, wpa0, plane_stride_a, ba0, ba1, ba2, nsega,
+                           npera, ya0, ya1, ya2, ldya, epia, resida, prea, pa, seeda, sitea, ws_bytes, quad_map_a);
+  if (rc) return rc;
+  rc = linear_fwd_args(gb, vecb, xb, ldxb, Mb, Kb, wb0, wb1, wb2, ldwb, wpb0, plane_stride_b, bb0, bb1, bb2, nsegb,
+                       nperb, yb0, yb1, yb2, ldyb, epib, residb, preb, pb, seedb, siteb, ws_bytes, quad_map_b);
+  if (rc) return rc;
+  return launch_pair<true>(ga, veca, gb, vecb, (hipStream_t)stream, ws, ws ? ws_bytes : 0);
+}
+
+extern "C" int64_t gct_linear_pair_ws_bytes(int64_t Ma, int64_t Na, int64_t Ka, int64_t Mb, int64_t Nb, int64_t Kb) {
+  const X6PairPlan pl = x6_pair_plan(Ma, Na, Ka, Mb, Nb, Kb);
+  if (pl.kind != X6PairPlan::GROUPED_CUT) return 0;
+  return slab_bytes(pl.splits, (pl.swap ? Ma : Mb) - pl.m1, pl.swap ? Na : Nb) + 256;
 }
 
 extern "C" int gct_gemm_set_mode(int mode) {
@@ -1499,13 +1613,11 @@
   return (tail > all ? tail : all) + 256;
 }
 
-extern "C" int gct_linear_dgrad(const float* dy0, const float* dy1, const float* dy2, int64_t lddy,
-                                int64_t M, int nseg, int nper, const float* w0, const float* w1,
-                                const float* w2, int64_t ldw, const uint16_t* wp0,
-                                int64_t plane_stride, int K, float* dx, int64_t lddx, int depi,
-                                const float* pre, float p, uint64_t seed, uint32_t site,
-                                float* ws, int64_t ws_bytes, const int32_t* quad_map, int64_t pre_rows,
-                                void* stream) {
+static int linear_dgrad_args(GemmArgs& g, bool& vec, const float* dy0, const float* dy1, const float* dy2, int64_t lddy,
+                             int64_t M, int nseg, int nper, const float* w0, const float* w1, const float* w2,
+                             int64_t ldw, const uint16_t* wp0, int64_t plane_stride, int K, float* dx, int64_t lddx,
+                             int depi, const float* pre, float p, uint64_t seed, uint32_t site, int64_t ws_bytes,
+                             const int32_t* quad_map, int64_t pre_rows) {
   GCT_CHECK_ARG(ws_bytes >= 0, "linear_dgrad: negative workspace size");
   GCT_CHECK_ARG(dy0 && w0 && dx && M >= 0 && K > 0 && nseg >= 1 && nseg <= 3 && nper > 0,
                 "linear_dgrad: bad args");
@@ -1516,7 +1628,7 @@
   GCT_CHECK_ARG(depi != GCT_DEPI_GELU_BWD || pre, "linear_dgrad: GELU bwd needs pre");
   GCT_CHECK_ARG(depi != GCT_DEPI_MUL_SAVED || pre, "linear_dgrad: saved-factor epilogue needs pre");
   GCT_CHECK_ARG(p >= 0.f && p < 1.f, "linear_dgrad: dropout p out of range");
-  GemmArgs g = {};
+  g = GemmArgs{};
   g.M = M; g.N = K; g.K = (int64_t)nseg * nper;
   g.a = mkseg(dy0, dy1, dy2); g.lda = lddy; g.a_nper = nper;
   g.b = mkseg(w0, w1, w2); g.ldb = ldw; g.b_nper = nper;
@@ -1527,9 +1639,46 @@
   g.bp0 = wp0; g.bp_stride = plane_stride;
   g.quad_map = quad_map;
   g.pre_rows = quad_map ? pre_rows : 0;
-  const bool vec = al16(dy0) && al16(dy1) && al16(dy2) && al16(w0) && al16(w1) && al16(w2) &&
+  vec = al16(dy0) && al16(dy1) && al16(dy2) && al16(w0) && al16(w1) && al16(w2) &&
                    (lddy % 4 == 0) && (ldw % 4 == 0) && (nper % 4 == 0) && (K % 4 == 0);
+  return GCT_OK;
+}
+
+extern "C" int gct_linear_dgrad(const float* dy0, const float* dy1, const float* dy2, int64_t lddy,
+                                int64_t M, int nseg, int nper, const float* w0, const float* w1,
+                                const float* w2, int64_t ldw, const uint16_t* wp0,
+                                int64_t plane_stride, int K, float* dx, int64_t lddx, int depi,
+                                const float* pre, float p, uint64_t seed, uint32_t site,
+                                float* ws, int64_t ws_bytes, const int32_t* quad_map, int64_t pre_rows,
+                                void* stream) {
+  GemmArgs g;
+  bool vec;
+  const int rc = linear_dgrad_args(g, vec, dy0, dy1, dy2, lddy, M, nseg, nper, w0, w1, w2, ldw, wp0, plane_stride, K, dx,
+                                   lddx, depi, pre, p, seed, site, ws_bytes, quad_map, pre_rows);
+  if (rc) return rc;
   return launch<true, false>(g, vec, (hipStream_t)stream, ws, ws ? ws_bytes : 0);
+}
+
+extern "C" int gct_linear_dgrad_pair(
+    const float* dya0, const float* dya1, const float* dya2, int64_t lddya, int64_t Ma, int nsega, int npera,
+    const float* wa0, const float* wa1, const float* wa2, int64_t ldwa, const uint16_t* wpa0, int64_t plane_stride_a,
+    int Ka, float* dxa, int64_t lddxa, int depia, const float* prea, float pa, uint64_t seeda, uint32_t sitea,
+    const int32_t* quad_map_a, int64_t pre_rows_a,
+    const float* dyb0, const float* dyb1, const float* dyb2, int64_t lddyb, int64_t Mb, int nsegb, int nperb,
+    const float* wb0, const float* wb1, const float* wb2, int64_t ldwb, const uint16_t* wpb0, int64_t plane_stride_b,
+    int Kb, float* dxb, int64_t lddxb, int depib, const float* preb, float pb, uint64_t seedb, uint32_t siteb,
+    const int32_t* quad_map_b, int64_t pre_rows_b, float* ws, int64_t ws_bytes, void* stream) {
+  GemmArgs ga, gb;
+  bool veca, vecb;
+  int rc = linear_dgrad_args(ga, veca, dya0, dya1, dya2, lddya, Ma, nsega, npera, wa0, wa1, wa2, ldwa, wpa0,
+                             plane_stride_a, Ka, dxa, lddxa, depia, prea, pa, seeda, sitea, ws_bytes, quad_map_a,
+                             pre_rows_a);
+  if (rc) return rc;
+  rc = linear_dgrad_args(gb, vecb, dyb0, dyb1, dyb2, lddyb, Mb, nsegb, nperb, wb0, wb1, wb2, ldwb, wpb0,
+                         plane_stride_b, Kb, dxb, lddxb, depib, preb, pb, seedb, siteb, ws_bytes, quad_map_b,
+                         pre_rows_b);
+  if (rc) return rc;
+  return launch_pair<false>(ga, veca, gb, vecb, (hipStream_t)stream, ws, ws ? ws_bytes : 0);
 }
 
 extern "C" int gct_linear_wgrad(const float* dy0, const float* dy1, const float* dy2, int64_t lddy,
diff --git a/gct_plus_amd/csrc/gemm_x6.inc b/gct_plus_amd/csrc/gemm_x6.inc
--- a/gct_plus_amd/csrc/gemm_x6.inc
+++ b/gct_plus_amd/csrc/gemm_x6.inc
@@ -70,9 +70,8 @@
 typedef float x6_f32x4 __attribute__((ext_vector_type(4)));
 #define X6_MFMA(a_, b_, c_) c_ = __builtin_amdgcn_mfma_f32_16x16x32_bf16(a_, b_, c_, 0, 0, 0)
 
-template <int MODE, int NP = 3>
-__global__ __launch_bounds__(512) __attribute__((amdgpu_waves_per_eu(2, 2))) void
-gemm_x6_kernel(const GemmArgs g) {
+template <int MODE, int NP>
+__device__ __forceinline__ void gemm_x6_tile(const GemmArgs& g, const unsigned bid, const unsigned nblk) {
   static_assert(NP == 2 || NP == 3, "bf16x3 or bf16x6");
   extern __shared__ __attribute__((aligned(16))) unsigned char xlds[];
   constexpr bool A_TR = MODE == X6_WGRAD, B_TR = MODE != X6_FWD, B_PL = MODE != X6_WGRAD;
@@ -83,7 +82,7 @@
   const unsigned tiles_n = (unsigned)((g.N + XBN - 1) / XBN);
   const unsigned tiles_m = (unsigned)((g.M + XBM - 1) / XBM);
   const unsigned per_split = tiles_m * tiles_n;
-  const unsigned lid = gct_xcd_remap(blockIdx.x, gridDim.x);
+  const unsigned lid = gct_xcd_remap(bid, nblk);
   const unsigned z = lid / per_split, rest = lid - z * per_split;
   const int64_t m0 = (int64_t)(rest / tiles_n) * XBM, n0 = (int64_t)(rest % tiles_n) * XBN;
   const int64_t kbeg = (int64_t)z * g.ksplit;
@@ -508,6 +507,24 @@
 #endif
 }
 
+template <int MODE, int NP = 3>
+__global__ __launch_bounds__(512) __attribute__((amdgpu_waves_per_eu(2, 2))) void
+gemm_x6_kernel(const GemmArgs g) {
+  gemm_x6_tile<MODE, NP>(g, blockIdx.x, gridDim.x);
+}
+
+struct GemmPairArgs {
+  GemmArgs g[2];
+};
+template <int MODE, int NP = 3>
+__global__ __launch_bounds__(512) __attribute__((amdgpu_waves_per_eu(2, 2))) void
+gemm_x6_pair_kernel(const GemmPairArgs p, const unsigned tiles0) {
+  static_assert(MODE == X6_FWD || MODE == X6_DGRAD, "grouped launches: forward and dgrad");
+  const bool second = blockIdx.x >= tiles0;
+  const GemmArgs g = p.g[second ? 1 : 0];
+  gemm_x6_tile<MODE, NP>(g, second ? blockIdx.x - tiles0 : blockIdx.x, second ? gridDim.x - tiles0 : tiles0);
+}
+
 template <int MODE>
 bool x6_ok(const GemmArgs& g, bool vec, int fwd_bn = XBN) {
   auto seg_ok = [](int64_t nper, int64_t extent, int64_t gran) { return nper >= extent || nper % gran == 0; };
@@ -548,6 +565,33 @@
   hipLaunchKernelGGL((gemm_x6_kernel<MODE, NP>), dim3((unsigned)tiles), dim3(512), X_LDS_BYTES, st, g);
   ++(NP == 3 ? g_x6_kernel_launches : g_x3_kernel_launches);
   GCT_LAUNCH_CHECK("gemm_x6");
+  return GCT_OK;
+}
+
+template <int MODE, int NP>
+int launch_x6_pair(const GemmArgs& g0, const GemmArgs& g1, hipStream_t st) {
+  const int64_t t0 = ((g0.M + XBM - 1) / XBM) * ((g0.N + XBN - 1) / XBN);
+  const int64_t t1 = ((g1.M + XBM - 1) / XBM) * ((g1.N + XBN - 1) / XBN);
+  if (t0 <= 0 || t1 <= 0 || g0.nsplit != 1 || g1.nsplit != 1 || t0 + t1 > INT_MAX) {
+    gct_set_error("gemm_x6 pair: bad grid");
+    return GCT_ERR_ARG;
+  }
+  static bool attr_set = false;
+  if (!attr_set) {
+    hipError_t e = hipFuncSetAttribute((const void*)gemm_x6_pair_kernel<MODE, NP>,
+                                       hipFuncAttributeMaxDynamicSharedMemorySize, X_LDS_BYTES);
+    if (e != hipSuccess) {
+      gct_set_error("gemm_x6 pair: cannot reserve %d bytes of LDS: %s", X_LDS_BYTES, hipGetErrorString(e));
+      return GCT_ERR_HIP;
+    }
+    attr_set = true;
+  }
+  GemmPairArgs p;
+  p.g[0] = g0; p.g[1] = g1;
+  hipLaunchKernelGGL((gemm_x6_pair_kernel<MODE, NP>), dim3((unsigned)(t0 + t1)), dim3(512), X_LDS_BYTES, st, p,
+                     (unsigned)t0);
+  ++(NP == 3 ? g_x6_kernel_launches : g_x3_kernel_launches);
+  GCT_LAUNCH_CHECK("gemm_x6 pair");
   return GCT_OK;
 }
 
diff --git a/gct_plus_amd/engine.py b/gct_plus_amd/engine.py
--- a/gct_plus_amd/engine.py
+++ b/gct_plus_amd/engine.py
@@ -282,10 +282,10 @@
             keys = live
     else:
         qb = _empty(Mq, d, xq)
-        ops.linear_fwd(xq, [m.q_linear.weight], [m.q_linear.bias], [qb], d)
         kvb = _empty(B * Lk, 2 * d, xkv) if keys is None else keys.empty(2 * d)
-        ops.linear_fwd(xkv, [m.k_linear.weight, m.v_linear.weight],
-                       [m.k_linear.bias, m.v_linear.bias], [kvb, kvb[:, d:]], 2 * d)
+        ops.linear_fwd_pair(xq, [m.q_linear.weight], [m.q_linear.bias], [qb], d,
+                            xkv, [m.k_linear.weight, m.v_linear.weight],
+                            [m.k_linear.bias, m.v_linear.bias], [kvb, kvb[:, d:]], 2 * d)
         q, k, v, ldq, ldkv = qb, kvb, kvb[:, d:], d, 2 * d
     site_p = run.site()
     o, lse, probs = ops.attn_fwd(q, k, v, ldq, ldkv, ldkv, mask_u8, B, H, Lq, Lk, dk, run.p,
@@ -349,14 +349,17 @@
         ops.linear_wgrad([dkv, dkv[:, d:]], 2 * d, sv.xkv,
                          [G(m.k_linear.weight), G(m.v_linear.weight)],
                          [G(m.k_linear.bias), G(m.v_linear.bias)])
-        ops.linear_dgrad([dq], d, Mq, [m.q_linear.weight], dxq_out, depi=depi_q)
+        wkv = [m.k_linear.weight, m.v_linear.weight]
         if sv.self_split:
             dxk = keys.empty(d)
-            ops.linear_dgrad([dkv, dkv[:, d:]], 2 * d, Mk, [m.k_linear.weight, m.v_linear.weight], dxk)
+            ops.linear_dgrad_pair([dq], d, Mq, [m.q_linear.weight], dxq_out, depi_q,
+                                  [dkv, dkv[:, d:]], 2 * d, Mk, wkv, dxk, ops.DEPI_STORE)
             keys.scatter_add(dxk, dxq_out)
         elif dxkv_out is not None:
-            ops.linear_dgrad([dkv, dkv[:, d:]], 2 * d, Mk, [m.k_linear.weight, m.v_linear.weight],
-                             dxkv_out, depi=depi_kv)
+            ops.linear_dgrad_pair([dq], d, Mq, [m.q_linear.weight], dxq_out, depi_q,
+                                  [dkv, dkv[:, d:]], 2 * d, Mk, wkv, dxkv_out, depi_kv)
+        else:
+            ops.linear_dgrad([dq], d, Mq, [m.q_linear.weight], dxq_out, depi=depi_q)
 
 
 def ffn_fwd(run: Run, ff, x, resid, live=None):
diff --git a/gct_plus_amd/ops.py b/gct_plus_amd/ops.py
--- a/gct_plus_amd/ops.py
+++ b/gct_plus_amd/ops.py
@@ -140,6 +140,14 @@
     v = _WS_NEED.get(key)
     if v is None:
         v = _WS_NEED[key] = int(getattr(_L(), fn)(a, b, c))
+    return v
+
+
+def _ws_need6(fn: str, *shape) -> int:
+    key = (fn,) + shape
+    v = _WS_NEED.get(key)
+    if v is None:
+        v = _WS_NEED[key] = int(getattr(_L(), fn)(*shape))
     return v
 
 
@@ -342,6 +350,65 @@
                                     _st()), "gct_linear_dgrad")
 
 
+GEMM_PAIRS = True
+
+
+def _fwd_bytes(M, K, N, planes):
+    return 4 * M * K + (6 if planes else 4) * N * K + 4 * N + 4 * M * N
+
+
+def linear_fwd_pair(xa, wsa: Sequence[torch.Tensor], bsa, outsa, ldya: int,
+                    xb, wsb_: Sequence[torch.Tensor], bsb, outsb, ldyb: int):
+    if not GEMM_PAIRS:
+        linear_fwd(xa, wsa, bsa, outsa, ldya)
+        linear_fwd(xb, wsb_, bsb, outsb, ldyb)
+        return
+    (Ma, Ka), (Mb, Kb) = xa.shape, xb.shape
+    npa, npb = wsa[0].shape[0], wsb_[0].shape[0]
+    Na, Nb = npa * len(wsa), npb * len(wsb_)
+    wa, ba, ya = _seg3(wsa), _seg3(bsa), _seg3(outsa)
+    wb, bb, yb = _seg3(wsb_), _seg3(bsb), _seg3(outsb)
+    need = max(_ws_need("gct_linear_fwd_ws_bytes", Ma, Ka, Na), _ws_need("gct_linear_fwd_ws_bytes", Mb, Kb, Nb),
+               _ws_need6("gct_linear_pair_ws_bytes", Ma, Na, Ka, Mb, Nb, Kb))
+    wpa, psa = _plane_ptr(wsa)
+    wpb, psb = _plane_ptr(wsb_)
+    wsb = workspace(need, xa.device) if need > 256 else None
+    with _Timed("gemm_fwd", 2.0 * Ma * Ka * Na + 2.0 * Mb * Kb * Nb,
+                _fwd_bytes(Ma, Ka, Na, wpa) + _fwd_bytes(Mb, Kb, Nb, wpb)):
+        check(_L().gct_linear_fwd_pair(
+            _p(xa), xa.stride(0), Ma, Ka, wa[0], wa[1], wa[2], wsa[0].stride(0), wpa, psa, ba[0], ba[1], ba[2],
+            len(wsa), npa, ya[0], ya[1], ya[2], ldya, EPI_BIAS, None, None, 0.0, 0, 0, None,
+            _p(xb), xb.stride(0), Mb, Kb, wb[0], wb[1], wb[2], wsb_[0].stride(0), wpb, psb, bb[0], bb[1], bb[2],
+            len(wsb_), npb, yb[0], yb[1], yb[2], ldyb, EPI_BIAS, None, None, 0.0, 0, 0, None,
+            _p(wsb), 0 if wsb is None else wsb.numel() * 4, _st()), "gct_linear_fwd_pair")
+
+
+def linear_dgrad_pair(dysa: Sequence[torch.Tensor], lddya: int, Ma: int, wsa: Sequence[torch.Tensor], dxa, depia,
+                      dysb: Sequence[torch.Tensor], lddyb: int, Mb: int, wsb_: Sequence[torch.Tensor], dxb, depib):
+    if not GEMM_PAIRS:
+        linear_dgrad(dysa, lddya, Ma, wsa, dxa, depi=depia)
+        linear_dgrad(dysb, lddyb, Mb, wsb_, dxb, depi=depib)
+        return
+    assert depia in (DEPI_STORE, DEPI_ACCUM) and depib in (DEPI_STORE, DEPI_ACCUM)
+    (npa, Ka), (npb, Kb) = wsa[0].shape, wsb_[0].shape
+    Na, Nb = npa * len(wsa), npb * len(wsb_)
+    da, wa, db, wb = _seg3(dysa), _seg3(wsa), _seg3(dysb), _seg3(wsb_)
+    _wait_pending(dxa)
+    _wait_pending(dxb)
+    with _Timed("gemm_dgrad", 2.0 * Ma * Ka * Na + 2.0 * Mb * Kb * Nb):
+        wpa, psa = _plane_ptr(wsa)
+        wpb, psb = _plane_ptr(wsb_)
+        need = max(_ws_need("gct_linear_dgrad_ws_bytes", Ma, Na, Ka), _ws_need("gct_linear_dgrad_ws_bytes", Mb, Nb, Kb),
+                   _ws_need6("gct_linear_pair_ws_bytes", Ma, Ka, Na, Mb, Kb, Nb))
+        wsb = workspace(need, dxa.device) if need > 256 else None
+        check(_L().gct_linear_dgrad_pair(
+            da[0], da[1], da[2], lddya, Ma, len(wsa), npa, wa[0], wa[1], wa[2], wsa[0].stride(0), wpa, psa, Ka,
+            _p(dxa), dxa.stride(0), depia, None, 0.0, 0, 0, None, 0,
+            db[0], db[1], db[2], lddyb, Mb, len(wsb_), npb, wb[0], wb[1], wb[2], wsb_[0].stride(0), wpb, psb, Kb,
+            _p(dxb), dxb.stride(0), depib, None, 0.0, 0, 0, None, 0,
+            _p(wsb), 0 if wsb is None else wsb.numel() * 4, _st()), "gct_linear_dgrad_pair")
+
+
 def nonzero_row_tiles(x2d: torch.Tensor):
     _chk(x2d, "x2d")
     rows, cols = x2d.shape
diff --git a/include/gctplus_hip.h b/include/gctplus_hip.h
--- a/include/gctplus_hip.h
+++ b/include/gctplus_hip.h
@@ -11,7 +11,7 @@
 #define GCT_ERR_ARG (-1)
 #define GCT_ERR_HIP (-2)
 
-#define GCT_ABI_VERSION 22
+#define GCT_ABI_VERSION 23
 
 int gct_version(void);
 const char* gct_last_error(void);
@@ -59,6 +59,36 @@
                      uint32_t site, float* ws, int64_t ws_bytes, const int32_t* quad_map, int64_t pre_rows,
                      void* stream);
 int64_t gct_linear_dgrad_ws_bytes(int64_t M, int Ntot, int K);
+
+int gct_linear_fwd_pair(const float* xa, int64_t ldxa, int64_t Ma, int Ka,
+                        const float* wa0, const float* wa1, const float* wa2, int64_t ldwa,
+                        const uint16_t* wpa0, int64_t plane_stride_a,
+                        const float* ba0, const float* ba1, const float* ba2,
+                        int nsega, int npera, float* ya0, float* ya1, float* ya2, int64_t ldya,
+                        int epia, const float* resida, float* prea, float pa, uint64_t seeda, uint32_t sitea,
+                        const int32_t* quad_map_a,
+                        const float* xb, int64_t ldxb, int64_t Mb, int Kb,
+                        const float* wb0, const float* wb1, const float* wb2, int64_t ldwb,
+                        const uint16_t* wpb0, int64_t plane_stride_b,
+                        const float* bb0, const float* bb1, const float* bb2,
+                        int nsegb, int nperb, float* yb0, float* yb1, float* yb2, int64_t ldyb,
+                        int epib, const float* residb, float* preb, float pb, uint64_t seedb, uint32_t siteb,
+                        const int32_t* quad_map_b,
+                        float* ws, int64_t ws_bytes, void* stream);
+int gct_linear_dgrad_pair(const float* dya0, const float* dya1, const float* dya2, int64_t lddya,
+                          int64_t Ma, int nsega, int npera,
+                          const float* wa0, const float* wa1, const float* wa2, int64_t ldwa,
+                          const uint16_t* wpa0, int64_t plane_stride_a, int Ka,
+                          float* dxa, int64_t lddxa, int depia, const float* prea, float pa, uint64_t seeda,
+                          uint32_t sitea, const int32_t* quad_map_a, int64_t pre_rows_a,
+                          const float* dyb0, const float* dyb1, const float* dyb2, int64_t lddyb,
+                          int64_t Mb, int nsegb, int nperb,
+                          const float* wb0, const float* wb1, const float* wb2, int64_t ldwb,
+                          const uint16_t* wpb0, int64_t plane_stride_b, int Kb,
+                          float* dxb, int64_t lddxb, int depib, const float* preb, float pb, uint64_t seedb,
+                          uint32_t siteb, const int32_t* quad_map_b, int64_t pre_rows_b,
+                          float* ws, int64_t ws_bytes, void* stream);
+int64_t gct_linear_pair_ws_bytes(int64_t Ma, int64_t Na, int64_t Ka, int64_t Mb, int64_t Nb, int64_t Kb);
 
 int gct_linear_wgrad(const float* dy0, const float* dy1, const float* dy2, int64_t lddy,
                      int64_t M, int nseg, int nper, const float* x, int64_t ldx, int K,
```

Result: no change. 11390 (median of 6 runs) (+0.5%).
